# david-andrew/TerminalRayTracer

Hardware: AMD Instinct MI355X
Metric: path rays/s (primary+secondary) at 1920x1080, 64 spheres, 8 bounces (higher is better)
Workload: dtype f64

## Files before the change

include/trt_hip_diag.h:

```cpp
#ifndef TRT_HIP_DIAG_H
#define TRT_HIP_DIAG_H

#include "trt_hip.h"

#ifdef __cplusplus
extern "C" {
#endif

int trt_set_list_pool_words(trt_context *ctx, size_t words);

int trt_enable_counters(trt_context *ctx, int enable);

int trt_read_counters(trt_context *ctx, unsigned long long *path_rays, unsigned long long *shadow_rays);

int trt_read_diagnostics(trt_context *ctx, unsigned long long *wave_loop_trips, unsigned long long *phase2_rounds);

int trt_path_family_code(trt_context *ctx, int kind, int sphere, const double *parent_origin);

long trt_read_path_tables(trt_context *ctx, const Camera *camera, unsigned long long *cells, size_t capacity_cells,
                          unsigned long long *pool, size_t capacity_pool, long info[8]);

int trt_read_sweep_fallbacks(trt_context *ctx, unsigned long long *swept_traces);

int trt_read_shading_passes(trt_context *ctx, unsigned long long *passes);

int trt_read_loop_diagnostics(trt_context *ctx, unsigned long long out[8]);

long trt_read_light_grid(trt_context *ctx, int point_light, int index, unsigned long long *masks, size_t capacity_words);

long trt_read_light_lists(trt_context *ctx, int point_light, int index, unsigned long long *cells, size_t capacity_cells,
                          unsigned long long *pool, size_t capacity_pool, long info[4]);

int trt_selftest_div_sqrt(trt_context *ctx, const double *a, const double *b, size_t n, double *quot, double *root);

int trt_selftest_unit(trt_context *ctx, const double *xyzw, size_t n, double *fast, double *reference);

int trt_selftest_cube(trt_context *ctx, const float *xyz, size_t n, float *device_out, float *host_out);

int trt_selftest_sky(trt_context *ctx, const double *dirs, size_t n, int dim, long long *exact, long long *estimate, int *ambiguous);

int trt_probe_rays(trt_context *ctx, const Ray *rays, size_t n, int *obj, double *point, double *normal,
                   double *material, double *lit);

int trt_probe_rays_production(trt_context *ctx, const Camera *camera, const Ray *rays, const int *families, size_t n, int *obj,
                              double *point, double *normal, double *material, double *lit);

long trt_launch_count(trt_context *ctx);
int trt_launch_span_ms(trt_context *first, long first_launch, trt_context *last, long last_launch, float *ms);

int trt_set_scene_image(trt_context *ctx, int mode);

int trt_render_image(trt_context *ctx, int *in_device_memory, unsigned long long *image_bytes);

int trt_set_scratch_fill(trt_context *ctx, int on);

int trt_dist_allow_rccl_override(int allow);

trt_context *trt_default_context(void);

int trt_build_counts(trt_context *ctx, unsigned long long *table_builds, unsigned long long *skybox_uploads);

int trt_ansi_delta_kernel_times(trt_context *ctx, const void *d_shown_rgb8, const void *d_next_rgb8, int width, int rows, void *d_text,
                                size_t capacity_bytes, unsigned long long *d_bytes, float *ms);
int trt_ansi_delta_half_kernel_times(trt_context *ctx, const void *d_shown_rgb8, const void *d_next_rgb8, int width, int rows, void *d_text,
                                     size_t capacity_bytes, unsigned long long *d_bytes, float *ms);

#ifdef __cplusplus
}
#endif
#endif
```

terminalraytracer_amd/csrc/trt_capi.hip:

```cpp
#include "trt_context.hpp"

using namespace trt_impl;

namespace trt_impl
{

thread_local char g_error[512] = "";

int fail(int code, const char *fmt, ...)
{
    va_list ap;
    va_start(ap, fmt);
    vsnprintf(g_error, sizeof g_error, fmt, ap);
    va_end(ap);
    return code;
}

unsigned long long skybox_stamp(const Skybox *sky)
{
    unsigned long long h = 1469598103934665603ull;
    const size_t face = (size_t)sky->dim * sky->dim, step = face / 256 ? face / 256 : 1;
    for (int f = 0; f < 6; f++)
        for (size_t i = 0; i < face; i += step)
        {
            const Color c = sky->colors[f][i];
            h = (h ^ c.r) * 1099511628211ull;
            h = (h ^ c.g) * 1099511628211ull;
            h = (h ^ c.b) * 1099511628211ull;
        }
    const Color last = sky->colors[5][face - 1];
    return (h ^ ((unsigned)last.r << 16 | (unsigned)last.g << 8 | last.b)) * 1099511628211ull;
}

int upload_skybox(trt_context *ctx, const Skybox *sky)
{
    const int dim = sky->dim;
    if (dim <= 0)
        return fail(TRT_ERR_ARGUMENT, "skybox dim %d", dim);
    for (int f = 0; f < 6; f++)
        if (!sky->colors[f])
            return fail(TRT_ERR_ARGUMENT, "skybox face %d is NULL", f);
    const size_t face = (size_t)dim * dim;
    std::vector<uint32_t> packed(6 * face);
    for (int f = 0; f < 6; f++)
    {
        const Color *src = sky->colors[f];
        uint32_t *dst = packed.data() + f * face;
        for (size_t i = 0; i < face; i++)
            dst[i] = (uint32_t)src[i].r | ((uint32_t)src[i].g << 8) | ((uint32_t)src[i].b << 16);
    }
    HIP_TRY(ctx->T->d_sky.reserve(6 * face));
    HIP_TRY(hipMemcpy(ctx->T->d_sky.ptr, packed.data(), packed.size() * sizeof(uint32_t), hipMemcpyHostToDevice));
    ctx->scene.sky = ctx->T->d_sky.ptr;
    ctx->scene.sky_dim = dim;
    ctx->scene.sky_dim_f = (double)dim;
    for (int f = 0; f < 6; f++)
        ctx->sky_faces[f] = sky->colors[f];
    ctx->sky_dim = dim;
    ctx->sky_stamp = skybox_stamp(sky);
    ctx->skybox_uploads++;
    return TRT_OK;
}

int g_moving_after = 2, g_still_after = 3;

int upload_primitives(trt_context *ctx, const Scene *scene, bool per_call)
{
    const int n = scene->num_spheres, nd = scene->num_directional_lights, np = scene->num_point_lights;
    if (n < 0 || nd < 0 || np < 0)
        return fail(TRT_ERR_ARGUMENT, "negative primitive count");
    if ((n && !scene->spheres) || (nd && !scene->directional_lights) || (np && !scene->point_lights))
        return fail(TRT_ERR_ARGUMENT, "NULL primitive array with a non-zero count");
    HIP_TRY(ctx->T->d_spheres.reserve((size_t)n * 9));
    HIP_TRY(ctx->T->d_dir.reserve((size_t)nd * 6));
    HIP_TRY(ctx->T->d_point.reserve((size_t)np * 7));
    if (n)
        HIP_TRY(hipMemcpy(ctx->T->d_spheres.ptr, scene->spheres, (size_t)n * sizeof(Sphere), hipMemcpyHostToDevice));
    if (nd)
        HIP_TRY(hipMemcpy(ctx->T->d_dir.ptr, scene->directional_lights, (size_t)nd * sizeof(DirectionalLight), hipMemcpyHostToDevice));
    if (np)
        HIP_TRY(hipMemcpy(ctx->T->d_point.ptr, scene->point_lights, (size_t)np * sizeof(PointLight), hipMemcpyHostToDevice));

    const int padded = trt_cull_padded(n, trt::kCullGroup);
    std::vector<float> cull((size_t)padded * 4);
    trt_cull_scene cs;
    trt_cull_build((const double *)scene->spheres, n, trt::kCullGroup, cull.data(), &cs);
    HIP_TRY(ctx->T->d_cull.reserve(cull.size()));
    if (padded)
        HIP_TRY(hipMemcpy(ctx->T->d_cull.ptr, cull.data(), cull.size() * sizeof(float), hipMemcpyHostToDevice));
    ctx->cull.table = ctx->T->d_cull.ptr;
    ctx->cull.padded = padded;
    ctx->cull.c0x = cs.c0[0];
    ctx->cull.c0y = cs.c0[1];
    ctx->cull.c0z = cs.c0[2];
    ctx->cull.cn = cs.cn;
    ctx->cull.rm = cs.rm;

    const double *hs = (const double *)scene->spheres, *hd = (const double *)scene->directional_lights, *hp = (const double *)scene->point_lights;
    const bool same_primitives = ctx->T->h_spheres.size() == (size_t)n * 9 && ctx->T->h_dir.size() == (size_t)nd * 6 && ctx->T->h_point.size() == (size_t)np * 7 &&
                                 (!n || !memcmp(ctx->T->h_spheres.data(), hs, (size_t)n * sizeof(Sphere))) &&
                                 (!nd || !memcmp(ctx->T->h_dir.data(), hd, (size_t)nd * sizeof(DirectionalLight))) &&
                                 (!np || !memcmp(ctx->T->h_point.data(), hp, (size_t)np * sizeof(PointLight))) &&
                                 !memcmp(ctx->T->ground_built, &scene->ground, sizeof ctx->T->ground_built);
    if (!per_call)
        ctx->moving_scene = false, ctx->scene_changes_in_a_row = ctx->scene_still_calls = 0;
    else if (!same_primitives)
    {
        ctx->scene_still_calls = 0;
        if (++ctx->scene_changes_in_a_row >= g_moving_after && g_moving_after > 0)
            ctx->moving_scene = true;
    }
    else
    {
        ctx->scene_changes_in_a_row = 0;
        if (++ctx->scene_still_calls >= g_still_after)
            ctx->moving_scene = false;
    }
    const bool same = same_primitives && ctx->T->built_for_moving_scene == ctx->moving_scene &&
                      ctx->T->grids_built_for[0] == ctx->dirgrid_cells && ctx->T->grids_built_for[1] == ctx->pointgrid_cells &&
                      ctx->T->grids_built_for[2] == ctx->dirgrid_slabs && ctx->T->grids_built_for[3] == ctx->pointgrid_shells &&
                      ctx->T->path_built_for[0] == ctx->path_g_eye && ctx->T->path_built_for[1] == ctx->path_g_sph &&
                      ctx->T->path_built_for[2] == ctx->path_min_spheres && ctx->T->path_built_for[3] == ctx->path_patches &&
                      !memcmp(ctx->T->ground_built, &scene->ground, sizeof ctx->T->ground_built);
    if (!same)
    {
        ctx->T->h_spheres.assign(hs, hs + (size_t)n * 9);
        ctx->T->h_dir.assign(hd, hd + (size_t)nd * 6);
        ctx->T->h_point.assign(hp, hp + (size_t)np * 7);
        ctx->T->built_for_moving_scene = ctx->moving_scene;
        const int rc = build_tables(ctx, cs, (const double *)&scene->ground);
        if (rc)
        {
            ctx->T->grids_built_for[0] = ctx->T->grids_built_for[1] = ctx->T->grids_built_for[2] = ctx->T->grids_built_for[3] = -1;
            return rc;
        }
    }

    trt::SceneView &v = ctx->scene;
    v.spheres = ctx->T->d_spheres.ptr;
    v.dir_lights = ctx->T->d_dir.ptr;
    v.point_lights = ctx->T->d_point.ptr;
    v.num_spheres = n;
    v.num_dir = nd;
    v.num_point = np;
    memcpy(v.ground, &scene->ground, sizeof(Plane));
    return refresh_occupancy(ctx);
}

}

extern "C" int trt_rowset_rows(const trt_rowset *r)
{
    if (!rowset_valid(r))
        return 0;
    const int tiles = (r->height + r->tile_rows - 1) / r->tile_rows;
    long rows = 0;
    for (int t = r->tile_first; t < tiles; t += r->tile_step)
        rows += std::min(r->tile_rows, r->height - t * r->tile_rows);
    return (int)rows;
}

extern "C" int trt_rowset_frame_row(const trt_rowset *r, int local_row)
{
    if (!rowset_valid(r) || local_row < 0 || local_row >= trt_rowset_rows(r))
        return -1;
    const int t = local_row / r->tile_rows;
    return (r->tile_first + t * r->tile_step) * r->tile_rows + (local_row - t * r->tile_rows);
}

extern "C" const char *trt_last_error(void) { return g_error; }
extern "C" const char *trt_version(void) { return "trt-mi355x 0.1 (gfx950, fp64, contraction off)"; }

static int init_context(trt_context *ctx);

extern "C" int trt_create(int device, trt_context **out)
{
    if (!out)
        return fail(TRT_ERR_ARGUMENT, "out is NULL");
    *out = nullptr;
    int count = 0;
    HIP_TRY(hipGetDeviceCount(&count));
    if (device < 0 || device >= count)
        return fail(TRT_ERR_ARGUMENT, "device %d out of range (%d visible)", device, count);
    HIP_TRY(hipSetDevice(device));
    std::unique_ptr<trt_context> ctx(new trt_context());
    ctx->device = device;
    const int rc = init_context(ctx.get());
    if (rc)
        return rc;
    *out = ctx.release();
    return TRT_OK;
}

static int init_context(trt_context *ctx)
{
    const int device = ctx->device;
    hipDeviceProp_t prop;
    HIP_TRY(hipGetDeviceProperties(&prop, device));
    ctx->compute_units = prop.multiProcessorCount;
    ctx->lds_limit = (int)prop.sharedMemPerBlock;
    ctx->T = std::make_shared<SceneTables>();
    ctx->T->device = device;
    ctx->T->eye_slots_taken = 1u;
    if (const char *e = getenv("TRT_LIGHTGRID"))
    {
        int gd = 0, gp = 0, sd = TRT_DIRGRID_SLABS, sp = TRT_POINTGRID_SHELLS;
        if (sscanf(e, "%d,%d,%d,%d", &gd, &gp, &sd, &sp) >= 2 && gd >= 0 && gp >= 0 && gd <= 2048 && gp <= 1024 && sd >= 1 && sp >= 1 && sd <= 64 && sp <= 64)
            ctx->dirgrid_cells = gd, ctx->pointgrid_cells = gp, ctx->dirgrid_slabs = sd, ctx->pointgrid_shells = sp;
    }
    if (const char *e = getenv("TRT_PATHGRID"))
    {
        int ge = 0, gs = 0, m = TRT_PATHGRID_PATCHES;
        if (sscanf(e, "%d,%d,%d", &ge, &gs, &m) >= 2 && ge >= 0 && gs >= 0 && ge <= 1024 && gs <= 256 && m >= -1 && m <= TRT_PATCH_MAX_M)
            ctx->path_g_eye = ge, ctx->path_g_sph = gs, ctx->path_patches = m;
    }
    if (const char *e = getenv("TRT_COMPACTION"))
    {
        int mode = -1;
        if (sscanf(e, "%d", &mode) == 1 && mode >= -1 && mode <= 1)
            ctx->compaction = mode;
    }
    HIP_TRY(ctx->own_stream.create());
    ctx->stream = ctx->own_stream;
    for (int i = 0; i < kEventRing; i++)
    {
        HIP_TRY(ctx->ev_start[i].create());
        HIP_TRY(ctx->ev_mid[i].create());
        HIP_TRY(ctx->ev_stop[i].create());
    }
    for (Event &e : ctx->ev_chunk)
        HIP_TRY(e.create(hipEventDisableTiming));
    for (Event &e : ctx->ev_band)
        HIP_TRY(e.create(hipEventDisableTiming));
    HIP_TRY(ctx->ev_fork.create(hipEventDisableTiming));
    HIP_TRY(ctx->d_counters.reserve(kCounterSlots));
    HIP_TRY(ctx->d_queue.reserve(trt::kQueueWords));
    HIP_TRY(hipMemset(ctx->d_counters.ptr, 0, kCounterSlots * sizeof(unsigned long long)));
    HIP_TRY(hipMemset(ctx->d_queue.ptr, 0, trt::kQueueWords * sizeof(unsigned int)));
    allow_large_lds_tables(ctx);
    allow_large_lds_render(ctx);
    allow_large_lds_diag(ctx);
    return TRT_OK;
}

extern "C" int trt_destroy(trt_context *ctx)
{
    if (!ctx)
        return TRT_OK;
    delete ctx;
    (void)hipGetLastError();
    return TRT_OK;
}

extern "C" int trt_set_stream(trt_context *ctx, void *hip_stream)
{
    if (!ctx)
        return fail(TRT_ERR_ARGUMENT, "ctx is NULL");
    HIP_TRY(hipSetDevice(ctx->device));
    HIP_TRY(hipStreamSynchronize(ctx->stream));
    ctx->stream = hip_stream ? (hipStream_t)hip_stream : ctx->own_stream;
    return TRT_OK;
}

extern "C" int trt_reserve_cus(trt_context *ctx, int reserved)
{
    if (!ctx || reserved < 0)
        return fail(TRT_ERR_ARGUMENT, "bad argument");
    if (reserved > ctx->compute_units / 2)
        return fail(TRT_ERR_ARGUMENT, "%d of %d compute units", reserved, ctx->compute_units);
    HIP_TRY(hipSetDevice(ctx->device));
    HIP_TRY(hipStreamSynchronize(ctx->stream));
    const bool was_own = ctx->stream == ctx->own_stream;
    Stream fresh;
    if (reserved == 0)
        HIP_TRY(fresh.create());
    else
    {
        std::vector<uint32_t> mask((size_t)(ctx->compute_units + 31) / 32, 0u);
        for (int cu = 0; cu < ctx->compute_units - reserved; cu++)
            mask[(size_t)cu / 32] |= 1u << (cu % 32);
        HIP_TRY(fresh.create((uint32_t)mask.size(), mask.data()));
    }
    ctx->own_stream = std::move(fresh);
    if (was_own)
        ctx->stream = ctx->own_stream;
    ctx->reserved_cus = reserved;
    return TRT_OK;
}

extern "C" int trt_get_stream(trt_context *ctx, void **hip_stream)
{
    if (!ctx || !hip_stream)
        return fail(TRT_ERR_ARGUMENT, "NULL argument");
    *hip_stream = (void *)ctx->stream;
    return TRT_OK;
}

static void detach_tables(trt_context *ctx)
{
    if (ctx->T.use_count() <= 1)
        return;
    ctx->T->eye_slots_taken &= ~(1u << ctx->eye_slot);
    ctx->T = std::make_shared<SceneTables>();
    ctx->T->device = ctx->device;
    ctx->T->eye_slots_taken = 1u;
    ctx->eye_slot = 0;
    invalidate_eye_tables(ctx);
    ctx->grids = trt::GridView{};
    ctx->sky_dim = -1;
}

namespace trt_impl
{
int refuse_if_shared(const trt_context *ctx, const char *what)
{
    if (ctx->T.use_count() > 1)
        return fail(TRT_ERR_ARGUMENT, "%s: this context's scene tables are shared with %ld other context(s) (trt_share_scene); "
                                      "change them before sharing, or give the context a scene of its own (trt_set_scene)", what, ctx->T.use_count() - 1);
    return TRT_OK;
}
}

extern "C" int trt_share_scene(trt_context *dst, trt_context *src)
{
    if (!dst || !src || dst == src)
        return fail(TRT_ERR_ARGUMENT, "bad argument");
    if (!src->have_scene)
        return fail(TRT_ERR_NO_SCENE, "the source context has no scene");
    if (dst->device != src->device)
        return fail(TRT_ERR_ARGUMENT, "contexts of different devices (%d, %d) cannot share tables", dst->device, src->device);
    HIP_TRY(hipSetDevice(dst->device));
    HIP_TRY(hipStreamSynchronize(dst->stream));
    HIP_TRY(hipStreamSynchronize(src->stream));
    if (dst->T == src->T)
        return TRT_OK;
    int slot = -1;
    for (int k = 0; k < kEyeSlots && slot < 0; k++)
        if (!(src->T->eye_slots_taken & (1u << k)))
            slot = k;
    if (slot < 0)
        return fail(TRT_ERR_CAPACITY, "%d contexts share these tables already", kEyeSlots);
    dst->T->eye_slots_taken &= ~(1u << dst->eye_slot);
    dst->T = src->T;
    dst->T->eye_slots_taken |= 1u << slot;
    dst->eye_slot = slot;
    dst->scene = src->scene;
    dst->cull = src->cull;
    dst->grids = src->grids;
    dst->grids.eye_at = (unsigned)((size_t)slot * 2 * 6 * (size_t)src->grids.g_eye * (size_t)src->grids.g_eye);
    invalidate_eye_tables(dst);
    invalidate_eye_tables(src, src->eye_slot);
    dst->dirgrid_cells = src->dirgrid_cells, dst->pointgrid_cells = src->pointgrid_cells;
    dst->dirgrid_slabs = src->dirgrid_slabs, dst->pointgrid_shells = src->pointgrid_shells;
    dst->path_g_eye = src->path_g_eye, dst->path_g_sph = src->path_g_sph, dst->path_min_spheres = src->path_min_spheres;
    dst->path_patches = src->path_patches, dst->list_pool_cap = src->list_pool_cap;
    memcpy(dst->sky_faces, src->sky_faces, sizeof dst->sky_faces);
    dst->sky_dim = src->sky_dim;
    dst->sky_stamp = src->sky_stamp;
    dst->ior_count = 0;
    dst->have_scene = true;
    dst->occupancy_for_lds = (size_t)-1;
    return refresh_occupancy(dst);
}

extern "C" int trt_scene_info(trt_context *ctx, unsigned long long *table_bytes, int *sharers, double *build_seconds)
{
    if (!ctx)
        return fail(TRT_ERR_ARGUMENT, "ctx is NULL");
    const SceneTables &t = *ctx->T;
    if (table_bytes)
        *table_bytes = t.d_spheres.capacity * 8 + t.d_dir.capacity * 8 + t.d_point.capacity * 8 + t.d_cull.capacity * 4 + t.d_dir_masks.capacity * 8 +
                       t.d_point_masks.capacity * 8 + t.d_dirgrids.capacity * sizeof(trt_dirgrid) + t.d_pointgrids.capacity * sizeof(trt_pointgrid) +
                       t.d_discs.capacity * sizeof(trt_dirgrid_disc) + t.d_cones.capacity * sizeof(trt_pointgrid_cone) + t.d_dir_lists.capacity * 8 +
                       t.d_point_lists.capacity * 8 + t.d_path_lists.capacity * 8 + t.d_pool.capacity * 8 + t.d_pool_used.capacity * 8 +
                       t.d_families.capacity * sizeof(trt_rayfamily) + t.d_sphere_fam.capacity * 8 + t.d_patch_rec.capacity * 8 + t.d_sky.capacity * 4;
    if (sharers)
        *sharers = (int)ctx->T.use_count();
    if (build_seconds)
        *build_seconds = t.build_seconds;
    return TRT_OK;
}

extern "C" int trt_set_scene(trt_context *ctx, const Scene *scene)
{
    if (!ctx || !scene)
        return fail(TRT_ERR_ARGUMENT, "NULL argument");
    HIP_TRY(hipSetDevice(ctx->device));
    HIP_TRY(hipStreamSynchronize(ctx->stream));
    ctx->have_scene = false;
    detach_tables(ctx);
    int rc = upload_primitives(ctx, scene);
    if (rc)
        return rc;
    rc = upload_skybox(ctx, &scene->skybox);
    if (rc)
        return rc;
    ctx->have_scene = true;
    return TRT_OK;
}

extern "C" int trt_set_refraction(trt_context *ctx, const double *ior, int count)
{
    if (!ctx || count < 0 || (count > 0 && !ior))
        return fail(TRT_ERR_ARGUMENT, "bad argument");
    HIP_TRY(hipSetDevice(ctx->device));
    HIP_TRY(hipStreamSynchronize(ctx->stream));
    ctx->ior_count = 0;
    if (count == 0)
        return TRT_OK;
    for (int i = 0; i < count; i++)
        if (!(ior[i] >= 0.0) || !(ior[i] < 1e6))
            return fail(TRT_ERR_ARGUMENT, "index of refraction %g of sphere %d", ior[i], i);
    HIP_TRY(ctx->d_ior.reserve((size_t)count));
    HIP_TRY(hipMemcpy(ctx->d_ior.ptr, ior, (size_t)count * sizeof(double), hipMemcpyHostToDevice));
    ctx->ior_count = count;
    return TRT_OK;
}

extern "C" int trt_set_kernel(trt_context *ctx, int which)
{
    if (!ctx || which < 0 || which > 1)
        return fail(TRT_ERR_ARGUMENT, "kernel %d", which);
    ctx->kernel = which;
    return TRT_OK;
}

extern "C" int trt_set_compaction(trt_context *ctx, int mode)
{
    if (!ctx || mode < -1 || mode > 1)
        return fail(TRT_ERR_ARGUMENT, "compaction mode %d", mode);
    ctx->compaction = mode;
    return TRT_OK;
}

extern "C" int trt_set_light_grids(trt_context *ctx, int directional_cells, int point_cells)
{
    if (!ctx || directional_cells < 0 || point_cells < 0 || directional_cells > 2048 || point_cells > 1024)
        return fail(TRT_ERR_ARGUMENT, "light grids %d, %d", directional_cells, point_cells);
    if (const int shared = refuse_if_shared(ctx, "trt_set_light_grids"))
        return shared;
    HIP_TRY(hipSetDevice(ctx->device));
    HIP_TRY(hipStreamSynchronize(ctx->stream));
    ctx->dirgrid_cells = directional_cells;
    ctx->pointgrid_cells = point_cells;
    if (!ctx->have_scene)
        return TRT_OK;
    const int n = (int)(ctx->T->h_spheres.size() / 9);
    std::vector<float> table((size_t)trt_cull_padded(n, trt::kCullGroup) * 4 + 4);
    trt_cull_scene cs;
    trt_cull_build(ctx->T->h_spheres.data(), n, trt::kCullGroup, table.data(), &cs);
    const int rc = build_tables(ctx, cs, ctx->scene.ground);
    return rc ? rc : refresh_occupancy(ctx);
}

extern "C" int trt_set_light_slabs(trt_context *ctx, int directional_slabs, int point_shells)
{
    if (!ctx || directional_slabs < 1 || point_shells < 1 || directional_slabs > 64 || point_shells > 64)
        return fail(TRT_ERR_ARGUMENT, "light slabs %d, %d", directional_slabs, point_shells);
    if (const int shared = refuse_if_shared(ctx, "trt_set_light_slabs"))
        return shared;
    const int slabs_before = ctx->dirgrid_slabs, shells_before = ctx->pointgrid_shells;
    ctx->dirgrid_slabs = directional_slabs;
    ctx->pointgrid_shells = point_shells;
    const int rc = trt_set_light_grids(ctx, ctx->dirgrid_cells, ctx->pointgrid_cells);
    if (rc)
        ctx->dirgrid_slabs = slabs_before, ctx->pointgrid_shells = shells_before;
    return rc;
}

extern "C" int trt_set_path_grids(trt_context *ctx, int eye_cells, int sphere_cells)
{
    if (!ctx || eye_cells < 0 || sphere_cells < 0 || eye_cells > 1024 || sphere_cells > 256)
        return fail(TRT_ERR_ARGUMENT, "path grids %d, %d", eye_cells, sphere_cells);
    if (const int shared = refuse_if_shared(ctx, "trt_set_path_grids"))
        return shared;
    HIP_TRY(hipSetDevice(ctx->device));
    HIP_TRY(hipStreamSynchronize(ctx->stream));
    ctx->path_g_eye = eye_cells;
    ctx->path_g_sph = sphere_cells;
    if (!ctx->have_scene)
        return TRT_OK;
    const int n = (int)(ctx->T->h_spheres.size() / 9);
    std::vector<float> table((size_t)trt_cull_padded(n, trt::kCullGroup) * 4 + 4);
    trt_cull_scene cs;
    trt_cull_build(ctx->T->h_spheres.data(), n, trt::kCullGroup, table.data(), &cs);
    const int rc = build_tables(ctx, cs, ctx->scene.ground);
    return rc ? rc : refresh_occupancy(ctx);
}

extern "C" int trt_set_path_patches(trt_context *ctx, int m)
{
    if (!ctx || m < -1 || m > TRT_PATCH_MAX_M)
        return fail(TRT_ERR_ARGUMENT, "patches %d", m);
    if (const int shared = refuse_if_shared(ctx, "trt_set_path_patches"))
        return shared;
    HIP_TRY(hipSetDevice(ctx->device));
    HIP_TRY(hipStreamSynchronize(ctx->stream));
    ctx->path_patches = m;
    if (!ctx->have_scene)
        return TRT_OK;
    const int n = (int)(ctx->T->h_spheres.size() / 9);
    std::vector<float> table((size_t)trt_cull_padded(n, trt::kCullGroup) * 4 + 4);
    trt_cull_scene cs;
    trt_cull_build(ctx->T->h_spheres.data(), n, trt::kCullGroup, table.data(), &cs);
    const int rc = build_tables(ctx, cs, ctx->scene.ground);
    return rc ? rc : refresh_occupancy(ctx);
}

extern "C" int trt_get_path_patches(trt_context *ctx, int *m, int *patches_per_sphere)
{
    if (!ctx)
        return fail(TRT_ERR_ARGUMENT, "ctx is NULL");
    if (m)
        *m = ctx->grids.path_enabled ? ctx->grids.patch_m : 0;
    if (patches_per_sphere)
        *patches_per_sphere = ctx->grids.path_enabled ? ctx->grids.patch_count : 0;
    return TRT_OK;
}

extern "C" int trt_set_path_grids_min_spheres(trt_context *ctx, int min_spheres)
{
    if (!ctx || min_spheres < 0)
        return fail(TRT_ERR_ARGUMENT, "min_spheres %d", min_spheres);
    if (const int shared = refuse_if_shared(ctx, "trt_set_path_grids_min_spheres"))
        return shared;
    HIP_TRY(hipSetDevice(ctx->device));
    HIP_TRY(hipStreamSynchronize(ctx->stream));
    ctx->path_min_spheres = min_spheres;
    if (!ctx->have_scene)
        return TRT_OK;
    const int n = (int)(ctx->T->h_spheres.size() / 9);
    std::vector<float> table((size_t)trt_cull_padded(n, trt::kCullGroup) * 4 + 4);
    trt_cull_scene cs;
    trt_cull_build(ctx->T->h_spheres.data(), n, trt::kCullGroup, table.data(), &cs);
    const int rc = build_tables(ctx, cs, ctx->scene.ground);
    return rc ? rc : refresh_occupancy(ctx);
}
```

terminalraytracer_amd/csrc/trt_context.hpp:

```cpp
#pragma once

#include "trt_hip.h"
#include "trt_hip_diag.h"

#include <hip/hip_runtime.h>

#include <math.h>
#include <stdarg.h>
#include <stdio.h>
#include <stdlib.h>
#include <string.h>

#include <algorithm>
#include <chrono>
#include <memory>
#include <mutex>
#include <thread>
#include <vector>

#ifndef TRT_DIRGRID_CELLS
#define TRT_DIRGRID_CELLS 128
#endif
#ifndef TRT_POINTGRID_CELLS
#define TRT_POINTGRID_CELLS 64
#endif
#ifndef TRT_DIRGRID_SLABS
#define TRT_DIRGRID_SLABS 16
#endif
#ifndef TRT_POINTGRID_SHELLS
#define TRT_POINTGRID_SHELLS 16
#endif

#ifndef TRT_PATHGRID_EYE
#define TRT_PATHGRID_EYE 64
#endif
#ifndef TRT_PATHGRID_SPHERE
#define TRT_PATHGRID_SPHERE 32
#endif
#ifndef TRT_PATHGRID_MIN_SPHERES
#define TRT_PATHGRID_MIN_SPHERES 12
#endif
#ifndef TRT_PATHGRID_PATCHES
#define TRT_PATHGRID_PATCHES -1
#endif
#ifndef TRT_PATCHES_FROM_SPHERES
#define TRT_PATCHES_FROM_SPHERES 128
#endif

#include "trt_common.hpp"
#include "trt_handles.hpp"
#include "trt_rounds.hpp"

namespace trt_impl
{

int fail(int code, const char *fmt, ...);

inline double host_seconds()
{
    return std::chrono::duration<double>(std::chrono::steady_clock::now().time_since_epoch()).count();
}

#define HIP_TRY(expr)                                                                                      \
    do                                                                                                     \
    {                                                                                                      \
        hipError_t e_ = (expr);                                                                            \
        if (e_ != hipSuccess)                                                                              \
            return fail(TRT_ERR_HIP, "%s failed: %s (%s:%d)", #expr, hipGetErrorString(e_), __FILE__, __LINE__); \
    } while (0)

#if defined(TRT_MARKS) && TRT_MARKS == 2
constexpr int kCounterSlots = trt::kProfileAt + 64 * trt::kProfileKinds;
#else
constexpr int kCounterSlots = 40;
#endif
constexpr int kEventRing = 256;
constexpr double kPi = 3.14159265358979323846;


inline double triangle_wave(double t)
{
    double m = fmod(t, 2 * kPi);
    return (m < kPi) ? (m / kPi) : (2 - (m / kPi));
}

}

using trt_impl::DeviceBuffer;
using trt_impl::Event;
using trt_impl::PinnedBuffer;
using trt_impl::Stream;
using trt_impl::kEventRing;

constexpr int kEyeSlots = 8;

struct SceneTables
{
    int device = 0;
    DeviceBuffer<double> d_spheres, d_dir, d_point;
    DeviceBuffer<float> d_cull;
    DeviceBuffer<unsigned long long> d_dir_masks, d_point_masks;
    DeviceBuffer<trt_dirgrid> d_dirgrids;
    DeviceBuffer<trt_pointgrid> d_pointgrids;
    DeviceBuffer<trt_dirgrid_disc> d_discs;
    DeviceBuffer<trt_pointgrid_cone> d_cones;
    DeviceBuffer<unsigned long long> d_dir_lists, d_point_lists, d_path_lists, d_pool;
    DeviceBuffer<unsigned long long> d_pool_used;
    DeviceBuffer<trt_rayfamily> d_families;
    DeviceBuffer<double> d_sphere_fam;
    DeviceBuffer<double> d_patch_rec;
    DeviceBuffer<uint32_t> d_sky;
    int path_built_for[4] = {-1, -1, -1, -2};
    int grids_built_for[4] = {-1, -1, -1, -1};
    size_t pool_scene_words = 0, pool_eye_words = 0;
    trt_cull_scene cull_scene{};
    double ground_built[6] = {0.0, 0.0, 0.0, 0.0, 0.0, 0.0};
    std::vector<double> h_spheres, h_dir, h_point;
    unsigned eye_slots_taken = 0;
    bool built_for_moving_scene = false;
    double build_seconds = 0.0;
    ~SceneTables() { (void)hipSetDevice(device); }
};

struct trt_context
{
    int device = 0;
    Stream own_stream;
    hipStream_t stream = nullptr;
    int compute_units = 0;
    int reserved_cus = 0;
    int lds_limit = 0;

    bool have_scene = false;
    std::shared_ptr<SceneTables> T;
    int eye_slot = 0;
    trt::SceneView scene{};
    trt::CullView cull{};
    DeviceBuffer<double> d_jitter, d_fb, d_axes, d_samples, d_samples_alt;
    DeviceBuffer<double> d_image, d_image_alt;
    trt::GridView grids{};
    int dirgrid_cells = TRT_DIRGRID_CELLS, pointgrid_cells = TRT_POINTGRID_CELLS;
    int dirgrid_slabs = TRT_DIRGRID_SLABS, pointgrid_shells = TRT_POINTGRID_SHELLS;
    int path_g_eye = TRT_PATHGRID_EYE, path_g_sph = TRT_PATHGRID_SPHERE;
    int path_min_spheres = TRT_PATHGRID_MIN_SPHERES;
    int path_patches = TRT_PATHGRID_PATCHES;
    size_t list_pool_cap = 0;
    int scene_changes_in_a_row = 0, scene_still_calls = 0;
    bool moving_scene = false;
    struct EyeSlot
    {
        double eye[3];
        trt_rayfamily families[2];
        bool valid;
    };
    EyeSlot eye_slots[kEyeSlots] = {};
    int batch_frames = 0, batch_launches = 0;
    struct BatchOccupancy
    {
        const void *kernel;
        size_t lds;
        int blocks;
    };
    std::vector<BatchOccupancy> batch_occupancy;
    DeviceBuffer<double> d_ior;
    DeviceBuffer<unsigned char> d_rgb8;
    DeviceBuffer<unsigned char> d_text;
    DeviceBuffer<unsigned char> d_text_rgb8;
    DeviceBuffer<unsigned char> d_shown[2];
    int shown_at = 0;
    bool shown_valid = false;
    bool shown_half = false;
    trt_rowset shown_rows{};
    DeviceBuffer<unsigned> d_delta_tile_bytes;
    DeviceBuffer<unsigned long long> d_delta_tile_at;
    DeviceBuffer<unsigned long long> d_delta_bytes;
    int ior_count = 0;
    DeviceBuffer<unsigned long long> d_counters;
    DeviceBuffer<unsigned int> d_queue;
    PinnedBuffer h_staging;

    int jit_spp = -1;
    double jit_pw = 0.0, jit_ph = 0.0;
    int axes_w = -1, axes_h = -1;
    double axes_sw = 0.0, axes_sh = 0.0;

    int kernel = 0;
    int rounds_blocks_per_cu = 0;
    int compact_blocks_per_cu = 0;
    int big_blocks_per_cu = 0;
    int device_blocks_per_cu = 0;
    int scene_image = -1;
    int last_variant = -1;
    int last_spp = 64;
    unsigned queue_ready[2][3] = {{0, 0, 0}, {0, 0, 0}};
    int compaction = -1;
    bool scratch_fill = false;
    size_t occupancy_for_lds = (size_t)-1;
    Event ev_chunk[16];
    Event ev_band[8];
    Stream copy_stream;
    Stream alt_stream;
    Event ev_fork;
    bool counters_enabled = false;
    unsigned long long last_trips = 0, last_phase2 = 0, last_swept = 0, last_passes = 0;
    unsigned long long last_loops[8] = {0, 0, 0, 0, 0, 0, 0, 0};

    Event ev_start[kEventRing], ev_mid[kEventRing], ev_stop[kEventRing];
    long launches = 0;

    const void *sky_faces[6] = {nullptr, nullptr, nullptr, nullptr, nullptr, nullptr};
    int sky_dim = -1;
    unsigned long long sky_stamp = 0;
    unsigned long long table_builds = 0, skybox_uploads = 0;

    ~trt_context()
    {
        (void)hipSetDevice(device);
        if (stream)
            (void)hipStreamSynchronize(stream);
        if (T)
            T->eye_slots_taken &= ~(1u << eye_slot);
    }
};

namespace trt_impl
{

inline size_t image_lds_bytes(const trt_context *ctx, int spp, int frames = 1)
{
    return trt::rounds_lds_bytes(ctx->scene, spp, ctx->grids.path_enabled ? ctx->grids.patch_count : 0, frames);
}

inline size_t compact_ring_at(const trt_context *ctx, int spp, int frames = 1)
{
    return (image_lds_bytes(ctx, spp, frames) / sizeof(double) + 1) & ~(size_t)1;
}

inline size_t compact_lds_bytes(const trt_context *ctx, int spp, int frames = 1)
{
    return sizeof(double) * (compact_ring_at(ctx, spp, frames) + (size_t)(trt::kCompactBlock / 64) * trt::kRingDoubles);
}

inline size_t scene_lds_bytes(const trt::SceneView &s)
{
    return sizeof(double) * ((size_t)s.num_spheres * trt::kSphereDoubles + (size_t)s.num_dir * trt::kDirLightDoubles +
                             (size_t)s.num_point * trt::kPointLightDoubles);
}

inline double host_now_ms()
{
    return std::chrono::duration<double, std::milli>(std::chrono::steady_clock::now().time_since_epoch()).count();
}
inline bool print_host_times()
{
    static const bool on = getenv("TRT_PRINT_HOST_TIMES") != nullptr;
    return on;
}

inline bool rowset_valid(const trt_rowset *r)
{
    return r && r->width > 0 && r->height > 0 && r->tile_rows > 0 && r->tile_first >= 0 && r->tile_step > 0;
}

inline void invalidate_eye_tables(trt_context *ctx, int keep = -1)
{
    for (int s = 0; s < kEyeSlots; s++)
        if (s != keep)
            ctx->eye_slots[s] = {};
}

int upload_skybox(trt_context *ctx, const Skybox *sky);
unsigned long long skybox_stamp(const Skybox *sky);
int upload_primitives(trt_context *ctx, const Scene *scene, bool per_call = false);
int refuse_if_shared(const trt_context *ctx, const char *what);
extern int g_moving_after, g_still_after;
int patches_for(const trt_context *ctx, int n);
int build_tables(trt_context *ctx, const trt_cull_scene &cs, const double *ground);
int ensure_eye_tables(trt_context *ctx, const Camera *camera, hipStream_t stream, int slot = -1);
void allow_large_lds_tables(const trt_context *ctx);
int refresh_occupancy(trt_context *ctx);
int prepare_jitter(trt_context *ctx, const Camera *cam, int width, int height, int spp);
int prepare_axes(trt_context *ctx, const Camera *cam, int width, int height);
void allow_large_lds_render(const trt_context *ctx);
void allow_large_lds_diag(const trt_context *ctx);

}
```

terminalraytracer_amd/csrc/trt_diag.hip:

```cpp
#define TRT_UNIT_DIAG 1
#include "trt_context.hpp"
#include "trt_simple.hpp"

using namespace trt_impl;

namespace trt_impl
{
void allow_large_lds_diag(const trt_context *ctx)
{
    (void)hipFuncSetAttribute((const void *)trt::probe_rays_kernel, hipFuncAttributeMaxDynamicSharedMemorySize, ctx->lds_limit);
    (void)hipFuncSetAttribute((const void *)trt::probe_rounds_kernel<false>, hipFuncAttributeMaxDynamicSharedMemorySize, ctx->lds_limit);
    (void)hipFuncSetAttribute((const void *)trt::probe_rounds_kernel<true>, hipFuncAttributeMaxDynamicSharedMemorySize, ctx->lds_limit);
}
}

extern "C" int trt_set_list_pool_words(trt_context *ctx, size_t words)
{
    if (!ctx)
        return fail(TRT_ERR_ARGUMENT, "ctx is NULL");
    const int rc = refuse_if_shared(ctx, "trt_set_list_pool_words");
    if (rc)
        return rc;
    ctx->list_pool_cap = words;
    ctx->T->grids_built_for[0] = -1;
    return TRT_OK;
}

extern "C" int trt_read_diagnostics(trt_context *ctx, unsigned long long *wave_loop_trips, unsigned long long *phase2_rounds)
{
    if (!ctx)
        return fail(TRT_ERR_ARGUMENT, "ctx is NULL");
    if (wave_loop_trips)
        *wave_loop_trips = ctx->last_trips;
    if (phase2_rounds)
        *phase2_rounds = ctx->last_phase2;
    return TRT_OK;
}

extern "C" int trt_read_sweep_fallbacks(trt_context *ctx, unsigned long long *swept_traces)
{
    if (!ctx || !swept_traces)
        return fail(TRT_ERR_ARGUMENT, "NULL argument");
    *swept_traces = ctx->last_swept;
    return TRT_OK;
}

extern "C" int trt_read_loop_diagnostics(trt_context *ctx, unsigned long long out[8])
{
    if (!ctx || !out)
        return fail(TRT_ERR_ARGUMENT, "NULL argument");
    memcpy(out, ctx->last_loops, sizeof ctx->last_loops);
    return TRT_OK;
}

extern "C" int trt_read_shading_passes(trt_context *ctx, unsigned long long *passes)
{
    if (!ctx || !passes)
        return fail(TRT_ERR_ARGUMENT, "NULL argument");
    *passes = ctx->last_passes;
    return TRT_OK;
}

extern "C" int trt_path_family_code(trt_context *ctx, int kind, int sphere, const double *parent_origin)
{
    if (!ctx || !ctx->have_scene || !ctx->grids.path_enabled || kind < 0 || kind > 3)
        return -1;
    if (kind < 2)
        return kind;
    const int n = (int)(ctx->T->h_spheres.size() / 9);
    if (sphere < 0 || sphere >= n)
        return -1;
    if (kind == 2)
        return 2 + sphere;
    if (!parent_origin)
        return -1;
    if (!ctx->grids.patch_m)
        return 2 + n + sphere;
    const double *c = ctx->T->h_spheres.data() + 9 * (size_t)sphere;
    const int k = trt_patch_of(ctx->grids.patch_m, parent_origin[0] - c[0], parent_origin[1] - c[1], parent_origin[2] - c[2]);
    return 2 + n + ((sphere << TRT_PATCH_SHIFT) | k);
}

extern "C" long trt_read_path_tables(trt_context *ctx, const Camera *camera, unsigned long long *cells, size_t capacity_cells,
                                     unsigned long long *pool, size_t capacity_pool, long info[8])
{
    if (!ctx || !camera || !cells || !pool || !info)
        return fail(TRT_ERR_ARGUMENT, "NULL argument");
    if (!ctx->have_scene)
        return fail(TRT_ERR_NO_SCENE, "no scene");
    HIP_TRY(hipSetDevice(ctx->device));
    const int rc = ensure_eye_tables(ctx, camera, ctx->stream);
    if (rc)
        return rc;
    HIP_TRY(hipStreamSynchronize(ctx->stream));
    const trt::GridView &g = ctx->grids;
    const int n = (int)(ctx->T->h_spheres.size() / 9);
    unsigned long long used[16 * (1 + kEyeSlots)] = {0};
    HIP_TRY(hipMemcpy(used, ctx->T->d_pool_used.ptr, sizeof used, hipMemcpyDeviceToHost));
    const size_t eye_total = 2 * 6 * (size_t)g.g_eye * g.g_eye, sph_total = 2 * (size_t)n * (size_t)g.patch_count * 6 * (size_t)g.g_sph * g.g_sph;
    const size_t total = g.path_enabled ? eye_total + sph_total : 0;
    const size_t pool_words = ctx->T->pool_scene_words + kEyeSlots * ctx->T->pool_eye_words;
    const size_t eye_from = ctx->T->pool_scene_words + (size_t)ctx->eye_slot * ctx->T->pool_eye_words;
    info[0] = g.path_enabled, info[1] = g.g_eye, info[2] = g.g_sph, info[3] = n, info[4] = (long)total;
    info[5] = (long)std::min<unsigned long long>(used[0], 1ull << 62), info[6] = (long)used[16 * (1 + ctx->eye_slot)] - (long)eye_from, info[7] = (long)pool_words;
    if (!g.path_enabled)
        return 0;
    if (capacity_cells < total || capacity_pool < pool_words)
        return fail(TRT_ERR_CAPACITY, "tables have %zu cells and %zu pool words", total, pool_words);
    HIP_TRY(hipMemcpy(cells, ctx->T->d_path_lists.ptr + g.eye_at, eye_total * sizeof(unsigned long long), hipMemcpyDeviceToHost));
    if (sph_total)
        HIP_TRY(hipMemcpy(cells + eye_total, ctx->T->d_path_lists.ptr + g.sph_at, sph_total * sizeof(unsigned long long), hipMemcpyDeviceToHost));
    HIP_TRY(hipMemcpy(pool, ctx->T->d_pool.ptr, pool_words * sizeof(unsigned long long), hipMemcpyDeviceToHost));
    return (long)total;
}

extern "C" long trt_read_light_grid(trt_context *ctx, int point_light, int index, unsigned long long *masks, size_t capacity_words)
{
    if (!ctx || !masks || index < 0)
        return fail(TRT_ERR_ARGUMENT, "bad argument");
    if (!ctx->have_scene)
        return fail(TRT_ERR_NO_SCENE, "no scene");
    const trt::GridView &g = ctx->grids;
    if (!g.enabled)
        return 0;
    if (index >= (point_light ? ctx->scene.num_point : ctx->scene.num_dir))
        return fail(TRT_ERR_ARGUMENT, "light %d", index);
    const size_t words = (size_t)std::max((ctx->scene.num_spheres + 63) / 64, 1);
    const size_t stride = (point_light ? g.point_stride : g.dir_stride) * words;
    if (capacity_words < stride)
        return fail(TRT_ERR_CAPACITY, "table has %zu words, buffer %zu", stride, capacity_words);
    HIP_TRY(hipSetDevice(ctx->device));
    HIP_TRY(hipStreamSynchronize(ctx->stream));
    HIP_TRY(hipMemcpy(masks, (point_light ? ctx->T->d_point_masks.ptr : ctx->T->d_dir_masks.ptr) + stride * (size_t)index, stride * sizeof(unsigned long long),
                      hipMemcpyDeviceToHost));
    return (long)stride;
}

extern "C" long trt_read_light_lists(trt_context *ctx, int point_light, int index, unsigned long long *cells, size_t capacity_cells,
                                     unsigned long long *pool, size_t capacity_pool, long info[4])
{
    const bool query = !cells && !pool && !capacity_cells && !capacity_pool;
    if (!ctx || !info || index < 0 || (!query && (!cells || !pool)))
        return fail(TRT_ERR_ARGUMENT, "bad argument");
    if (!ctx->have_scene)
        return fail(TRT_ERR_NO_SCENE, "no scene");
    const trt::GridView &g = ctx->grids;
    const size_t stride = point_light ? g.point_stride : g.dir_stride;
    const size_t pool_words = ctx->T->pool_scene_words;
    info[0] = g.enabled ? (long)stride : 0, info[1] = g.list_bits, info[2] = g.enabled ? (long)pool_words : 0, info[3] = g.enabled;
    if (!g.enabled)
        return 0;
    if (index >= (point_light ? ctx->scene.num_point : ctx->scene.num_dir))
        return fail(TRT_ERR_ARGUMENT, "light %d", index);
    if (query)
        return (long)stride;
    if (capacity_cells < stride || capacity_pool < pool_words)
        return fail(TRT_ERR_CAPACITY, "table has %zu cells and %zu pool words", stride, pool_words);
    HIP_TRY(hipSetDevice(ctx->device));
    HIP_TRY(hipStreamSynchronize(ctx->stream));
    HIP_TRY(hipMemcpy(cells, (point_light ? ctx->T->d_point_lists.ptr : ctx->T->d_dir_lists.ptr) + stride * (size_t)index, stride * sizeof(unsigned long long),
                      hipMemcpyDeviceToHost));
    HIP_TRY(hipMemcpy(pool, ctx->T->d_pool.ptr, pool_words * sizeof(unsigned long long), hipMemcpyDeviceToHost));
    return (long)stride;
}

extern "C" int trt_selftest_div_sqrt(trt_context *ctx, const double *a, const double *b, size_t n, double *quot, double *root)
{
    if (!ctx || !a || !b || !quot || !root)
        return fail(TRT_ERR_ARGUMENT, "NULL argument");
    if (n == 0)
        return TRT_OK;
    HIP_TRY(hipSetDevice(ctx->device));
    DeviceBuffer<double> buf;
    HIP_TRY(buf.reserve(4 * n));
    double *da = buf.ptr, *db = buf.ptr + n, *dq = buf.ptr + 2 * n, *dr = buf.ptr + 3 * n;
    HIP_TRY(hipMemcpy(da, a, n * sizeof(double), hipMemcpyHostToDevice));
    HIP_TRY(hipMemcpy(db, b, n * sizeof(double), hipMemcpyHostToDevice));
    hipLaunchKernelGGL(trt::div_sqrt_kernel, dim3((unsigned)((n + 255) / 256)), dim3(256), 0, ctx->stream, da, db, (long)n, dq, dr);
    HIP_TRY(hipGetLastError());
    HIP_TRY(hipStreamSynchronize(ctx->stream));
    HIP_TRY(hipMemcpy(quot, dq, n * sizeof(double), hipMemcpyDeviceToHost));
    HIP_TRY(hipMemcpy(root, dr, n * sizeof(double), hipMemcpyDeviceToHost));
    return TRT_OK;
}

extern "C" int trt_selftest_unit(trt_context *ctx, const double *xyzw, size_t n, double *fast, double *reference)
{
    if (!ctx || !xyzw || !fast || !reference)
        return fail(TRT_ERR_ARGUMENT, "NULL argument");
    if (n == 0)
        return TRT_OK;
    HIP_TRY(hipSetDevice(ctx->device));
    DeviceBuffer<double> buf;
    HIP_TRY(buf.reserve(12 * n));
    double *dv = buf.ptr, *df = buf.ptr + 4 * n, *dr = buf.ptr + 8 * n;
    HIP_TRY(hipMemcpy(dv, xyzw, 4 * n * sizeof(double), hipMemcpyHostToDevice));
    hipLaunchKernelGGL(trt::unit_selftest_kernel, dim3((unsigned)((n + 255) / 256)), dim3(256), 0, ctx->stream, dv, (long)n, df, dr);
    HIP_TRY(hipGetLastError());
    HIP_TRY(hipStreamSynchronize(ctx->stream));
    HIP_TRY(hipMemcpy(fast, df, 4 * n * sizeof(double), hipMemcpyDeviceToHost));
    HIP_TRY(hipMemcpy(reference, dr, 4 * n * sizeof(double), hipMemcpyDeviceToHost));
    return TRT_OK;
}

namespace
{
__global__ void cube_selftest_kernel(const float *xyz, long n, float *out)
{
    const long i = (long)blockIdx.x * blockDim.x + threadIdx.x;
    if (i >= n)
        return;
    int face;
    float sc, tc, ma2;
    trt_cube_lookup(xyz[3 * i], xyz[3 * i + 1], xyz[3 * i + 2], &face, &sc, &tc, &ma2);
    out[4 * i] = (float)face, out[4 * i + 1] = sc, out[4 * i + 2] = tc, out[4 * i + 3] = ma2;
}
}

namespace
{
__global__ void sky_selftest_kernel(const double *dirs, long n, int dim, long *exact, long *estimate, int *ambiguous)
{
    const long i = (long)blockIdx.x * blockDim.x + threadIdx.x;
    if (i >= n)
        return;
    const trt::d3 d = trt::d3{dirs[3 * i], dirs[3 * i + 1], dirs[3 * i + 2]};
    bool amb;
    exact[i] = trt::sky_index_unit(dim, d, (double)dim);
    estimate[i] = trt::sky_index_estimate(dim, (float)dim, d, amb);
    ambiguous[i] = amb;
}
}

extern "C" int trt_selftest_sky(trt_context *ctx, const double *dirs, size_t n, int dim, long long *exact, long long *estimate, int *ambiguous)
{
    if (!ctx || !dirs || !exact || !estimate || !ambiguous || dim < 1)
        return fail(TRT_ERR_ARGUMENT, "bad argument");
    if (n == 0)
        return TRT_OK;
    HIP_TRY(hipSetDevice(ctx->device));
    DeviceBuffer<double> in;
    DeviceBuffer<long> out;
    DeviceBuffer<int> flags;
    HIP_TRY(in.reserve(3 * n));
    HIP_TRY(out.reserve(2 * n));
    HIP_TRY(flags.reserve(n));
    HIP_TRY(hipMemcpy(in.ptr, dirs, 3 * n * sizeof(double), hipMemcpyHostToDevice));
    hipLaunchKernelGGL(sky_selftest_kernel, dim3((unsigned)((n + 255) / 256)), dim3(256), 0, ctx->stream, (const double *)in.ptr, (long)n, dim, out.ptr, out.ptr + n, flags.ptr);
    HIP_TRY(hipGetLastError());
    HIP_TRY(hipStreamSynchronize(ctx->stream));
    HIP_TRY(hipMemcpy(exact, out.ptr, n * sizeof(long), hipMemcpyDeviceToHost));
    HIP_TRY(hipMemcpy(estimate, out.ptr + n, n * sizeof(long), hipMemcpyDeviceToHost));
    HIP_TRY(hipMemcpy(ambiguous, flags.ptr, n * sizeof(int), hipMemcpyDeviceToHost));
    return TRT_OK;
}

extern "C" int trt_selftest_cube(trt_context *ctx, const float *xyz, size_t n, float *device_out, float *host_out)
{
    if (!ctx || !xyz || !device_out || !host_out)
        return fail(TRT_ERR_ARGUMENT, "NULL argument");
    if (n == 0)
        return TRT_OK;
    HIP_TRY(hipSetDevice(ctx->device));
    DeviceBuffer<float> buf;
    HIP_TRY(buf.reserve(7 * n));
    HIP_TRY(hipMemcpy(buf.ptr, xyz, 3 * n * sizeof(float), hipMemcpyHostToDevice));
    hipLaunchKernelGGL(cube_selftest_kernel, dim3((unsigned)((n + 255) / 256)), dim3(256), 0, ctx->stream, (const float *)buf.ptr, (long)n, buf.ptr + 3 * n);
    HIP_TRY(hipGetLastError());
    HIP_TRY(hipStreamSynchronize(ctx->stream));
    HIP_TRY(hipMemcpy(device_out, buf.ptr + 3 * n, 4 * n * sizeof(float), hipMemcpyDeviceToHost));
    for (size_t i = 0; i < n; i++)
    {
        int face;
        float sc, tc, ma2;
        trt_cube_lookup(xyz[3 * i], xyz[3 * i + 1], xyz[3 * i + 2], &face, &sc, &tc, &ma2);
        host_out[4 * i] = (float)face, host_out[4 * i + 1] = sc, host_out[4 * i + 2] = tc, host_out[4 * i + 3] = ma2;
    }
    return TRT_OK;
}

extern "C" int trt_probe_rays(trt_context *ctx, const Ray *rays, size_t n, int *obj, double *point, double *normal,
                              double *material, double *lit)
{
    if (!ctx || !rays || !obj || !point || !normal || !material || !lit)
        return fail(TRT_ERR_ARGUMENT, "NULL argument");
    if (!ctx->have_scene)
        return fail(TRT_ERR_NO_SCENE, "trt_set_scene has not been called");
    if (n == 0)
        return TRT_OK;
    HIP_TRY(hipSetDevice(ctx->device));
    DeviceBuffer<double> buf;
    DeviceBuffer<int> dobj;
    HIP_TRY(buf.reserve(n * (6 + 3 + 3 + 5 + 3)));
    HIP_TRY(dobj.reserve(n));
    double *dr = buf.ptr, *dp = dr + 6 * n, *dn = dp + 3 * n, *dm = dn + 3 * n, *dl = dm + 5 * n;
    HIP_TRY(hipMemcpy(dr, rays, n * sizeof(Ray), hipMemcpyHostToDevice));
    hipLaunchKernelGGL(trt::probe_rays_kernel, dim3((unsigned)((n + 255) / 256)), dim3(256), scene_lds_bytes(ctx->scene), ctx->stream,
                       ctx->scene, dr, (long)n, dobj.ptr, dp, dn, dm, dl);
    HIP_TRY(hipGetLastError());
    HIP_TRY(hipStreamSynchronize(ctx->stream));
    HIP_TRY(hipMemcpy(obj, dobj.ptr, n * sizeof(int), hipMemcpyDeviceToHost));
    HIP_TRY(hipMemcpy(point, dp, 3 * n * sizeof(double), hipMemcpyDeviceToHost));
    HIP_TRY(hipMemcpy(normal, dn, 3 * n * sizeof(double), hipMemcpyDeviceToHost));
    HIP_TRY(hipMemcpy(material, dm, 5 * n * sizeof(double), hipMemcpyDeviceToHost));
    HIP_TRY(hipMemcpy(lit, dl, 3 * n * sizeof(double), hipMemcpyDeviceToHost));
    return TRT_OK;
}

extern "C" int trt_probe_rays_production(trt_context *ctx, const Camera *camera, const Ray *rays, const int *families, size_t n, int *obj,
                                         double *point, double *normal, double *material, double *lit)
{
    if (!ctx || !camera || !rays || !obj || !point || !normal || !material || !lit)
        return fail(TRT_ERR_ARGUMENT, "NULL argument");
    if (!ctx->have_scene)
        return fail(TRT_ERR_NO_SCENE, "trt_set_scene has not been called");
    if (n == 0)
        return TRT_OK;
    HIP_TRY(hipSetDevice(ctx->device));
    const int rc = ensure_eye_tables(ctx, camera, ctx->stream);
    if (rc)
        return rc;
    DeviceBuffer<double> buf;
    DeviceBuffer<int> dobj;
    HIP_TRY(buf.reserve(n * (6 + 3 + 3 + 5 + 3)));
    HIP_TRY(dobj.reserve(2 * n));
    double *dr = buf.ptr, *dp = dr + 6 * n, *dn = dp + 3 * n, *dm = dn + 3 * n, *dl = dm + 5 * n;
    HIP_TRY(hipMemcpy(dr, rays, n * sizeof(Ray), hipMemcpyHostToDevice));
    if (families)
    {
        const int ns = ctx->scene.num_spheres, pm = ctx->grids.path_enabled ? ctx->grids.patch_m : 0, pc = ctx->grids.path_enabled ? ctx->grids.patch_count : 0;
        std::vector<int> codes(families, families + n);
        for (int &c : codes)
        {
            bool ok = c == 0 || c == 1 || (c >= 2 && c < 2 + ns);
            if (!ok && c >= 2 + ns)
            {
                const int rest = c - 2 - ns;
                ok = pm ? ((rest >> TRT_PATCH_SHIFT) < ns && (rest & ((1 << TRT_PATCH_SHIFT) - 1)) < pc) : rest < ns;
            }
            if (!ok)
                c = -1;
        }
        HIP_TRY(hipMemcpy(dobj.ptr + n, codes.data(), n * sizeof(int), hipMemcpyHostToDevice));
    }
    trt::FrameView f{};
    memcpy(f.cam, camera, sizeof(Camera));
    f.jitter = ctx->d_jitter.ptr;
    if (ctx->grids.path_enabled && ctx->grids.patch_m > 0)
        hipLaunchKernelGGL(trt::probe_rounds_kernel<true>, dim3((unsigned)((n + trt::kPersistentBlock - 1) / trt::kPersistentBlock)), dim3(trt::kPersistentBlock),
                           image_lds_bytes(ctx, 0), ctx->stream, ctx->scene, ctx->cull, f, ctx->grids, (const double *)dr,
                           families ? (const int *)(dobj.ptr + n) : (const int *)nullptr, (long)n, dobj.ptr, dp, dn, dm, dl);
    else
        hipLaunchKernelGGL(trt::probe_rounds_kernel<false>, dim3((unsigned)((n + trt::kPersistentBlock - 1) / trt::kPersistentBlock)), dim3(trt::kPersistentBlock),
                           image_lds_bytes(ctx, 0), ctx->stream, ctx->scene, ctx->cull, f, ctx->grids, (const double *)dr,
                           families ? (const int *)(dobj.ptr + n) : (const int *)nullptr, (long)n, dobj.ptr, dp, dn, dm, dl);
    HIP_TRY(hipGetLastError());
    HIP_TRY(hipStreamSynchronize(ctx->stream));
    HIP_TRY(hipMemcpy(obj, dobj.ptr, n * sizeof(int), hipMemcpyDeviceToHost));
    HIP_TRY(hipMemcpy(point, dp, 3 * n * sizeof(double), hipMemcpyDeviceToHost));
    HIP_TRY(hipMemcpy(normal, dn, 3 * n * sizeof(double), hipMemcpyDeviceToHost));
    HIP_TRY(hipMemcpy(material, dm, 5 * n * sizeof(double), hipMemcpyDeviceToHost));
    HIP_TRY(hipMemcpy(lit, dl, 3 * n * sizeof(double), hipMemcpyDeviceToHost));
    return TRT_OK;
}
```

terminalraytracer_amd/csrc/trt_raygrid.h:

```cpp
#ifndef TRT_RAYGRID_H
#define TRT_RAYGRID_H

#include "trt_lightgrid.h"

typedef struct
{
    double a[3];
    double r_chk;
    double r_chk2;
    double rg2;
} trt_rayfamily;

#define TRT_RAYFAMILY_DOUBLES 6

#define TRT_LIST_MAX_SPHERES 256
#define TRT_PATH_MAX_SPHERES 1024
#define TRT_LIST_MAX_SPHERES_WIDE 65535
#define TRT_LIST_POOLED 0x80u
#define TRT_LIST_NONE 0xFFu

TRT_HD void trt_mirror_point(const double p[3], const double p0[3], const double nrm[3], double out[3])
{
    const double nn = nrm[0] * nrm[0] + nrm[1] * nrm[1] + nrm[2] * nrm[2];
    const double h = ((p[0] - p0[0]) * nrm[0] + (p[1] - p0[1]) * nrm[1] + (p[2] - p0[2]) * nrm[2]) / nn;
    out[0] = p[0] - 2.0 * h * nrm[0];
    out[1] = p[1] - 2.0 * h * nrm[1];
    out[2] = p[2] - 2.0 * h * nrm[2];
}

#define TRT_FAMILY_SLACK 4e-6

TRT_HD void trt_rayfamily_set(trt_rayfamily *F, const double apex[3], double r_chk, double rg)
{
    F->a[0] = apex[0], F->a[1] = apex[1], F->a[2] = apex[2];
    F->r_chk = r_chk;
    F->r_chk2 = r_chk * r_chk;
    F->rg2 = rg * rg;
}

static inline void trt_eye_families(const double eye[3], const double *ground , const trt_cull_scene *cs,
                                    trt_rayfamily fam[2])
{
    const double reach = (double)cs->cn + (double)cs->rm;
    double m[3];
    trt_mirror_point(eye, ground, ground + 3, m);
    const double *apex[2] = {eye, m};
    for (int k = 0; k < 2; k++)
    {
        const double lc[3] = {apex[k][0] - cs->c0[0], apex[k][1] - cs->c0[1], apex[k][2] - cs->c0[2]};
        const double away = __builtin_sqrt(lc[0] * lc[0] + lc[1] * lc[1] + lc[2] * lc[2]);
        const double mag = __builtin_fabs(apex[k][0]) + __builtin_fabs(apex[k][1]) + __builtin_fabs(apex[k][2]) + reach;
        trt_rayfamily_set(&fam[k], apex[k], (k ? TRT_FAMILY_SLACK : 0.0) + 1e-9 * mag, TRT_LIGHTGRID_RANGE * (reach + away) + 1.0);
    }
}

TRT_HD int trt_cubemap_cell(float x, float y, float z, float half_g, float g_max, int g)
{
    int face;
    float pu, pv, ma2;
    trt_cube_lookup(x, y, z, &face, &pu, &pv, &ma2);
#if defined(__HIP_DEVICE_COMPILE__)
    const float inv = __builtin_amdgcn_rcpf(0.5f * __builtin_fabsf(ma2));
#else
    const float inv = 1.0f / (0.5f * __builtin_fabsf(ma2));
#endif
    float cu = __builtin_fmaf(pu * inv, half_g, half_g), cv = __builtin_fmaf(pv * inv, half_g, half_g);
    cu = __builtin_fminf(__builtin_fmaxf(cu, 0.0f), g_max);
    cv = __builtin_fminf(__builtin_fmaxf(cv, 0.0f), g_max);
    return (face * g + (int)cv) * g + (int)cu;
}

#define TRT_PATCH_MAX_M 4
#define TRT_PATCH_MAX (6 * TRT_PATCH_MAX_M * TRT_PATCH_MAX_M)
#define TRT_PATCH_SHIFT 7
#define TRT_PATCH_RECORD 8

typedef struct
{
    int m;
    int count;
    double rec[TRT_PATCH_MAX][4];
} trt_patchset;

static inline void trt_patchset_init(trt_patchset *P, int m)
{
    if (m < 0)
        m = 0;
    if (m > TRT_PATCH_MAX_M)
        m = TRT_PATCH_MAX_M;
    P->m = m;
    P->count = m ? 6 * m * m : 1;
    for (int k = 0; k < TRT_PATCH_MAX; k++)
        P->rec[k][0] = P->rec[k][1] = P->rec[k][2] = 0.0, P->rec[k][3] = 1.0 + 1e-6;
    if (!m)
        return;
    const double step = 2.0 / (double)m;
    for (int face = 0; face < 6; face++)
        for (int j = 0; j < m; j++)
            for (int c = 0; c < m; c++)
            {
                const double u0 = c == 0 ? -1.001 : -1.0 + ((double)c - 0.02) * step, u1 = c == m - 1 ? 1.001 : -1.0 + ((double)c + 1.02) * step;
                const double v0 = j == 0 ? -1.001 : -1.0 + ((double)j - 0.02) * step, v1 = j == m - 1 ? 1.001 : -1.0 + ((double)j + 1.02) * step;
                const double cu[4] = {u0, u1, u1, u0}, cv[4] = {v0, v0, v1, v1};
                double corner[4][3], mid[3] = {0.0, 0.0, 0.0};
                for (int q = 0; q < 4; q++)
                {
                    trt_face_direction(face, cu[q], cv[q], corner[q]);
                    const double len = __builtin_sqrt(corner[q][0] * corner[q][0] + corner[q][1] * corner[q][1] + corner[q][2] * corner[q][2]);
                    for (int a = 0; a < 3; a++)
                        corner[q][a] /= len, mid[a] += corner[q][a];
                }
                double *rec = P->rec[(face * m + j) * m + c];
                for (int a = 0; a < 3; a++)
                    rec[a] = 0.25 * mid[a];
                for (int it = 1; it <= 4096; it++)
                {
                    int far_q = 0;
                    double far_d2 = -1.0;
                    for (int q = 0; q < 4; q++)
                    {
                        const double e[3] = {corner[q][0] - rec[0], corner[q][1] - rec[1], corner[q][2] - rec[2]};
                        const double d2 = e[0] * e[0] + e[1] * e[1] + e[2] * e[2];
                        if (d2 > far_d2)
                            far_d2 = d2, far_q = q;
                    }
                    for (int a = 0; a < 3; a++)
                        rec[a] += (corner[far_q][a] - rec[a]) / (double)(it + 1);
                }
                double far2 = 0.0;
                for (int q = 0; q < 4; q++)
                {
                    const double e[3] = {corner[q][0] - rec[0], corner[q][1] - rec[1], corner[q][2] - rec[2]};
                    const double d2 = e[0] * e[0] + e[1] * e[1] + e[2] * e[2];
                    far2 = d2 > far2 ? d2 : far2;
                }
                rec[3] = __builtin_sqrt(far2) * (1.0 + 1e-6) + 1e-9;
            }
}

TRT_HD int trt_patch_of(int m, double wx, double wy, double wz)
{
    return m ? trt_cubemap_cell((float)wx, (float)wy, (float)wz, 0.5f * (float)m, (float)(m - 1), m) : 0;
}

typedef struct
{
    double rg;
    double slack;
} trt_family_consts;

#define TRT_PATCH_APEX(c, r_abs, t) ((c) + (r_abs) * (t))
#define TRT_PATCH_RCHK(r_abs, rho, slack) ((r_abs) * (rho) + (slack))

static inline void trt_mirror_offset(const double t[3], const double nrm[3], double out[3])
{
    const double zero[3] = {0.0, 0.0, 0.0};
    trt_mirror_point(t, zero, nrm, out);
}

static inline void trt_patch_records(const trt_patchset *P, const double *ground, double *out )
{
    for (int k = 0; k < P->count; k++)
    {
        double tm[3];
        trt_mirror_offset(P->rec[k], ground + 3, tm);
        double *o = out + (size_t)k * TRT_PATCH_RECORD;
        o[0] = P->rec[k][0], o[1] = P->rec[k][1], o[2] = P->rec[k][2], o[3] = P->rec[k][3];
        o[4] = tm[0], o[5] = tm[1], o[6] = tm[2], o[7] = P->rec[k][3];
    }
}

static inline void trt_sphere_families(const double *spheres, int n, const double *ground, const trt_cull_scene *cs, const trt_patchset *P,
                                       trt_rayfamily *fam, double *centres, trt_family_consts *consts)
{
    const double reach = (double)cs->cn + (double)cs->rm;
    const double mag = __builtin_fabs(cs->c0[0]) + __builtin_fabs(cs->c0[1]) + __builtin_fabs(cs->c0[2]) + reach + 1.0;
    double away = reach;
    for (int i = 0; i < n; i++)
    {
        double m[3];
        trt_mirror_point(spheres + 9 * i, ground, ground + 3, m);
        const double lc[3] = {m[0] - cs->c0[0], m[1] - cs->c0[1], m[2] - cs->c0[2]};
        const double far = __builtin_sqrt(lc[0] * lc[0] + lc[1] * lc[1] + lc[2] * lc[2]);
        away = far > away ? far : away;
    }
    const double rg = TRT_LIGHTGRID_RANGE * (reach + away) + 1.0;
    consts->rg = rg;
    consts->slack = TRT_FAMILY_SLACK + 1e-9 * mag;
    const int count = P->count;
    for (int i = 0; i < n; i++)
    {
        const double *c = spheres + 9 * i;
        const double r_abs = __builtin_fabs(c[3]);
        double m[3];
        trt_mirror_point(c, ground, ground + 3, m);
        if (centres)
            centres[4 * i + 0] = m[0], centres[4 * i + 1] = m[1], centres[4 * i + 2] = m[2],
                            centres[4 * i + 3] = P->m ? r_abs : TRT_PATCH_RCHK(r_abs, P->rec[0][3], consts->slack);
        for (int k = 0; k < count; k++)
        {
            const double *t = P->rec[k];
            double tm[3];
            trt_mirror_offset(t, ground + 3, tm);
            const double a[3] = {TRT_PATCH_APEX(c[0], r_abs, t[0]), TRT_PATCH_APEX(c[1], r_abs, t[1]), TRT_PATCH_APEX(c[2], r_abs, t[2])};
            const double am[3] = {TRT_PATCH_APEX(m[0], r_abs, tm[0]), TRT_PATCH_APEX(m[1], r_abs, tm[1]), TRT_PATCH_APEX(m[2], r_abs, tm[2])};
            const double r_chk = TRT_PATCH_RCHK(r_abs, t[3], consts->slack);
            trt_rayfamily_set(&fam[(size_t)i * count + k], a, r_chk, rg);
            trt_rayfamily_set(&fam[((size_t)n + i) * count + k], am, r_chk + TRT_FAMILY_SLACK, rg);
        }
    }
}

TRT_HD int trt_rayfamily_member(const trt_rayfamily *F, double ox, double oy, double oz, double dx, double dy, double dz)
{
    const double wx = ox - F->a[0], wy = oy - F->a[1], wz = oz - F->a[2];
    const double cx = wy * dz - wz * dy, cy = wz * dx - wx * dz, cz = wx * dy - wy * dx;
    const double c2 = cx * cx + cy * cy + cz * cz, lam = wx * dx + wy * dy + wz * dz, w2 = wx * wx + wy * wy + wz * wz;
    return c2 <= F->r_chk2 && lam >= -F->r_chk && w2 <= F->rg2;
}

TRT_HD void trt_rayfamily_cone(const trt_rayfamily *F, const double *s, trt_pointgrid_cone *c)
{
    const double rg = __builtin_sqrt(F->rg2);
    const double a[3] = {s[0] - F->a[0], s[1] - F->a[1], s[2] - F->a[2]};
    const double D = __builtin_sqrt(a[0] * a[0] + a[1] * a[1] + a[2] * a[2]);
    const double M = rg + D + __builtin_fabs(s[3]);
    const double E = 0x1p-37 * M * M;
    const double r_build = F->r_chk * (1.0 + 1e-9) + 1e-13 * rg;
    const double rho = __builtin_sqrt(s[3] * s[3] + E) + 0x1p-45 * M + r_build;
    const double sin_grow = 1.0000000000e-5, cos_grow = 0.99999999995;
    c->everywhere = !(rho / D < 0.7) ? 1.0 : 0.0;
    if (c->everywhere != 0.0)
    {
        c->a[0] = c->a[1] = c->a[2] = 0.0;
        c->sin_a = 1.0, c->cos_a = 0.0;
        return;
    }
    for (int k = 0; k < 3; k++)
        c->a[k] = a[k] / D;
    const double sn = rho / D, cn = __builtin_sqrt(1.0 - sn * sn);
    const double sg = sn * cos_grow + cn * sin_grow + 1e-12, cg = cn * cos_grow - sn * sin_grow - 1e-12;
    c->sin_a = sg < 1.0 ? sg : 1.0;
    c->cos_a = cg > 0.0 ? cg : 0.0;
    if (!(cg > 0.0))
        c->everywhere = 1.0;
}


TRT_HD int trt_list_count(const unsigned long long *mask, int words)
{
    int count = 0;
    for (int w = 0; w < words; w++)
        count += __builtin_popcountll(mask[w]);
    return count;
}

TRT_HD unsigned long long trt_list_pack(const unsigned long long *mask, int words, int count, unsigned long long *pool, unsigned pool_offset,
                                        int bits)
{
    const int per = 64 / bits, inline_max = 56 / bits;
    if (count <= inline_max)
    {
        unsigned long long cell = (unsigned long long)count << 56;
        int k = 0;
        for (int w = 0; w < words; w++)
        {
            unsigned long long m = mask[w];
            while (m)
            {
                const int lead = __builtin_clzll(m);
                m &= ~(0x8000000000000000ull >> lead);
                cell |= (unsigned long long)(unsigned)(w * 64 + lead) << (bits * k++);
            }
        }
        return cell;
    }
    if (!pool)
        return (unsigned long long)TRT_LIST_NONE << 56;
    unsigned long long cur = 0;
    int k = 0;
    for (int w = 0; w < words; w++)
    {
        unsigned long long m = mask[w];
        while (m)
        {
            const int lead = __builtin_clzll(m);
            m &= ~(0x8000000000000000ull >> lead);
            cur |= (unsigned long long)(unsigned)(w * 64 + lead) << (bits * (k % per));
            if (++k % per == 0)
            {
                pool[pool_offset + (unsigned)(k / per) - 1u] = cur;
                cur = 0;
            }
        }
    }
    if (k % per)
        pool[pool_offset + (unsigned)(k / per)] = cur;
    return ((unsigned long long)TRT_LIST_POOLED << 56) | ((unsigned long long)(unsigned)count << 32) | pool_offset;
}

TRT_HD unsigned trt_list_pool_words(int count, int bits)
{
    const int per = 64 / bits, inline_max = 56 / bits;
    return count <= inline_max ? 0u : (unsigned)((count + per - 1) / per);
}

TRT_HD int trt_list_entries(unsigned long long cell)
{
    const unsigned ctl = (unsigned)(cell >> 56);
    if (ctl == TRT_LIST_NONE)
        return -1;
    return ctl & TRT_LIST_POOLED ? (int)((cell >> 32) & 0xffffu) : (int)ctl;
}

TRT_HD int trt_list_entry(unsigned long long cell, const unsigned long long *pool, int k, int bits)
{
    const int per = 64 / bits;
    const unsigned long long emask = (1ull << bits) - 1ull;
    if ((unsigned)(cell >> 56) & TRT_LIST_POOLED)
        return (int)((pool[(unsigned)cell + (unsigned)(k / per)] >> (bits * (k % per))) & emask);
    return (int)((cell >> (bits * k)) & emask);
}

#define TRT_FAMILY_TILE 8
#define TRT_LIST_MAX_SPHERES_HOST 256
TRT_HD int trt_family_tiled(int g) { return g >= TRT_FAMILY_TILE && g % TRT_FAMILY_TILE == 0; }

static inline long trt_rayfamily_build(const double *spheres, int n, const trt_rayfamily *F, int g, unsigned long long *masks,
                                       trt_pointgrid_cone *cones)
{
    const int words = (n + 63) / 64 > 0 ? (n + 63) / 64 : 1;
    for (int i = 0; i < n; i++)
        trt_rayfamily_cone(F, spheres + 9 * i, cones + i);
    const int tiled = trt_family_tiled(g), gt = g / TRT_FAMILY_TILE;
    long bits = 0;
    long tile_of_row = -1;
    unsigned char reach[64 * TRT_LIST_MAX_SPHERES_HOST];
    for (long cell = 0; cell < 6L * g * g; cell++)
    {
        unsigned long long *m = masks + cell * words;
        for (int w = 0; w < words; w++)
            m[w] = 0;
        const int face = (int)(cell / ((long)g * g)), j = (int)((cell / g) % g), c = (int)(cell % g);
        const int cached = tiled && gt <= 64 && n <= TRT_LIST_MAX_SPHERES_HOST;
        if (cached && tile_of_row != (long)face * gt + j / TRT_FAMILY_TILE)
        {
            tile_of_row = (long)face * gt + j / TRT_FAMILY_TILE;
            for (int tc = 0; tc < gt; tc++)
                for (int i = 0; i < n; i++)
                    reach[tc * TRT_LIST_MAX_SPHERES_HOST + i] = (unsigned char)trt_pointgrid_reaches(cones + i, face, tc, j / TRT_FAMILY_TILE, gt);
        }
        for (int i = 0; i < n; i++)
        {
            const int in_tile = !tiled ? 1 : (cached ? reach[(c / TRT_FAMILY_TILE) * TRT_LIST_MAX_SPHERES_HOST + i]
                                                    : trt_pointgrid_reaches(cones + i, face, c / TRT_FAMILY_TILE, j / TRT_FAMILY_TILE, gt));
            if (in_tile && trt_pointgrid_reaches(cones + i, face, c, j, g))
            {
                trt_lightgrid_set(m, i);
                bits++;
            }
        }
    }
    return bits;
}

#endif
```

terminalraytracer_amd/csrc/trt_rounds.hpp:

```cpp
#pragma once

#include "trt_device.hpp"
#include "trt_filter.h"
#include "trt_lightgrid.h"
#include "trt_raygrid.h"
#include "trt_common.hpp"

#define TRT_EXPECT_LIST(c) __builtin_expect(!!(c), 1)
#define TRT_EXPECT_RARE(c) __builtin_expect(!!(c), 0)

namespace trt
{


#define CONSTANT_AS __attribute__((address_space(4)))
template <class T>
TRT_DEV T load_kernel_argument(const char CONSTANT_AS *at)
{
    static_assert(sizeof(T) % 8 == 0 && alignof(T) == 8, "argument structs are whole 64-bit words");
    T out;
    const unsigned long long CONSTANT_AS *src = (const unsigned long long CONSTANT_AS *)at;
    unsigned long long *dst = (unsigned long long *)&out;
#pragma unroll
    for (size_t i = 0; i < sizeof(T) / 8; i++)
        dst[i] = src[i];
    return out;
}

struct GridView
{
    const trt_dirgrid *dir;
    const trt_pointgrid *point;
    const unsigned long long *dir_lists, *point_lists;
    unsigned dir_stride, point_stride;
    int enabled;
    int list_bits;
    int path_enabled;
    int g_eye, g_sph;
    int patch_m, patch_count;
    unsigned eye_at, sph_at;
    const unsigned long long *path_lists;
    const unsigned long long *pool;
    const double *sphere_fam;
    const double *patch_rec;
    double rg2_sph;
    double slack0;
    trt_rayfamily eye[2];
};

static_assert(sizeof(trt_rayfamily) == 8 * TRT_RAYFAMILY_DOUBLES, "families of the eye in the LDS image");
static_assert(sizeof(trt_dirgrid) == 8 * kDirGridDoubles && sizeof(trt_pointgrid) == 8 * kPointGridDoubles, "light-table headers in the LDS image");

constexpr int kDirRecord = 8;

struct LdsImage
{
    const float4 *cull;
    const float4 *cull_dir;
    const double *sph;
    const double *mat;
    const double *dir;
    const double *pt;
    const double *b255;
    const double *cam;
    const double *jit;
    const trt_dirgrid *dirgrid;
    const trt_pointgrid *pointgrid;
    const double *fam;
    const double *eye;
    const double *patch;
};

inline size_t rounds_lds_bytes(const SceneView &s, int spp, int patches, int frames = 1)
{
    const size_t padded = ((size_t)s.num_spheres + kCullGroup - 1) / kCullGroup * kCullGroup;
    return sizeof(double) * (padded * 2 + (size_t)s.num_spheres * 4 + ((size_t)s.num_spheres + 2) * 5 + (size_t)s.num_dir * kDirRecord +
                             (size_t)s.num_point * 7 + 256 + kLdsCameraDoubles + 2 * (size_t)spp + 1  +
                             (size_t)s.num_dir * padded * 2 + (size_t)s.num_dir * kDirGridDoubles + (size_t)s.num_point * kPointGridDoubles +
                             (size_t)s.num_spheres * 4 + 2 * TRT_RAYFAMILY_DOUBLES + (size_t)patches * TRT_PATCH_RECORD +
                             (size_t)(frames - 1) * (kLdsCameraDoubles + 2 * TRT_RAYFAMILY_DOUBLES));
}

struct ImageParts
{
    float4 *cull, *cull_dir;
    double *sph, *mat, *dir, *pt, *b255, *cam, *jit, *dirgrid, *pointgrid, *fam, *eye, *patch;
};

TRT_DEV ImageParts image_layout(double *base, int n, int nd, int np, int padded, int spp, int frames = 1)
{
    ImageParts p;
    p.cull = (float4 *)base;
    p.sph = base + padded * 2;
    p.mat = p.sph + 4 * n;
    p.dir = p.mat + (n + 2) * 5;
    p.pt = p.dir + nd * kDirRecord;
    p.b255 = p.pt + np * 7;
    p.cam = p.b255 + 256;
    p.jit = p.cam + frames * kLdsCameraDoubles;
    p.cull_dir = (float4 *)(base + (((p.jit + 2 * spp) - base + 1) & ~1L));
    p.dirgrid = (double *)(p.cull_dir + nd * padded);
    p.pointgrid = p.dirgrid + nd * kDirGridDoubles;
    p.fam = p.pointgrid + np * kPointGridDoubles;
    p.eye = p.fam + 4 * n;
    p.patch = p.eye + frames * 2 * TRT_RAYFAMILY_DOUBLES;
    return p;
}

TRT_DEV LdsImage image_view(const ImageParts &p)
{
    return LdsImage{p.cull, p.cull_dir, p.sph, p.mat, p.dir, p.pt, p.b255, p.cam, p.jit,
                    (const trt_dirgrid *)p.dirgrid, (const trt_pointgrid *)p.pointgrid, p.fam, p.eye, p.patch};
}

TRT_DEV void fill_image(const ImageParts &p, const SceneView &s, const CullView &cull, const FrameView &f, const GridView &grids)
{
    const int n = s.num_spheres, nd = s.num_dir, np = s.num_point;
    for (int i = threadIdx.x; i < cull.padded; i += blockDim.x)
        p.cull[i] = ((const float4 *)cull.table)[i];
    for (int i = threadIdx.x; i < n; i += blockDim.x)
    {
        const double *sp = s.spheres + (long)i * kSphereDoubles;
        p.sph[4 * i + 0] = sp[0];
        p.sph[4 * i + 1] = sp[1];
        p.sph[4 * i + 2] = sp[2];
        p.sph[4 * i + 3] = sp[3] * sp[3];
        for (int j = 0; j < 5; j++)
            p.mat[i * 5 + j] = sp[4 + j];
    }
    for (int i = threadIdx.x; i < 10; i += blockDim.x)
        p.mat[n * 5 + i] = s.ground[6 + i];
    for (int i = threadIdx.x; i < nd; i += blockDim.x)
    {
        const double *li = s.dir_lights + i * kDirLightDoubles;
        const d3 tl = unit(scale(load3(li), -1.0));
        p.dir[i * kDirRecord + 0] = tl.x, p.dir[i * kDirRecord + 1] = tl.y, p.dir[i * kDirRecord + 2] = tl.z;
        p.dir[i * kDirRecord + 3] = li[3], p.dir[i * kDirRecord + 4] = li[4], p.dir[i * kDirRecord + 5] = li[5];
        p.dir[i * kDirRecord + 6] = dot(tl, tl);
        p.dir[i * kDirRecord + 7] = dot(tl, load3(s.ground + 3));
    }
    for (int i = threadIdx.x; i < np * 7; i += blockDim.x)
        p.pt[i] = s.point_lights[i];
    for (int i = threadIdx.x; i < 256; i += blockDim.x)
        p.b255[i] = (double)i / 255.0;
    for (int i = threadIdx.x; i < 12; i += blockDim.x)
        p.cam[i] = f.cam[i];
    if (threadIdx.x < 3)
        p.cam[13 + threadIdx.x] = f.cam[6 + threadIdx.x] * -f.cam[12];
    if (threadIdx.x == 0)
        p.cam[12] = -f.cam[12];
    for (int i = threadIdx.x; i < 2 * f.spp; i += blockDim.x)
        p.jit[i] = f.jitter[i];
    __syncthreads();
    for (int i = threadIdx.x; i < nd * cull.padded; i += blockDim.x)
    {
        const int li = i / cull.padded, j = i - li * cull.padded;
        const float4 e = p.cull[j];
        const float dx = (float)p.dir[li * kDirRecord + 0], dy = (float)p.dir[li * kDirRecord + 1], dz = (float)p.dir[li * kDirRecord + 2];
        p.cull_dir[i] = float4{e.x, e.y, e.z, trt_filter_fixed_dir_kk(e.x, e.y, e.z, e.w, dx, dy, dz)};
    }
    if (grids.enabled)
    {
        for (int i = threadIdx.x; i < nd * kDirGridDoubles; i += blockDim.x)
            p.dirgrid[i] = ((const double *)grids.dir)[i];
        for (int i = threadIdx.x; i < np * kPointGridDoubles; i += blockDim.x)
            p.pointgrid[i] = ((const double *)grids.point)[i];
    }
    if (grids.path_enabled)
    {
        for (int i = threadIdx.x; i < n * 4; i += blockDim.x)
            p.fam[i] = grids.sphere_fam[i];
        for (int i = threadIdx.x; i < 2 * TRT_RAYFAMILY_DOUBLES; i += blockDim.x)
            p.eye[i] = ((const double *)grids.eye)[i];
        for (int i = threadIdx.x; i < grids.patch_count * TRT_PATCH_RECORD; i += blockDim.x)
            p.patch[i] = grids.patch_rec[i];
    }
    __syncthreads();
    if (grids.enabled)
    {
        for (int i = threadIdx.x; i < nd; i += blockDim.x)
        {
            const d3 sd = load3(p.dir + i * kDirRecord);
            if (!(__builtin_fabs(dot(sd, sd) - 1.0) <= 9.094947017729282e-13))
                ((trt_dirgrid *)p.dirgrid)[i].rg2 = -1.0f;
        }
        __syncthreads();
    }
}

TRT_DEV LdsImage stage_lds_image(double *lds, const SceneView &s, const CullView &cull, const FrameView &f, const GridView &grids)
{
    const ImageParts p = image_layout(lds, s.num_spheres, s.num_dir, s.num_point, cull.padded, f.spp);
    fill_image(p, s, cull, f, grids);
    return image_view(p);
}

struct Hit
{
    double d2;
    d3 p;
    int i;
    double t;
};


template <bool ANY_HIT, bool REFRACT = false, bool UNIT_A = false>
TRT_DEV bool exact_step(const LdsImage &L, d3 o, d3 d, double a, int i, bool valid, Hit &best, int inside = -1)
{
    static_assert(!(ANY_HIT && REFRACT), "shadow rays are the reference's");
    const double2 c01 = ((const double2 *)L.sph)[2 * i], c23 = ((const double2 *)L.sph)[2 * i + 1];
    const d3 c = d3{c01.x, c01.y, c23.x};
    const d3 oc = sub(o, c);
    const double b = 2.0 * dot(oc, d);
    const double cc = dot(oc, oc) - c23.y;
    const double disc = b * b - 4.0 * a * cc;
    const bool far_root = REFRACT && i == inside;
    bool done = false;
    if (valid && !(disc < 0.0) && (b < 0.0 || far_root))
    {
        const double root = sqrt_exact(disc);
        if (ANY_HIT)
        {
            const double q = -b - root;
            bool hit = UNIT_A ? q > TRT_SHADOW_QMIN : q / (2.0 * a) > 0.0;
            if (UNIT_A && q > 0.0 && !hit)
                hit = q / (2.0 * a) > 0.0;
            best.i = hit ? i : best.i;
            done = hit;
        }
        else
        {
            const double t0 = (far_root ? -b + root : -b - root) / (2.0 * a);
            const bool hit = t0 > 0.0;
            const d3 p = d3{o.x + t0 * d.x, o.y + t0 * d.y, o.z + t0 * d.z};
            const double d2 = dist2(o, p);
            const bool closer = hit && d2 < best.d2;
            best.d2 = closer ? d2 : best.d2;
            best.t = closer ? t0 : best.t;
            best.i = closer ? i : best.i;
        }
    }
    return done;
}

constexpr int kListPrefilter = 12;


template <bool ANY_HIT, bool REFRACT = false, int MARK_BASE = 0>
TRT_DEV Hit trace(const LdsImage &L, const CullView &cull, int n, d3 o, d3 d, bool active, unsigned long long active_lanes, d3 gp, d3 gn, unsigned &phase2_rounds, unsigned &lane_tests,
                  const float4 *fixed, bool use_list, unsigned long long cell, const unsigned long long *pool, int list_bits, int inside = -1,
                  const double *shared_ad = nullptr)
{
#define TRT_TRACE_MARK(k) TRT_MARK_AT(MARK_BASE + (k))
    (void)fixed;
    Hit best;
    best.d2 = __builtin_inf();
    best.p = o;
    best.i = -1;
    best.t = 0.0;
    const double a = shared_ad ? shared_ad[0] : dot(d, d);
    if (TRT_EXPECT_LIST(use_list))
    {
        const unsigned ctl = (unsigned)(cell >> 56);
        bool pooled = (ctl & TRT_LIST_POOLED) != 0;
        int count = active ? (pooled ? (int)((cell >> 32) & 0xffffu) : (int)ctl) : 0;
        const unsigned at = (unsigned)cell;
        const unsigned entry_mask = (1u << list_bits) - 1u;
        const int per_shift = list_bits == 8 ? 3 : 2, per_mask = (1 << per_shift) - 1;
        int fetch_at = lanes_with(pooled) != 0 ? 0 : per_mask + 1;
        asm("" : "+s"(fetch_at));
        unsigned long long cur = cell;
        int k = 0;
        TRT_TRACE_MARK(0);
        if (__any(count > kListPrefilter))
        {
            trt_ray_filter flt;
            trt_filter_setup(&flt, o.x, o.y, o.z, d.x, d.y, d.z, a, cull.c0x, cull.c0y, cull.c0z, cull.cn, cull.rm);
            unsigned long long kept = 0, word = cell;
            int nk = 0;
            bool over = false;
            for (int j = 0; __any(j < count); j++)
            {
                const bool valid = j < count;
                if ((j & per_mask) == fetch_at)
                    if (__any(valid && pooled))
                        if (valid && pooled)
                            word = pool[at + ((unsigned)j >> per_shift)];
                const unsigned i = valid ? (unsigned)word & entry_mask : 0u;
                word >>= list_bits;
                unsigned sign;
                if (ANY_HIT && fixed)
                {
                    const float4 e = fixed[i];
                    sign = trt_filter_sign_fixed_dir(&flt, e.x, e.y, e.z, e.w);
                }
                else
                {
                    const float4 e = L.cull[i];
                    sign = trt_filter_sign(&flt, e.x, e.y, e.z, e.w);
                }
                if (valid && (!flt.ok || !(sign >> 31)))
                {
                    over = over || nk > per_mask;
                    kept |= nk <= per_mask ? (unsigned long long)i << (list_bits * nk) : 0ull;
                    nk++;
                }
            }
            if (!__any(over))
            {
                cur = kept;
                count = nk;
                pooled = false;
                fetch_at = per_mask + 1;
            }
        }
        TRT_TRACE_MARK(1);
        while (__any(k < count))
        {
            phase2_rounds++;
            const bool valid = k < count;
            lane_tests += valid;
            if ((k & per_mask) == fetch_at)
                if (__any(valid && pooled))
                    if (valid && pooled)
                        cur = pool[at + ((unsigned)k >> per_shift)];
            const int i = valid ? (int)((unsigned)cur & entry_mask) : 0;
            cur >>= list_bits;
            k++;
            if (exact_step<ANY_HIT, REFRACT, ANY_HIT>(L, o, d, a, i, valid, best, inside))
                count = 0;
        }
    }
    else
    {
        trt_ray_filter flt;
        trt_filter_setup(&flt, o.x, o.y, o.z, d.x, d.y, d.z, a, cull.c0x, cull.c0y, cull.c0z, cull.cn, cull.rm);
        TRT_TRACE_MARK(0);
        for (int base = 0; base < cull.padded; base += 64)
        {
            const int chunk = (cull.padded - base) < 64 ? (cull.padded - base) : 64;
            unsigned word[2];
#pragma unroll
            for (int h = 0; h < 2; h++)
            {
                const int first = base + 32 * h, count = (chunk - 32 * h) < 32 ? (chunk - 32 * h) : 32;
                unsigned bits = ~0u;
                for (int g = 0; g < count; g += kCullGroup)
                {
#pragma unroll
                    for (int j = 0; j < kCullGroup; j++)
                    {
                        if (ANY_HIT && fixed)
                        {
                            const float4 e = fixed[first + g + j];
                            bits = __builtin_amdgcn_alignbit(bits, trt_filter_sign_fixed_dir(&flt, e.x, e.y, e.z, e.w), 31);
                        }
                        else
                        {
                            const float4 e = L.cull[first + g + j];
                            bits = __builtin_amdgcn_alignbit(bits, trt_filter_sign(&flt, e.x, e.y, e.z, e.w), 31);
                        }
                    }
                }
                word[h] = count > 0 ? ~(bits << (32 - count)) & (count == 32 ? ~0u : ~((1u << (32 - count)) - 1u)) : 0u;
            }
            unsigned long long cand = ((unsigned long long)word[0] << 32) | word[1];
            if (!flt.ok)
                cand = chunk == 64 ? ~0ull : ~((1ull << (64 - chunk)) - 1ull);
            if (!active)
                cand = 0;
            TRT_TRACE_MARK(1);
            while (__any(cand != 0))
            {
                phase2_rounds++;
                const int lead = __builtin_clzll(cand | 1ull);
                const bool valid = cand != 0 && base + lead < n;
                lane_tests += valid;
                const int i = valid ? base + lead : 0;
                cand &= ~(0x8000000000000000ull >> lead);
                if (exact_step<ANY_HIT, REFRACT>(L, o, d, a, i, valid, best, inside))
                    cand = 0ull;
            }
        }
    }
    if (!ANY_HIT && best.i >= 0)
        best.p = d3{o.x + best.t * d.x, o.y + best.t * d.y, o.z + best.t * d.z};
    TRT_TRACE_MARK(2);
    {
        const double denom = shared_ad ? shared_ad[1] : dot(d, gn), num = dot(sub(gp, o), gn);
        const bool steep = __builtin_fabs(denom) > 0.00001;
        const bool same_sign = (long long)(__builtin_bit_cast(unsigned long long, num) ^ __builtin_bit_cast(unsigned long long, denom)) >= 0;
        const bool maybe = active && !(ANY_HIT && best.i >= 0) && steep && same_sign;
        unsigned long long maybe_lanes = active_lanes & lanes_with(steep) & lanes_with(same_sign);
        if (ANY_HIT)
            maybe_lanes &= ~lanes_with(best.i >= 0);
        if (maybe_lanes != 0)
        {
            const double t = num / denom;
            const bool hit = maybe && t > 0.00001;
            if (ANY_HIT)
                best.i = hit ? n : best.i;
            else
            {
                const d3 p = d3{o.x + t * d.x, o.y + t * d.y, o.z + t * d.z};
                const double d2 = dist2(o, p);
                const bool closer = hit && d2 < best.d2;
                best.d2 = closer ? d2 : best.d2;
                best.p.x = closer ? p.x : best.p.x;
                best.p.y = closer ? p.y : best.p.y;
                best.p.z = closer ? p.z : best.p.z;
                best.i = closer ? n : best.i;
            }
        }
    }
    TRT_TRACE_MARK(3);
#undef TRT_TRACE_MARK
    return best;
}

TRT_DEV void point_light_search(const LdsImage &L, int n, d3 o, d3 d, bool active, unsigned long long active_lanes, d3 gp, d3 gn, unsigned &rounds, unsigned &lane_tests,
                                unsigned long long cell, const unsigned long long *pool, int list_bits, double lo, double hi, bool &dark, bool &unsure)
{
    (void)n;
    const double a = dot(d, d);
    const unsigned ctl = (unsigned)(cell >> 56);
    const bool pooled = (ctl & TRT_LIST_POOLED) != 0;
    int count = active ? (pooled ? (int)((cell >> 32) & 0xffffu) : (int)ctl) : 0;
    const unsigned at = (unsigned)cell;
    const unsigned entry_mask = (1u << list_bits) - 1u;
    const int per_shift = list_bits == 8 ? 3 : 2, per_mask = (1 << per_shift) - 1;
    int fetch_at = lanes_with(pooled) != 0 ? 0 : per_mask + 1;
    asm("" : "+s"(fetch_at));
    unsigned long long cur = cell;
    int k = 0;
    dark = false, unsure = false;
    while (__any(k < count))
    {
        rounds++;
        const bool valid = k < count;
        lane_tests += valid;
        if ((k & per_mask) == fetch_at)
            if (__any(valid && pooled))
                if (valid && pooled)
                    cur = pool[at + ((unsigned)k >> per_shift)];
        const int i = valid ? (int)((unsigned)cur & entry_mask) : 0;
        cur >>= list_bits;
        k++;
        const double2 c01 = ((const double2 *)L.sph)[2 * i], c23 = ((const double2 *)L.sph)[2 * i + 1];
        const d3 oc = sub(o, d3{c01.x, c01.y, c23.x});
        const double b = 2.0 * dot(oc, d);
        const double cc = dot(oc, oc) - c23.y;
        const double disc = b * b - 4.0 * a * cc;
        if (valid && !(disc < 0.0) && b < 0.0)
        {
            const double q = -b - sqrt_exact(disc), qq = q * q;
            const bool blocks = q > TRT_SHADOW_QMIN && qq * TRT_SHADOW_K1 <= lo;
            unsure = unsure || (q > 0.0 && !blocks && !(qq >= hi));
            dark = dark || blocks;
            count = blocks ? 0 : count;
        }
    }
    {
        const double denom = dot(d, gn), num = dot(sub(gp, o), gn);
        const bool steep = __builtin_fabs(denom) > 0.00001;
        const bool same_sign = (long long)(__builtin_bit_cast(unsigned long long, num) ^ __builtin_bit_cast(unsigned long long, denom)) >= 0;
        const bool maybe = active && !dark && steep && same_sign;
        if (__any(maybe))
        {
            const double t = num / denom;
            const bool hit = maybe && t > 0.00001;
            const double qq = (t * t) * (4.0 * a) * a;
            const bool blocks = hit && qq * TRT_SHADOW_K1 <= lo;
            dark = dark || blocks;
            unsure = unsure || (hit && !blocks && !(qq >= hi));
        }
    }
    unsure = unsure && !dark;
}

template <bool BATCH = false>
TRT_DEV unsigned long long path_cell(const LdsImage &L, const GridView &G, int n, int fam, d3 o, d3 d, bool active, unsigned long long active_lanes,
                                     unsigned long long &fallback_lanes, int frame = 0)
{
    const bool in_family = fam >= 0;
    const unsigned long long family_lanes = lanes_with(in_family);
    const bool has = active && in_family;
    const int f = has ? fam : 0;
    const int s = f >= 2 ? f - 2 : 0, i = s >= n ? s - n : s;
    const bool of_eye = f < 2, mirrored = s >= n;
    const double *rec = L.fam + 4 * i;
    d3 apex = mirrored ? load3(rec) : load3(L.sph + 4 * i);
    double r_chk = mirrored ? rec[3] + TRT_FAMILY_SLACK : rec[3];
    const double *E = BATCH ? L.eye + frame * (2 * TRT_RAYFAMILY_DOUBLES) + TRT_RAYFAMILY_DOUBLES * (f & 1) : L.eye + TRT_RAYFAMILY_DOUBLES * (f & 1);
    const double rg2_eye = E[5];
    if (of_eye)
    {
        apex = load3(E);
        r_chk = E[3];
    }
    const double rg2 = of_eye ? rg2_eye : G.rg2_sph;
    const d3 w = sub(o, apex);
    const d3 c = d3{w.y * d.z - w.z * d.y, w.z * d.x - w.x * d.z, w.x * d.y - w.y * d.x};
    const bool near_line = dot(c, c) <= r_chk * r_chk, ahead = dot(w, d) >= -r_chk, in_range = dot(w, w) <= rg2;
    const bool unit_dir = __builtin_fabs(dot(d, d) - 1.0) <= 9.094947017729282e-13;
    const bool member = near_line & ahead & in_range & unit_dir;
    const unsigned long long member_lanes = family_lanes & lanes_with(near_line) & lanes_with(ahead) & lanes_with(in_range) & lanes_with(unit_dir);
    const int g = of_eye ? G.g_eye : G.g_sph;
    const int at = trt_cubemap_cell((float)d.x, (float)d.y, (float)d.z, 0.5f * (float)g, (float)(g - 1), g);
    const unsigned eye_cells = 6u * (unsigned)G.g_eye * (unsigned)G.g_eye, sph_cells = 6u * (unsigned)G.g_sph * (unsigned)G.g_sph;
    const unsigned base = of_eye ? G.eye_at + (BATCH ? 2u * (unsigned)frame + (unsigned)f : (unsigned)f) * eye_cells : G.sph_at + (unsigned)s * sph_cells;
    unsigned long long cell = 0;
    if (has && member)
        cell = G.path_lists[base + (unsigned)at];
    fallback_lanes = active_lanes & (~member_lanes | lanes_with((unsigned)(cell >> 56) == TRT_LIST_NONE));
    return cell;
}

template <bool BATCH = false>
TRT_DEV unsigned long long path_cell_patches(const LdsImage &L, const GridView &G, int n, int &fam, d3 o, d3 d, bool active, unsigned long long active_lanes,
                                             unsigned long long &fallback_lanes, int frame = 0)
{
    const bool in_family = fam >= 0;
    const unsigned long long family_lanes = lanes_with(in_family);
    const bool has = active && in_family;
    const int f = has ? fam : 0;
    const bool of_eye = f < 2, mirrored = f >= 2 + n;
    const int code = f - 2 - n;
    const int i = mirrored ? code >> TRT_PATCH_SHIFT : (of_eye ? 0 : f - 2);
    const double *at_sphere = L.sph + 4 * i, *at_mirror = L.fam + 4 * i;
    const double *src = of_eye ? L.eye + (BATCH ? frame * (2 * TRT_RAYFAMILY_DOUBLES) : 0) + TRT_RAYFAMILY_DOUBLES * (f & 1) : (mirrored ? at_mirror : at_sphere);
    const d3 base_at = load3(src);
    const int here = trt_cubemap_cell((float)(o.x - base_at.x), (float)(o.y - base_at.y), (float)(o.z - base_at.z), 0.5f * (float)G.patch_m,
                                      (float)(G.patch_m - 1), G.patch_m);
    const int k = mirrored ? code & ((1 << TRT_PATCH_SHIFT) - 1) : (of_eye ? 0 : here);
    fam = !has ? -1 : (f == 0 ? 1 : (!of_eye && !mirrored ? 2 + n + (((f - 2) << TRT_PATCH_SHIFT) | k) : -1));
    const double r_abs = of_eye ? 0.0 : at_mirror[3];
    const double *pr = L.patch + TRT_PATCH_RECORD * k + (mirrored ? 4 : 0);
    const d3 apex = d3{TRT_PATCH_APEX(base_at.x, r_abs, pr[0]), TRT_PATCH_APEX(base_at.y, r_abs, pr[1]), TRT_PATCH_APEX(base_at.z, r_abs, pr[2])};
    const double rho = pr[3];
    double rchk_eye = src[3], rg2_eye = src[5];
    asm("" : "+v"(rchk_eye), "+v"(rg2_eye));
    double r_chk = TRT_PATCH_RCHK(r_abs, rho, G.slack0), rg2 = G.rg2_sph;
    r_chk = mirrored ? r_chk + TRT_FAMILY_SLACK : r_chk;
    r_chk = of_eye ? rchk_eye : r_chk;
    rg2 = of_eye ? rg2_eye : rg2;
    const d3 w = sub(o, apex);
    const d3 c = d3{w.y * d.z - w.z * d.y, w.z * d.x - w.x * d.z, w.x * d.y - w.y * d.x};
    const bool near_line = dot(c, c) <= r_chk * r_chk, ahead = dot(w, d) >= -r_chk, in_range = dot(w, w) <= rg2;
    const bool unit_dir = __builtin_fabs(dot(d, d) - 1.0) <= 9.094947017729282e-13;
    const bool member = near_line & ahead & in_range & unit_dir;
    const unsigned long long member_lanes = family_lanes & lanes_with(near_line) & lanes_with(ahead) & lanes_with(in_range) & lanes_with(unit_dir);
    const int g = of_eye ? G.g_eye : G.g_sph;
    const int at = trt_cubemap_cell((float)d.x, (float)d.y, (float)d.z, 0.5f * (float)g, (float)(g - 1), g);
    const unsigned eye_cells = 6u * (unsigned)G.g_eye * (unsigned)G.g_eye, sph_cells = 6u * (unsigned)G.g_sph * (unsigned)G.g_sph;
    const unsigned table = ((mirrored ? (unsigned)n : 0u) + (unsigned)i) * (unsigned)G.patch_count + (unsigned)k;
    const unsigned base = of_eye ? G.eye_at + (BATCH ? 2u * (unsigned)frame + (unsigned)f : (unsigned)f) * eye_cells : G.sph_at + table * sph_cells;
    unsigned long long cell = 0;
    if (has && member)
        cell = G.path_lists[base + (unsigned)at];
    fallback_lanes = active_lanes & (~member_lanes | lanes_with((unsigned)(cell >> 56) == TRT_LIST_NONE));
    return cell;
}

TRT_DEV unsigned lanes_below(unsigned long long mask)
{
    return __builtin_amdgcn_mbcnt_hi((unsigned)(mask >> 32), __builtin_amdgcn_mbcnt_lo((unsigned)mask, 0u));
}

struct Tally
{
    unsigned path = 0, shadow = 0, rounds = 0, swept = 0, passes = 0;
    unsigned iters[3] = {0, 0, 0};
    unsigned tests[3] = {0, 0, 0};
    unsigned full = 0;
};

struct PathHit
{
    Hit ph;
    bool hit;
    bool sky;
    unsigned long long hit_lanes, sky_lanes;
    d3 back;
    d3 normal;
    int mat;
};

template <bool COUNT, bool REFRACT = false, bool PATCHES = false, bool BATCH = false>
TRT_DEV PathHit path_stage(const LdsImage &L, const CullView &cull, const GridView &grids, int n, d3 o, d3 d, int &fam, bool alive, unsigned long long alive_lanes,
                           d3 gp, d3 gn, Tally &tally, int inside = -1, int frame = 0)
{
    bool p_list = false;
    unsigned long long p_cell = 0;
    if (grids.path_enabled)
    {
        unsigned long long fallback_lanes;
        if constexpr (PATCHES)
            p_cell = path_cell_patches<BATCH>(L, grids, n, fam, o, d, alive, alive_lanes, fallback_lanes, frame);
        else
            p_cell = path_cell<BATCH>(L, grids, n, fam, o, d, alive, alive_lanes, fallback_lanes, frame);
        p_list = fallback_lanes == 0;
    }
    if (COUNT && !p_list)
        tally.swept++;
    PathHit r;
    r.ph = trace<false, REFRACT, 2>(L, cull, n, o, d, alive, alive_lanes, gp, gn, tally.iters[0], tally.tests[0], nullptr, p_list, p_cell, grids.pool, grids.list_bits, inside);
    r.hit = alive && r.ph.i >= 0;
    r.sky = alive && r.ph.i < 0;
    r.hit_lanes = alive_lanes & lanes_with(r.ph.i >= 0);
    r.sky_lanes = alive_lanes & ~r.hit_lanes;
    if (r.hit)
        fam = r.ph.i < n ? 2 + r.ph.i : (PATCHES ? fam : (fam == 0 ? 1 : (fam >= 2 && fam < 2 + n ? fam + n : -1)));
    r.back = unit(r.hit ? sub(o, r.ph.p) : d);
    r.normal = d;
    r.mat = 0;
    if (r.hit_lanes != 0)
    {
        d3 raw = gn;
        r.mat = n + checker_odd(r.ph.p);
        if (r.ph.i >= 0 && r.ph.i < n)
        {
            raw = sub(r.ph.p, load3(L.sph + 4 * r.ph.i));
            r.mat = r.ph.i;
        }
        r.normal = unit(raw);
    }
    TRT_MARK_AT(6);
    return r;
}

template <bool COUNT>
TRT_DEV d3 shadow_stage(const LdsImage &L, const CullView &cull, const GridView &grids, int n, int nd, int nl, d3 o, d3 normal, int mat,
                        bool lit_lanes, unsigned long long lit_word, d3 gp, d3 gn, Tally &tally)
{
    d3 lit = d3{0.0, 0.0, 0.0};
    if (lit_word == 0)
        return lit;
    for (int li = 0; li < nl; li++)
    {
        if (COUNT && lit_lanes)
            tally.shadow++;
        d3 sd, lcolor;
        bool is_lit;
        double factor;
        if (li < nd)
        {
            TRT_MARK_AT(24);
            sd = load3(L.dir + li * kDirRecord);
            lcolor = load3(L.dir + li * kDirRecord + 3);
            bool use_list = false;
            unsigned long long cell = 0;
            if (grids.enabled)
            {
                const trt_dirgrid *G = L.dirgrid + li;
                int far;
                const int c = trt_dirgrid_cell(G, o.x, o.y, o.z, &far);
                if (lit_lanes && !far)
                    cell = grids.dir_lists[(size_t)li * grids.dir_stride + (unsigned)c];
                use_list = (lit_word & (lanes_with(far != 0) | lanes_with((unsigned)(cell >> 56) == TRT_LIST_NONE))) == 0;
            }
            if (COUNT && !use_list)
                tally.swept++;
            TRT_MARK_AT(8);
            const Hit sh = trace<true, false, 9>(L, cull, n, o, sd, lit_lanes, lit_word, gp, gn, tally.iters[1], tally.tests[1], L.cull_dir + li * cull.padded, use_list, cell, grids.pool, grids.list_bits,
                                                 -1, L.dir + li * kDirRecord + 6);
            is_lit = sh.i < 0;
            factor = min1(dot(normal, sd));
            TRT_MARK_AT(13);
        }
        else
        {
            TRT_MARK_AT(25);
            const double *pl = L.pt + (li - nd) * 7;
            const d3 to_light = sub(load3(pl), o);
            const double light_d2 = dot(to_light, to_light);
            const double strength = clampd(pl[6] / light_d2, 0.0, 1.0);
            sd = unit(to_light);
            lcolor = load3(pl + 3);
            bool use_list = false;
            unsigned long long cell = 0;
            if (grids.enabled)
            {
                const trt_pointgrid *G = L.pointgrid + (li - nd);
                int far;
                const int c = trt_pointgrid_cell(G, o.x, o.y, o.z, &far);
                far |= !(__builtin_fabs(dot(sd, sd) - 1.0) <= 9.094947017729282e-13);
                if (lit_lanes && !far)
                    cell = grids.point_lists[(size_t)(li - nd) * grids.point_stride + (unsigned)c];
                use_list = (lit_word & (lanes_with(far != 0) | lanes_with((unsigned)(cell >> 56) == TRT_LIST_NONE))) == 0;
            }
            if (COUNT && !use_list)
                tally.swept++;
            TRT_MARK_AT(14);
            bool full = !use_list;
            is_lit = true;
            if (use_list)
            {
                const trt_pointgrid *G = L.pointgrid + (li - nd);
                double lo, hi;
                trt_point_shadow_bounds(G, light_d2, dot(sd, sd), &lo, &hi);
                bool dark, unsure;
                point_light_search(L, n, o, sd, lit_lanes, lit_word, gp, gn, tally.iters[2], tally.tests[2], cell, grids.pool, grids.list_bits, lo, hi, dark, unsure);
                is_lit = !dark;
                full = __any(lit_lanes && unsure);
                TRT_MARK_AT(17);
            }
            if (TRT_EXPECT_RARE(full))
            {
                if (COUNT)
                    tally.full++;
                const Hit sh = trace<false, false, 26>(L, cull, n, o, sd, lit_lanes, lit_word, gp, gn, tally.iters[2], tally.tests[2], nullptr, use_list, cell, grids.pool, grids.list_bits);
                is_lit = sh.i < 0;
                const bool surely_lit = light_d2 < sh.d2 * (1.0 - 1.01e-6) - 1.01e-6;
                const bool surely_dark = sh.d2 > 1e-10 && light_d2 >= sh.d2;
                if (sh.i >= 0)
                    is_lit = surely_lit;
                if (__any(lit_lanes && sh.i >= 0 && !surely_lit && !surely_dark))
                {
                    const d3 to_blocker = sub(add(sh.p, scale(unit(sub(o, sh.p)), 0.000001)), o);
                    if (sh.i >= 0 && !surely_lit && !surely_dark)
                        is_lit = light_d2 < dot(to_blocker, to_blocker);
                }
            }
            factor = strength * min1(dot(normal, sd));
            TRT_MARK_AT(19);
        }
        if (lit_lanes && is_lit)
            lit = add(lit, mulc(scale(lcolor, factor), load3(L.mat + mat * 5)));
    }
    return lit;
}

#ifndef TRT_ROUNDS_WAVES
#if TRT_BLOCK > 768
#define TRT_ROUNDS_WAVES 4
#else
#define TRT_ROUNDS_WAVES 3
#endif
#endif

constexpr int kRingTasks = 128;
constexpr int kRingDoubles = 7 * kRingTasks + kRingTasks / 4 + 3 * 64;

constexpr size_t kArgScene = 0;
constexpr size_t kArgCull = (kArgScene + sizeof(SceneView) + alignof(CullView) - 1) / alignof(CullView) * alignof(CullView);
constexpr size_t kArgFrame = (kArgCull + sizeof(CullView) + alignof(FrameView) - 1) / alignof(FrameView) * alignof(FrameView);
constexpr size_t kArgGrids = (kArgFrame + sizeof(FrameView) + alignof(GridView) - 1) / alignof(GridView) * alignof(GridView);
struct RenderKernelArguments
{
    SceneView s;
    CullView cull;
    FrameView f;
    GridView grids;
};
static_assert(offsetof(RenderKernelArguments, cull) == kArgCull && offsetof(RenderKernelArguments, f) == kArgFrame &&
                  offsetof(RenderKernelArguments, grids) == kArgGrids,
              "TRT_FRESH_ARGS reads the kernel's arguments at these offsets");

constexpr int kBatchMax = 8;
struct BatchView
{
    double cam[kBatchMax][15];
    trt_rayfamily eye[kBatchMax][2];
    unsigned frames, units_per_frame;
    unsigned frame_magic, reserved;
};
constexpr size_t kArgBatch = (kArgGrids + sizeof(GridView) + alignof(BatchView) - 1) / alignof(BatchView) * alignof(BatchView);
static_assert(kArgBatch + sizeof(BatchView) <= 4096, "the arguments of a BATCH launch fit the 4 KB kernarg segment");
static_assert(sizeof(BatchView::cam) % 8 == 0 && offsetof(BatchView, eye) == sizeof(BatchView::cam) && offsetof(BatchView, frames) % 8 == 0,
              "BatchView is read as whole 64-bit words");
constexpr int kBatchFrameShift = 28;
constexpr int kBatchBounceMask = (1 << kBatchFrameShift) - 1;
static_assert(kBatchMax <= 8, "three bits of `bounces` hold the frame");
template <class T>
TRT_DEV T *in_device_memory(T *p)
{
    T __attribute__((address_space(1))) *g = (T __attribute__((address_space(1))) *)p;
    asm("" : "+s"(g));
    return (T *)g;
}
TRT_DEV SceneView in_device_memory(SceneView v)
{
    v.spheres = in_device_memory(v.spheres), v.dir_lights = in_device_memory(v.dir_lights), v.point_lights = in_device_memory(v.point_lights);
    v.sky = in_device_memory(v.sky);
    return v;
}
TRT_DEV CullView in_device_memory(CullView v)
{
    v.table = in_device_memory(v.table);
    return v;
}
TRT_DEV FrameView in_device_memory(FrameView v)
{
    v.jitter = in_device_memory(v.jitter), v.col_x = in_device_memory(v.col_x), v.row_y = in_device_memory(v.row_y);
    v.samples = in_device_memory(v.samples), v.out = in_device_memory(v.out), v.ior = in_device_memory(v.ior);
    v.counters = in_device_memory(v.counters), v.queue = in_device_memory(v.queue);
    return v;
}
TRT_DEV GridView in_device_memory(GridView v)
{
    v.dir = in_device_memory(v.dir), v.point = in_device_memory(v.point);
    v.dir_lists = in_device_memory(v.dir_lists), v.point_lists = in_device_memory(v.point_lists);
    v.path_lists = in_device_memory(v.path_lists), v.pool = in_device_memory(v.pool), v.sphere_fam = in_device_memory(v.sphere_fam);
    v.patch_rec = in_device_memory(v.patch_rec);
    return v;
}
#define TRT_FRESH_ARGS                                                                             \
    const char CONSTANT_AS *fresh_ = (const char CONSTANT_AS *)__builtin_amdgcn_kernarg_segment_ptr(); \
    asm volatile("" : "+s"(fresh_));                                                               \
    const SceneView s = in_device_memory(load_kernel_argument<SceneView>(fresh_ + kArgScene));     \
    const CullView cull = in_device_memory(load_kernel_argument<CullView>(fresh_ + kArgCull));     \
    const FrameView f = in_device_memory(load_kernel_argument<FrameView>(fresh_ + kArgFrame));     \
    const GridView grids = in_device_memory(load_kernel_argument<GridView>(fresh_ + kArgGrids));   \
    const int n = s.num_spheres, nd = s.num_dir, nl = s.num_dir + s.num_point;                     \
    const unsigned pixels_here = (unsigned)f.local_rows * (unsigned)f.width;                       \
    const unsigned total = pixels_here * (unsigned)f.spp;                                          \
    const d3 gp = load3(s.ground), gn = load3(s.ground + 3);                                       \
    (void)n, (void)nd, (void)nl, (void)total, (void)pixels_here, (void)gp, (void)gn, (void)cull, (void)grids

struct alignas(8) BatchShape
{
    unsigned frames, units_per_frame, frame_magic, reserved;
};
TRT_DEV BatchShape load_batch_shape()
{
    const char CONSTANT_AS *args = (const char CONSTANT_AS *)__builtin_amdgcn_kernarg_segment_ptr();
    asm volatile("" : "+s"(args));
    return load_kernel_argument<BatchShape>(args + kArgBatch + offsetof(BatchView, frames));
}

TRT_DEV LdsImage stage_lds_image_batch(double *lds, const SceneView &s, const CullView &cull, const FrameView &f, const GridView &grids)
{
    const int frames = (int)load_batch_shape().frames;
    const ImageParts p = image_layout(lds, s.num_spheres, s.num_dir, s.num_point, cull.padded, f.spp, frames);
    fill_image(p, s, cull, f, grids);
    const double CONSTANT_AS *cams = (const double CONSTANT_AS *)((const char CONSTANT_AS *)__builtin_amdgcn_kernarg_segment_ptr() + kArgBatch);
    const double CONSTANT_AS *eyes = cams + sizeof(BatchView::cam) / sizeof(double);
    for (int i = threadIdx.x; i < frames * kLdsCameraDoubles; i += blockDim.x)
    {
        const int b = i / kLdsCameraDoubles, j = i - b * kLdsCameraDoubles;
        const double CONSTANT_AS *c = cams + b * 15;
        p.cam[i] = j < 12 ? c[j] : (j == 12 ? -c[12] : c[6 + (j - 13)] * -c[12]);
    }
    if (grids.path_enabled)
        for (int i = threadIdx.x; i < frames * 2 * TRT_RAYFAMILY_DOUBLES; i += blockDim.x)
            p.eye[i] = eyes[i];
    __syncthreads();
    return image_view(p);
}

#ifndef TRT_COMPACT_BLOCK
#define TRT_COMPACT_BLOCK 1024
#endif
constexpr int kCompactBlock = TRT_COMPACT_BLOCK;
constexpr int kBigBlock = 1024;

template <bool COUNT, bool REFRACT = false, bool COMPACT = false, bool PATCHES = false, bool BIG = false, bool DEVICE_IMAGE = false, bool BATCH = false,
          class... BatchArgument>
__global__ __launch_bounds__(BIG ? kBigBlock : COMPACT ? kCompactBlock : kPersistentBlock, ((COMPACT && !COUNT) || BIG) ? 4 : TRT_ROUNDS_WAVES) void render_rounds_kernel(SceneView s, CullView cull, FrameView f, GridView grids, BatchArgument... batch)
{
    static_assert(sizeof...(BatchArgument) == (BATCH ? 1 : 0), "a BATCH launch has one more argument, a BatchView; the others none");
    static_assert(!BATCH || (!COUNT && !REFRACT && !BIG && !DEVICE_IMAGE), "several frames per launch: the plain, patch and decoupled rounds");
    static_assert(!(REFRACT && COMPACT), "the refraction extension runs on the plain rounds");
    static_assert(!(PATCHES && COMPACT), "scenes with patches run the plain rounds");
    static_assert(!BIG || (PATCHES && !COUNT && !REFRACT && !COMPACT), "1024-thread workgroups: the shipping patch instantiation only");
    static_assert(!DEVICE_IMAGE || (!REFRACT && !COMPACT && !BIG), "the device-memory image: the plain rounds only");
    extern __shared__ __attribute__((aligned(16))) double lds[];
    const LdsImage L = BATCH ? stage_lds_image_batch(lds, s, cull, f, grids)
                       : DEVICE_IMAGE ? image_view(image_layout(const_cast<double *>(f.image), s.num_spheres, s.num_dir, s.num_point, cull.padded, f.spp))
                                      : stage_lds_image(lds, s, cull, f, grids);
    const int n = s.num_spheres, nd = s.num_dir, nl = s.num_dir + s.num_point;
    const int lane = threadIdx.x & 63;
    const unsigned pixels_here = (unsigned)f.local_rows * (unsigned)f.width;
    const unsigned total = pixels_here * (unsigned)f.spp;
    (void)total;
    const d3 gp = load3(s.ground), gn = load3(s.ground + 3);

    bool alive = true;
    bool want_unit = true;
    unsigned slot_id = 0;
    d3 sample = d3{0.0, 0.0, 0.0};
    double weight = 1.0, weight_sum = 0.0;
    int bounces = 0;
    d3 o = d3{0.0, 0.0, 0.0}, d = d3{0.0, 0.0, -1.0};
    d3 next_dir = d;
    int fam = 0;
    int inside = -1;
    Tally tally;
    unsigned pool_next = 0, pool_end = 0;
    {
        const unsigned group = blockIdx.x, waves = blockDim.x >> 6, wave = (unsigned)__builtin_amdgcn_readfirstlane((int)(threadIdx.x >> 6));
        const unsigned j = (group >> f.queue_shift) * waves + wave;
        pool_next = ((j << f.queue_shift) + (group & ((1u << f.queue_shift) - 1u))) * f.chunk;
        pool_end = pool_next + f.chunk;
    }
    double *const ring = lds + f.ring_at + (unsigned)__builtin_amdgcn_readfirstlane((int)(threadIdx.x >> 6)) * kRingDoubles;
    unsigned short *const ring_mat = (unsigned short *)(ring + 7 * kRingTasks);
    double *const parked = ring + 7 * kRingTasks + kRingTasks / 4;
    if (COMPACT)
    {
        for (int i = lane; i < kRingDoubles; i += 64)
            ring[i] = 0.0;
        __builtin_amdgcn_fence(__ATOMIC_SEQ_CST, "wavefront");
// ... 399 lines not shown
```

terminalraytracer_amd/csrc/trt_tables.hip:

```cpp
#include "trt_context.hpp"

using namespace trt_impl;

namespace
{

__global__ void build_dirgrid_kernel(const trt_dirgrid_disc *discs, int n, int g, int slabs, int words, unsigned long long *masks)
{
    const long cell = (long)blockIdx.x * blockDim.x + threadIdx.x;
    if (cell >= (long)slabs * g * g)
        return;
    const int c = (int)(cell % g), j = (int)((cell / g) % g), slab = (int)(cell / ((long)g * g));
    for (int w = 0; w < words; w++)
    {
        unsigned long long m = 0;
        for (int b = 0; b < 64 && w * 64 + b < n; b++)
            if (trt_dirgrid_in_slab(discs + w * 64 + b, slab) && trt_dirgrid_reaches(discs + w * 64 + b, c, j))
                m |= 0x8000000000000000ull >> b;
        masks[cell * words + w] = m;
    }
}

__global__ void build_pointgrid_kernel(const trt_pointgrid_cone *cones, int n, int g, int shells, int words, unsigned long long *masks)
{
    const long cell = (long)blockIdx.x * blockDim.x + threadIdx.x;
    if (cell >= 6L * shells * g * g)
        return;
    const int shell = (int)(cell / (6L * g * g)), face = (int)((cell / ((long)g * g)) % 6), j = (int)((cell / g) % g), c = (int)(cell % g);
    for (int w = 0; w < words; w++)
    {
        unsigned long long m = 0;
        for (int b = 0; b < 64 && w * 64 + b < n; b++)
            if (trt_pointgrid_in_shell(cones + w * 64 + b, shell, shells) && trt_pointgrid_reaches(cones + w * 64 + b, face, c, j, g))
                m |= 0x8000000000000000ull >> b;
        masks[cell * words + w] = m;
    }
}

__device__ unsigned long long pack_cell(const unsigned long long *mask, int words, unsigned long long *pool, unsigned long long *pool_used,
                                        unsigned pool_limit, int bits, bool valid = true)
{
    const int count = valid ? trt_list_count(mask, words) : 0;
    const unsigned need = valid ? trt_list_pool_words(count, bits) : 0u;
    const int lane = (int)(threadIdx.x & 63);
    unsigned upto = need;
#pragma unroll
    for (int d = 1; d < 64; d <<= 1)
    {
        const unsigned below = __shfl_up(upto, d);
        upto += lane >= d ? below : 0u;
    }
    const unsigned total = __shfl(upto, 63);
    unsigned long long base = 0;
    if (total)
    {
        if (lane == 63)
            base = atomicAdd(pool_used, (unsigned long long)total);
        base = __shfl(base, 63);
    }
    if (!valid)
        return 0ull;
    if (need == 0)
        return trt_list_pack(mask, words, count, nullptr, 0u, bits);
    const unsigned long long at = base + (upto - need);
    if (count > 0xffff || at + need > (unsigned long long)pool_limit)
        return (unsigned long long)TRT_LIST_NONE << 56;
    return trt_list_pack(mask, words, count, pool, (unsigned)at, bits);
}

__global__ void set_pool_counter_kernel(unsigned long long *counter, unsigned long long value) { *counter = value; }

__global__ void pack_lists_kernel(const unsigned long long *masks, long cells, int words, unsigned long long *lists, unsigned long long *pool,
                                  unsigned long long *pool_used, unsigned pool_limit, int bits)
{
    const long cell = (long)blockIdx.x * blockDim.x + threadIdx.x;
    const bool valid = cell < cells;
    const unsigned long long packed = pack_cell(masks + (valid ? cell : 0) * words, words, pool, pool_used, pool_limit, bits, valid);
    if (valid)
        lists[cell] = packed;
}

static_assert(TRT_FAMILY_TILE * TRT_FAMILY_TILE == 64, "a tile per wave");
constexpr int kSceneTilesPerBlock = 16;
unsigned family_grid_blocks(int g, int tiles_per_block)
{
    const unsigned cells = 6u * (unsigned)g * (unsigned)g;
    return trt_family_tiled(g) ? (cells / 64u + (unsigned)tiles_per_block - 1u) / (unsigned)tiles_per_block : (cells + 255u) / 256u;
}

template <int kWords>
constexpr size_t family_lds_bytes()
{
    return sizeof(trt_pointgrid_cone) * 64 * kWords + sizeof(unsigned long long) * kWords + sizeof(unsigned long long) * 4 * 64 * kWords;
}

template <int kWords>
__global__ __launch_bounds__(256) void build_family_lists_kernel(const double *spheres, int n, const trt_rayfamily *families, trt_rayfamily f0,
                                                                 trt_rayfamily f1, int by_value, int g, unsigned long long *lists,
                                                                 unsigned long long *pool, unsigned long long *pool_used, unsigned pool_limit,
                                                                 int tiles_per_block)
{
    extern __shared__ __attribute__((aligned(16))) unsigned char family_lds[];
    trt_pointgrid_cone *const cones = (trt_pointgrid_cone *)family_lds;
    unsigned long long *const reach = (unsigned long long *)(cones + 64 * kWords);
    unsigned long long(*const part)[64][kWords] = (unsigned long long(*)[64][kWords])(reach + kWords);
    const int bits = kWords > 4 ? 16 : 8;
    const trt_rayfamily F = by_value ? (blockIdx.y == 0 ? f0 : f1) : families[blockIdx.y];
    for (int i = threadIdx.x; i < n; i += blockDim.x)
        trt_rayfamily_cone(&F, spheres + 9 * i, &cones[i]);
    __syncthreads();
    const unsigned cells = 6u * (unsigned)g * (unsigned)g;
    const int words = (n + 63) / 64 > 0 ? (n + 63) / 64 : 1;
    if (!trt_family_tiled(g))
    {
        const unsigned cell = blockIdx.x * blockDim.x + threadIdx.x;
        const bool valid = cell < cells;
        const int face = (int)(cell / ((unsigned)g * (unsigned)g)), j = (int)((cell / (unsigned)g) % (unsigned)g), c = (int)(cell % (unsigned)g);
        unsigned long long m[kWords];
#pragma unroll
        for (int w = 0; w < kWords; w++)
            m[w] = 0;
        for (int i = 0; valid && i < n; i++)
            if (trt_pointgrid_reaches(&cones[i], face, c, j, g))
                m[i >> 6] |= 0x8000000000000000ull >> (i & 63);
        const unsigned long long packed = pack_cell(m, words, pool, pool_used, pool_limit, bits, valid);
        if (valid)
            lists[(size_t)blockIdx.y * cells + cell] = packed;
        return;
    }
    const unsigned gt = (unsigned)g / TRT_FAMILY_TILE, tiles = 6u * gt * gt;
    const int lane = (int)(threadIdx.x & 63), q = (int)(threadIdx.x >> 6);
    for (unsigned tile = blockIdx.x * (unsigned)tiles_per_block; tile < tiles && tile < (blockIdx.x + 1u) * (unsigned)tiles_per_block; tile++)
    {
        const int face = (int)(tile / (gt * gt)), tj = (int)((tile / gt) % gt), tc = (int)(tile % gt);
        __syncthreads();
#pragma unroll
        for (int chunk = 0; chunk < kWords / 4; chunk++)
        {
            const int i = 256 * chunk + (int)threadIdx.x;
            const bool reaches = i < n && trt_pointgrid_reaches(&cones[i], face, tc, tj, (int)gt);
            const unsigned long long word = __ballot(reaches);
            if (lane == 0)
                reach[4 * chunk + q] = word;
        }
        __syncthreads();
        const int j = tj * TRT_FAMILY_TILE + lane / TRT_FAMILY_TILE, c = tc * TRT_FAMILY_TILE + lane % TRT_FAMILY_TILE;
#pragma unroll
        for (int w = 0; w < kWords; w++)
        {
            unsigned long long m = 0;
            unsigned long long todo = 64 * w < n ? reach[w] & (0x1111111111111111ull << q) : 0ull;
            while (todo)
            {
                const int k = __builtin_ctzll(todo);
                todo &= todo - 1;
                if (trt_pointgrid_reaches(&cones[64 * w + k], face, c, j, g))
                    m |= 0x8000000000000000ull >> k;
            }
            part[q][lane][w] = m;
        }
        __syncthreads();
        if (q == 0)
        {
            unsigned long long m[kWords];
#pragma unroll
            for (int w = 0; w < kWords; w++)
                m[w] = part[0][lane][w] | part[1][lane][w] | part[2][lane][w] | part[3][lane][w];
            const unsigned cell = ((unsigned)face * (unsigned)g + (unsigned)j) * (unsigned)g + (unsigned)c;
            lists[(size_t)blockIdx.y * cells + cell] = pack_cell(m, words, pool, pool_used, pool_limit, bits);
        }
    }
}

void launch_family_builder(int n, dim3 grid, hipStream_t stream, const double *spheres, const trt_rayfamily *families, trt_rayfamily f0, trt_rayfamily f1,
                           int by_value, int g, unsigned long long *lists, unsigned long long *pool, unsigned long long *pool_used, unsigned pool_limit,
                           int tiles_per_block)
{
    if (n <= TRT_LIST_MAX_SPHERES)
        hipLaunchKernelGGL(build_family_lists_kernel<4>, grid, dim3(256), family_lds_bytes<4>(), stream, spheres, n, families, f0, f1, by_value, g, lists, pool,
                           pool_used, pool_limit, tiles_per_block);
    else
        hipLaunchKernelGGL(build_family_lists_kernel<TRT_PATH_MAX_SPHERES / 64>, grid, dim3(256), family_lds_bytes<TRT_PATH_MAX_SPHERES / 64>(), stream, spheres, n,
                           families, f0, f1, by_value, g, lists, pool, pool_used, pool_limit, tiles_per_block);
}

}

namespace trt_impl
{

void allow_large_lds_tables(const trt_context *ctx)
{
    (void)hipFuncSetAttribute((const void *)build_family_lists_kernel<TRT_PATH_MAX_SPHERES / 64>, hipFuncAttributeMaxDynamicSharedMemorySize, ctx->lds_limit);
}

static int build_light_grids(trt_context *ctx, const trt_cull_scene &cs)
{
    const int n = (int)(ctx->T->h_spheres.size() / 9), nd = (int)(ctx->T->h_dir.size() / 6), np = (int)(ctx->T->h_point.size() / 7);
    const int gd = ctx->dirgrid_cells, gp = ctx->pointgrid_cells, sd = std::max(ctx->dirgrid_slabs, 1), sp = std::max(ctx->pointgrid_shells, 1);
    trt::GridView &g = ctx->grids;
    g.enabled = 0;
    ctx->T->grids_built_for[0] = gd;
    ctx->T->grids_built_for[1] = gp;
    ctx->T->grids_built_for[2] = ctx->dirgrid_slabs;
    ctx->T->grids_built_for[3] = ctx->pointgrid_shells;
    if (gd < 8 || gp < 2 || nd + np == 0 || n > TRT_LIST_MAX_SPHERES_WIDE)
        return TRT_OK;
    const int bits = n > TRT_LIST_MAX_SPHERES ? 16 : 8;
    g.list_bits = bits;
    const size_t words = (size_t)std::max((n + 63) / 64, 1), slots = (size_t)std::max(n, 1);
    const size_t dir_stride = (size_t)sd * gd * gd * words, point_stride = 6 * (size_t)sp * gp * gp * words;
    std::vector<trt_dirgrid> dg(nd);
    std::vector<trt_pointgrid> pg(np);
    std::vector<trt_dirgrid_disc> discs(slots * nd);
    std::vector<trt_pointgrid_cone> cones(slots * np);
    for (int i = 0; i < nd; i++)
    {
        const double *li = ctx->T->h_dir.data() + 6 * i;
        const double to_light[3] = {-li[0], -li[1], -li[2]};
        const double len2 = to_light[0] * to_light[0] + to_light[1] * to_light[1] + to_light[2] * to_light[2];
        if (!(len2 > 0.0) || !(len2 < 1e300))
            return TRT_OK;
        trt_dirgrid_prepare(ctx->T->h_spheres.data(), n, &cs, to_light, gd, sd, &dg[i], discs.data() + slots * i);
    }
    for (int i = 0; i < np; i++)
        trt_pointgrid_prepare(ctx->T->h_spheres.data(), n, &cs, ctx->T->h_point.data() + 7 * i, gp, sp, &pg[i], cones.data() + slots * i);
    HIP_TRY(ctx->T->d_dir_masks.reserve(dir_stride * nd));
    HIP_TRY(ctx->T->d_point_masks.reserve(point_stride * np));
    HIP_TRY(ctx->T->d_dirgrids.reserve(nd));
    HIP_TRY(ctx->T->d_pointgrids.reserve(np));
    HIP_TRY(ctx->T->d_discs.reserve(discs.size()));
    HIP_TRY(ctx->T->d_cones.reserve(cones.size()));
    if (nd)
    {
        HIP_TRY(hipMemcpy(ctx->T->d_dirgrids.ptr, dg.data(), dg.size() * sizeof(trt_dirgrid), hipMemcpyHostToDevice));
        HIP_TRY(hipMemcpy(ctx->T->d_discs.ptr, discs.data(), discs.size() * sizeof(trt_dirgrid_disc), hipMemcpyHostToDevice));
    }
    if (np)
    {
        HIP_TRY(hipMemcpy(ctx->T->d_pointgrids.ptr, pg.data(), pg.size() * sizeof(trt_pointgrid), hipMemcpyHostToDevice));
        HIP_TRY(hipMemcpy(ctx->T->d_cones.ptr, cones.data(), cones.size() * sizeof(trt_pointgrid_cone), hipMemcpyHostToDevice));
    }
    const int block = 256;
    for (int i = 0; i < nd; i++)
        hipLaunchKernelGGL(build_dirgrid_kernel, dim3((unsigned)(((size_t)sd * gd * gd + block - 1) / block)), dim3(block), 0, ctx->stream,
                           ctx->T->d_discs.ptr + slots * i, n, gd, sd, (int)words, ctx->T->d_dir_masks.ptr + dir_stride * i);
    for (int i = 0; i < np; i++)
        hipLaunchKernelGGL(build_pointgrid_kernel, dim3((unsigned)((6 * (size_t)sp * gp * gp + block - 1) / block)), dim3(block), 0, ctx->stream,
                           ctx->T->d_cones.ptr + slots * i, n, gp, sp, (int)words, ctx->T->d_point_masks.ptr + point_stride * i);
    const size_t dir_cells = (size_t)sd * gd * gd, point_cells = 6 * (size_t)sp * gp * gp;
    HIP_TRY(ctx->T->d_dir_lists.reserve(dir_cells * nd));
    HIP_TRY(ctx->T->d_point_lists.reserve(point_cells * np));
    HIP_TRY(hipMemsetAsync(ctx->T->d_dir_lists.ptr, 0xFF, std::max<size_t>(dir_cells * nd, 1) * sizeof(unsigned long long), ctx->stream));
    HIP_TRY(hipMemsetAsync(ctx->T->d_point_lists.ptr, 0xFF, std::max<size_t>(point_cells * np, 1) * sizeof(unsigned long long), ctx->stream));
    if (nd)
        hipLaunchKernelGGL(pack_lists_kernel, dim3((unsigned)((dir_cells * nd + block - 1) / block)), dim3(block), 0, ctx->stream, ctx->T->d_dir_masks.ptr,
                           (long)(dir_cells * nd), (int)words, ctx->T->d_dir_lists.ptr, ctx->T->d_pool.ptr, ctx->T->d_pool_used.ptr, (unsigned)ctx->T->pool_scene_words, bits);
    if (np)
        hipLaunchKernelGGL(pack_lists_kernel, dim3((unsigned)((point_cells * np + block - 1) / block)), dim3(block), 0, ctx->stream, ctx->T->d_point_masks.ptr,
                           (long)(point_cells * np), (int)words, ctx->T->d_point_lists.ptr, ctx->T->d_pool.ptr, ctx->T->d_pool_used.ptr, (unsigned)ctx->T->pool_scene_words, bits);
    HIP_TRY(hipGetLastError());
    HIP_TRY(hipStreamSynchronize(ctx->stream));
    g.dir = ctx->T->d_dirgrids.ptr;
    g.point = ctx->T->d_pointgrids.ptr;
    g.dir_lists = ctx->T->d_dir_lists.ptr;
    g.point_lists = ctx->T->d_point_lists.ptr;
    g.dir_stride = (unsigned)dir_cells;
    g.point_stride = (unsigned)point_cells;
    g.pool = ctx->T->d_pool.ptr;
    g.enabled = 1;
    return TRT_OK;
}

constexpr unsigned long long kAutoPatchBudgetBytes = 4ull << 30;
int patches_for(const trt_context *ctx, int n)
{
    if (ctx->path_patches >= 0)
        return std::min(ctx->path_patches, TRT_PATCH_MAX_M);
    if (ctx->moving_scene)
        return 0;
    int m = n >= TRT_PATCHES_FROM_SPHERES ? 2 : 0;
    const unsigned long long per_table = 6ull * (unsigned long long)ctx->path_g_sph * (unsigned long long)ctx->path_g_sph;
    while (m > 0 && 2ull * (unsigned long long)n * (6ull * m * m) * per_table * 12ull > kAutoPatchBudgetBytes)
        m--;
    return m;
}

static int build_path_tables(trt_context *ctx, const trt_cull_scene &cs, const double *ground)
{
    const int n = (int)(ctx->T->h_spheres.size() / 9);
    trt::GridView &g = ctx->grids;
    g.path_enabled = 0;
    g.patch_m = g.patch_count = 0;
    invalidate_eye_tables(ctx);
    ctx->T->path_built_for[0] = ctx->path_g_eye;
    ctx->T->path_built_for[1] = ctx->path_g_sph;
    ctx->T->path_built_for[2] = ctx->path_min_spheres;
    ctx->T->path_built_for[3] = ctx->path_patches;
    ctx->T->cull_scene = cs;
    memcpy(ctx->T->ground_built, ground, sizeof ctx->T->ground_built);
    const int ge = ctx->path_g_eye, gs = ctx->path_g_sph;
    if (ge < 2 || gs < 2 || n > TRT_PATH_MAX_SPHERES || n < ctx->path_min_spheres)
        return TRT_OK;
    trt_patchset patches;
    trt_patchset_init(&patches, patches_for(ctx, n));
    const size_t P = (size_t)patches.count, families = 2 * (size_t)n * P;
    const size_t eye_cells = 6 * (size_t)ge * ge, sph_cells = 6 * (size_t)gs * gs;
    const size_t eye_part = (size_t)kEyeSlots * 2 * eye_cells;
    if (eye_part + families * sph_cells >= 0xffffffffull)
        return fail(TRT_ERR_CAPACITY, "path tables of %zu families x %zu cells", families, sph_cells);
    HIP_TRY(ctx->T->d_path_lists.reserve(eye_part + families * sph_cells));
    HIP_TRY(hipMemsetAsync(ctx->T->d_path_lists.ptr, 0xFF, (eye_part + families * sph_cells) * sizeof(unsigned long long), ctx->stream));
    HIP_TRY(ctx->T->d_families.reserve(std::max<size_t>(families, 1)));
    HIP_TRY(ctx->T->d_sphere_fam.reserve(4 * (size_t)std::max(n, 1)));
    HIP_TRY(ctx->T->d_patch_rec.reserve(P * TRT_PATCH_RECORD));
    std::vector<trt_rayfamily> fam(std::max<size_t>(families, 1));
    std::vector<double> rec(4 * (size_t)std::max(n, 1)), prec(P * TRT_PATCH_RECORD);
    trt_family_consts consts;
    trt_sphere_families(ctx->T->h_spheres.data(), n, ground, &cs, &patches, fam.data(), rec.data(), &consts);
    trt_patch_records(&patches, ground, prec.data());
    HIP_TRY(hipMemcpy(ctx->T->d_patch_rec.ptr, prec.data(), prec.size() * sizeof(double), hipMemcpyHostToDevice));
    if (n)
    {
        HIP_TRY(hipMemcpy(ctx->T->d_families.ptr, fam.data(), families * sizeof(trt_rayfamily), hipMemcpyHostToDevice));
        HIP_TRY(hipMemcpy(ctx->T->d_sphere_fam.ptr, rec.data(), 4 * (size_t)n * sizeof(double), hipMemcpyHostToDevice));
        for (size_t first = 0; first < families; first += 32768)
        {
            const unsigned batch = (unsigned)std::min<size_t>(32768, families - first);
            launch_family_builder(n, dim3(family_grid_blocks(gs, kSceneTilesPerBlock), batch), ctx->stream, (const double *)ctx->T->d_spheres.ptr,
                                  (const trt_rayfamily *)ctx->T->d_families.ptr + first, trt_rayfamily{}, trt_rayfamily{}, 0, gs,
                                  ctx->T->d_path_lists.ptr + eye_part + first * sph_cells, ctx->T->d_pool.ptr, ctx->T->d_pool_used.ptr, (unsigned)ctx->T->pool_scene_words,
                                  kSceneTilesPerBlock);
        }
        HIP_TRY(hipGetLastError());
        HIP_TRY(hipStreamSynchronize(ctx->stream));
    }
    g.path_lists = ctx->T->d_path_lists.ptr;
    g.eye_at = (unsigned)((size_t)ctx->eye_slot * 2 * eye_cells);
    g.sph_at = (unsigned)eye_part;
    g.pool = ctx->T->d_pool.ptr;
    g.sphere_fam = ctx->T->d_sphere_fam.ptr;
    g.patch_rec = ctx->T->d_patch_rec.ptr;
    g.patch_m = patches.m;
    g.patch_count = patches.count;
    g.rg2_sph = consts.rg * consts.rg;
    g.slack0 = consts.slack;
    g.g_eye = ge;
    g.g_sph = gs;
    g.path_enabled = 1;
    return TRT_OK;
}

int build_tables(trt_context *ctx, const trt_cull_scene &cs, const double *ground)
{
    ctx->table_builds++;
    const size_t n = ctx->T->h_spheres.size() / 9, nd = ctx->T->h_dir.size() / 6, np = ctx->T->h_point.size() / 7;
    const size_t gd = (size_t)ctx->dirgrid_cells, gp = (size_t)ctx->pointgrid_cells, ge = (size_t)ctx->path_g_eye, gs = (size_t)ctx->path_g_sph;
    const size_t sd = (size_t)std::max(ctx->dirgrid_slabs, 1), sp = (size_t)std::max(ctx->pointgrid_shells, 1);
    const int m = patches_for(ctx, (int)n);
    const size_t sphere_cells = 2 * n * (m ? 6 * (size_t)m * m : 1) * 6 * gs * gs;
    const size_t wide = n > TRT_LIST_MAX_SPHERES ? 2 : 1, sphere_part = n > TRT_PATH_MAX_SPHERES ? 0 : (m ? sphere_cells / 2 : sphere_cells);
    ctx->T->pool_scene_words = std::max<size_t>(1024, wide * (nd * sd * gd * gd + np * 6 * sp * gp * gp + sphere_part));
    const size_t per_word = wide == 2 ? 4 : 8;
    ctx->T->pool_eye_words = std::max<size_t>(1024, 2 * 6 * ge * ge * std::min<size_t>((n + per_word - 1) / per_word, 64));
    if (ctx->list_pool_cap)
    {
        ctx->T->pool_scene_words = std::min(ctx->T->pool_scene_words, std::max<size_t>(ctx->list_pool_cap, 1));
        ctx->T->pool_eye_words = std::min(ctx->T->pool_eye_words, std::max<size_t>(ctx->list_pool_cap, 1));
    }
    const double t0 = host_seconds();
    int rc = TRT_OK;
    for (int pass = 0; pass < 2 && !rc; pass++)
    {
        if (ctx->T->pool_scene_words + kEyeSlots * ctx->T->pool_eye_words >= 0xffffffffull)
            return fail(TRT_ERR_CAPACITY, "candidate tables too large");
        ctx->grids = trt::GridView{};
        ctx->grids.list_bits = n > TRT_LIST_MAX_SPHERES ? 16 : 8;
        HIP_TRY(ctx->T->d_pool.reserve(ctx->T->pool_scene_words + kEyeSlots * ctx->T->pool_eye_words));
        HIP_TRY(ctx->T->d_pool_used.reserve(16 * (1 + kEyeSlots)));
        HIP_TRY(hipMemsetAsync(ctx->T->d_pool_used.ptr, 0, 16 * (1 + kEyeSlots) * sizeof(unsigned long long), ctx->stream));
        rc = build_light_grids(ctx, cs);
        if (!rc)
            rc = build_path_tables(ctx, cs, ground);
        if (rc || ctx->list_pool_cap)
            break;
        unsigned long long asked = 0;
        HIP_TRY(hipMemcpyAsync(&asked, ctx->T->d_pool_used.ptr, sizeof asked, hipMemcpyDeviceToHost, ctx->stream));
        HIP_TRY(hipStreamSynchronize(ctx->stream));
        if (asked <= ctx->T->pool_scene_words)
            break;
        ctx->T->pool_scene_words = (size_t)asked + 1024;
    }
    ctx->T->build_seconds = host_seconds() - t0;
    return rc;
}

static int build_eye_slot(trt_context *ctx, const trt_rayfamily *families, int slot, hipStream_t stream)
{
    const trt::GridView &g = ctx->grids;
    const int n = (int)(ctx->T->h_spheres.size() / 9), ge = g.g_eye;
    const size_t eye_cells = 6 * (size_t)ge * ge;
    const size_t pool_from = ctx->T->pool_scene_words + (size_t)slot * ctx->T->pool_eye_words;
    unsigned long long *const counter = ctx->T->d_pool_used.ptr + 16 * (1 + slot);
    hipLaunchKernelGGL(set_pool_counter_kernel, dim3(1), dim3(1), 0, stream, counter, (unsigned long long)pool_from);
    launch_family_builder(n, dim3(family_grid_blocks(ge, 1), 2u), stream, (const double *)ctx->T->d_spheres.ptr, (const trt_rayfamily *)nullptr, families[0], families[1], 1,
                          ge, ctx->T->d_path_lists.ptr + (size_t)slot * 2 * eye_cells, ctx->T->d_pool.ptr, counter, (unsigned)(pool_from + ctx->T->pool_eye_words), 1);
    HIP_TRY(hipGetLastError());
    return TRT_OK;
}

int ensure_eye_tables(trt_context *ctx, const Camera *camera, hipStream_t stream, int slot)
{
    trt::GridView &g = ctx->grids;
    if (!g.path_enabled)
        return TRT_OK;
    if (slot < 0)
        slot = ctx->eye_slot;
    trt_context::EyeSlot &built = ctx->eye_slots[slot];
    const double eye[3] = {camera->frame.origin.x, camera->frame.origin.y, camera->frame.origin.z};
    if (built.valid && !memcmp(eye, built.eye, sizeof eye))
        return TRT_OK;
    built.valid = false;
    trt_eye_families(eye, ctx->T->ground_built, &ctx->T->cull_scene, built.families);
    if (slot == ctx->eye_slot)
        g.eye[0] = built.families[0], g.eye[1] = built.families[1];
    const int rc = build_eye_slot(ctx, built.families, slot, stream);
    if (rc)
        return rc;
    memcpy(built.eye, eye, sizeof eye);
    built.valid = true;
    return TRT_OK;
}

}
```

terminalraytracer_amd/hip.py:

```python
import ctypes as C
import functools
import os

import numpy as np

from . import layout as L

_HERE = os.path.dirname(os.path.abspath(__file__))
LIB_PATH = os.environ.get("TRT_HIP_LIB") or os.path.join(_HERE, "libtrt_hip.so")

TRT_OK = 0
ERRORS = {-1: "TRT_ERR_HIP", -2: "TRT_ERR_ARGUMENT", -3: "TRT_ERR_NO_SCENE", -4: "TRT_ERR_CAPACITY",
          -5: "TRT_ERR_NOT_INITIALISED"}


class TrtError(RuntimeError):
    def __init__(self, code, message):
        super().__init__(f"{ERRORS.get(code, code)}: {message}")
        self.code = code


class RowSet(C.Structure):
    _fields_ = [("width", C.c_int), ("height", C.c_int), ("tile_rows", C.c_int), ("tile_first", C.c_int),
                ("tile_step", C.c_int)]

    @staticmethod
    def whole(width, height):
        return RowSet(width, height, height, 0, 1)

    @staticmethod
    def shard(width, height, rank, world, tile_rows=8):
        return RowSet(width, height, tile_rows, rank, world)


_VP, _I, _SZ = C.c_void_p, C.c_int, C.c_size_t
SYMBOLS = {
    "project_scene": (None, [C.POINTER(L.Scene), C.POINTER(L.Screen)]),
    "trt_render_frame": (_I, [C.POINTER(L.Scene), C.POINTER(L.Screen), _I, _I]),
    "render_frame": (_I, [C.POINTER(L.Scene), C.POINTER(L.Screen), _I, _I]),
    "trt_render_frame_rgb8": (_I, [C.POINTER(L.Scene), _I, _I, _I, _I, _VP]),
    "trt_render_frame_ansi": (_I, [C.POINTER(L.Scene), _I, _I, _I, _I, _VP]),
    "trt_render_frame_ansi_half": (_I, [C.POINTER(L.Scene), _I, _I, _I, _I, _VP]),
    "trt_render_frame_ansi_delta": (_I, [C.POINTER(L.Scene), _I, _I, _I, _I, _VP, _SZ, C.POINTER(_SZ)]),
    "trt_init": (_I, [_I]),
    "trt_shutdown": (_I, []),
    "trt_upload_skybox": (_I, [C.POINTER(L.Skybox)]),
    "trt_invalidate_skybox": (_I, []),
    "trt_rowset_rows": (_I, [C.POINTER(RowSet)]),
    "trt_rowset_frame_row": (_I, [C.POINTER(RowSet), _I]),
    "trt_create": (_I, [_I, C.POINTER(_VP)]),
    "trt_destroy": (_I, [_VP]),
    "trt_set_stream": (_I, [_VP, _VP]),
    "trt_set_scene": (_I, [_VP, C.POINTER(L.Scene)]),
    "trt_render_device": (_I, [_VP, C.POINTER(L.Camera), C.POINTER(RowSet), _I, _I, _VP, _SZ]),
    "trt_render_device_rgb8": (_I, [_VP, C.POINTER(L.Camera), C.POINTER(RowSet), _I, _I, _VP, _SZ]),
    "trt_quantize_device": (_I, [_VP, _VP, _SZ, _VP]),
    "trt_ansi_bytes": (_SZ, [_I, _I]),
    "trt_render_device_ansi": (_I, [_VP, C.POINTER(L.Camera), C.POINTER(RowSet), _I, _I, _VP, _SZ]),
    "trt_ansi_from_rgb8_device": (_I, [_VP, _VP, _I, _I, _VP]),
    "trt_ansi_half_bytes": (_SZ, [_I, _I]),
    "trt_render_device_ansi_half": (_I, [_VP, C.POINTER(L.Camera), C.POINTER(RowSet), _I, _I, _VP, _SZ]),
    "trt_ansi_half_from_rgb8_device": (_I, [_VP, _VP, _I, _I, _VP]),
    "trt_render_host_ansi_half": (_I, [_VP, C.POINTER(L.Camera), C.POINTER(RowSet), _I, _I, _VP]),
    "trt_render_device_batch_ansi_half": (_I, [_VP, _VP, _I, C.POINTER(RowSet), _I, _I, _VP, _SZ]),
    "trt_render_host_batch_ansi_half": (_I, [_VP, _VP, _I, C.POINTER(RowSet), _I, _I, _VP]),
    "trt_render_frame_ansi_delta_half": (_I, [C.POINTER(L.Scene), _I, _I, _I, _I, _VP, _SZ, C.POINTER(_SZ)]),
    "trt_ansi_delta_half_capacity": (_SZ, [_I, _I]),
    "trt_ansi_delta_half_from_rgb8_device": (_I, [_VP, _VP, _VP, _I, _I, _VP, _SZ, _VP]),
    "trt_ansi_delta_half_kernel_times": (_I, [_VP, _VP, _VP, _I, _I, _VP, _SZ, _VP, C.POINTER(C.c_float)]),
    "trt_render_device_ansi_delta_half": (_I, [_VP, C.POINTER(L.Camera), C.POINTER(RowSet), _I, _I, _VP, _SZ, _VP]),
    "trt_render_host_ansi_delta_half": (_I, [_VP, C.POINTER(L.Camera), C.POINTER(RowSet), _I, _I, _VP, _SZ, C.POINTER(_SZ)]),
    "trt_ansi_delta_capacity": (_SZ, [_I, _I]),
    "trt_ansi_delta_from_rgb8_device": (_I, [_VP, _VP, _VP, _I, _I, _VP, _SZ, _VP]),
    "trt_ansi_delta_kernel_times": (_I, [_VP, _VP, _VP, _I, _I, _VP, _SZ, _VP, C.POINTER(C.c_float)]),
    "trt_render_device_ansi_delta": (_I, [_VP, C.POINTER(L.Camera), C.POINTER(RowSet), _I, _I, _VP, _SZ, _VP]),
    "trt_render_host_ansi_delta": (_I, [_VP, C.POINTER(L.Camera), C.POINTER(RowSet), _I, _I, _VP, _SZ, C.POINTER(_SZ)]),
    "trt_ansi_delta_reset": (_I, [_VP]),
    "trt_render_host": (_I, [_VP, C.POINTER(L.Camera), C.POINTER(RowSet), _I, _I, _VP]),
    "trt_render_host_rgb8": (_I, [_VP, C.POINTER(L.Camera), C.POINTER(RowSet), _I, _I, _VP]),
    "trt_render_host_ansi": (_I, [_VP, C.POINTER(L.Camera), C.POINTER(RowSet), _I, _I, _VP]),
    "trt_render_device_batch": (_I, [_VP, _VP, _I, C.POINTER(RowSet), _I, _I, _VP, _SZ]),
    "trt_render_host_batch": (_I, [_VP, _VP, _I, C.POINTER(RowSet), _I, _I, _VP]),
    "trt_render_device_batch_rgb8": (_I, [_VP, _VP, _I, C.POINTER(RowSet), _I, _I, _VP, _SZ]),
    "trt_render_host_batch_rgb8": (_I, [_VP, _VP, _I, C.POINTER(RowSet), _I, _I, _VP]),
    "trt_render_device_batch_ansi": (_I, [_VP, _VP, _I, C.POINTER(RowSet), _I, _I, _VP, _SZ]),
    "trt_render_host_batch_ansi": (_I, [_VP, _VP, _I, C.POINTER(RowSet), _I, _I, _VP]),
    "trt_batch_info": (_I, [_VP, C.POINTER(_I), C.POINTER(_I)]),
    "trt_synchronize": (_I, [_VP]),
    "trt_kernel_times": (_I, [_VP, C.POINTER(C.c_float), _I]),
    "trt_render_kernel_times": (_I, [_VP, C.POINTER(C.c_float), C.POINTER(C.c_float), _I]),
    "trt_enable_counters": (_I, [_VP, _I]),
    "trt_read_counters": (_I, [_VP, C.POINTER(C.c_ulonglong), C.POINTER(C.c_ulonglong)]),
    "trt_read_diagnostics": (_I, [_VP, C.POINTER(C.c_ulonglong), C.POINTER(C.c_ulonglong)]),
    "trt_set_kernel": (_I, [_VP, _I]),
    "trt_set_light_grids": (_I, [_VP, _I, _I]),
    "trt_set_light_slabs": (_I, [_VP, _I, _I]),
    "trt_share_scene": (_I, [_VP, _VP]),
    "trt_set_scene_policy": (_I, [_I, _I]),
    "trt_scene_is_moving": (_I, []),
    "trt_scene_info": (_I, [_VP, C.POINTER(C.c_ulonglong), C.POINTER(_I), C.POINTER(C.c_double)]),
    "trt_set_list_pool_words": (_I, [_VP, C.c_size_t]),
    "trt_set_path_grids": (_I, [_VP, _I, _I]),
    "trt_set_path_grids_min_spheres": (_I, [_VP, _I]),
    "trt_set_path_patches": (_I, [_VP, _I]),
    "trt_get_path_patches": (_I, [_VP, C.POINTER(_I), C.POINTER(_I)]),
    "trt_path_family_code": (_I, [_VP, _I, _I, _VP]),
    "trt_set_compaction": (_I, [_VP, _I]),
    "trt_render_variant": (_I, [_VP, C.POINTER(_I), C.POINTER(_I)]),
    "trt_set_scene_image": (_I, [_VP, _I]),
    "trt_render_image": (_I, [_VP, C.POINTER(_I), C.POINTER(C.c_ulonglong)]),
    "trt_set_scratch_fill": (_I, [_VP, _I]),
    "trt_default_context": (_VP, []),
    "trt_build_counts": (_I, [_VP, C.POINTER(C.c_ulonglong), C.POINTER(C.c_ulonglong)]),
    "trt_read_path_tables": (C.c_long, [_VP, C.POINTER(L.Camera), _VP, C.c_size_t, _VP, C.c_size_t, C.POINTER(C.c_long)]),
    "trt_read_sweep_fallbacks": (_I, [_VP, C.POINTER(C.c_ulonglong)]),
    "trt_read_shading_passes": (_I, [_VP, C.POINTER(C.c_ulonglong)]),
    "trt_read_loop_diagnostics": (_I, [_VP, C.POINTER(C.c_ulonglong)]),
    "trt_set_refraction": (_I, [_VP, _VP, _I]),
    "trt_reserve_cus": (_I, [_VP, _I]),
    "trt_get_stream": (_I, [_VP, C.POINTER(C.c_void_p)]),
    "trt_selftest_cube": (_I, [_VP, _VP, C.c_size_t, _VP, _VP]),
    "trt_selftest_unit": (_I, [_VP, _VP, C.c_size_t, _VP, _VP]),
    "trt_selftest_sky": (_I, [_VP, _VP, C.c_size_t, _I, _VP, _VP, _VP]),
    "trt_read_light_grid": (C.c_long, [_VP, _I, _I, _VP, C.c_size_t]),
    "trt_read_light_lists": (C.c_long, [_VP, _I, _I, _VP, C.c_size_t, _VP, C.c_size_t, C.POINTER(C.c_long)]),
    "trt_kernel_info": (_I, [_VP] + [C.POINTER(_I)] * 5),
    "trt_selftest_div_sqrt": (_I, [_VP, _VP, _VP, _SZ, _VP, _VP]),
    "trt_probe_rays": (_I, [_VP, _VP, _SZ, _VP, _VP, _VP, _VP, _VP]),
    "trt_probe_rays_production": (_I, [_VP, C.POINTER(L.Camera), _VP, _VP, _SZ, _VP, _VP, _VP, _VP, _VP]),
    "trt_launch_count": (C.c_long, [_VP]),
    "trt_launch_span_ms": (_I, [_VP, C.c_long, _VP, C.c_long, C.POINTER(C.c_float)]),
    "trt_dist_unique_id": (_I, [_VP]),
    "trt_dist_frame_times": (_I, [_VP, C.POINTER(C.c_float), C.POINTER(C.c_float)]),
    "trt_dist_allow_rccl_override": (_I, [_I]),
    "trt_dist_rccl_library": (C.c_char_p, []),
    "trt_dist_comm_ranks": (_I, [_VP]),
    "trt_dist_create": (_I, [_I, C.POINTER(L.Scene), _VP, _I, _I, _I, _I, _I, _I, _I, C.POINTER(_VP)]),
    "trt_dist_set_scene": (_I, [_VP, C.POINTER(L.Scene)]),
    "trt_dist_render": (_I, [_VP, C.POINTER(L.Camera), _I, _I, C.POINTER(_VP)]),
    "trt_dist_synchronize": (_I, [_VP]),
    "trt_dist_enable_rgb8": (_I, [_VP]),
    "trt_dist_render_rgb8": (_I, [_VP, C.POINTER(L.Camera), _I, _I, C.POINTER(_VP)]),
    "trt_dist_fetch_rgb8": (_I, [_VP, _VP, _VP]),
    "trt_dist_fetch": (_I, [_VP, _VP, _VP]),
    "trt_dist_source_rows": (_I, [_I, _I, _I, _I, C.POINTER(_I)]),
    "trt_dist_info": (_I, [_VP] + [C.POINTER(_I)] * 5),
    "trt_dist_context": (_VP, [_VP, _I]),
    "trt_dist_destroy": (_I, [_VP]),
    "trt_dist_last_error": (C.c_char_p, []),
    "trt_last_error": (C.c_char_p, []),
    "trt_version": (C.c_char_p, []),
}


@functools.lru_cache(maxsize=None)
def lib():
    if not os.path.exists(LIB_PATH):
        raise ImportError(f"{LIB_PATH} is missing: build it with `make lib` (hipcc --offload-arch=gfx950). "
                          "There is no fallback path.")
    try:
        import torch
    except ImportError:
        pass
    dll = C.CDLL(LIB_PATH)
    for name, (res, args) in SYMBOLS.items():
        fn = getattr(dll, name)
        fn.restype = res
        fn.argtypes = args
    return dll


def _check(code):
    if code != TRT_OK:
        raise TrtError(code, lib().trt_last_error().decode())


def camera_struct(camera_array):
    cam = L.Camera()
    a = np.ascontiguousarray(camera_array, dtype=np.float64).reshape(15)
    C.memmove(C.byref(cam), a.ctypes.data, 120)
    return cam


class Context:

    PRODUCTION, REFERENCE_ORDER = 0, 1

    def __init__(self, device=0, _borrowed=None):
        self._owned = _borrowed is None
        if self._owned:
            self._h = _VP()
            _check(lib().trt_create(device, C.byref(self._h)))
        else:
            self._h = _VP(_borrowed)
        self.device = device

    def close(self):
        if self._h and self._owned:
            lib().trt_destroy(self._h)
        self._h = _VP()

    def __enter__(self):
        return self

    def __exit__(self, *exc):
        self.close()

    def __del__(self):
        try:
            self.close()
        except Exception:
            pass

    def set_stream(self, stream_handle):
        _check(lib().trt_set_stream(self._h, _VP(stream_handle or 0)))

    def set_scene(self, scene_data):
        scene = scene_data.as_scene()
        _check(lib().trt_set_scene(self._h, C.byref(scene)))

    def set_kernel(self, which):
        _check(lib().trt_set_kernel(self._h, which))

    def reserve_cus(self, reserved):
        _check(lib().trt_reserve_cus(self._h, reserved))

    def stream_ptr(self):
        p = C.c_void_p()
        _check(lib().trt_get_stream(self._h, C.byref(p)))
        return p.value or 0

    def set_light_grids(self, directional_cells, point_cells):
        _check(lib().trt_set_light_grids(self._h, directional_cells, point_cells))

    def share_scene(self, source):
        _check(lib().trt_share_scene(self._h, source._h))

    def scene_info(self):
        b, n, t = C.c_ulonglong(), _I(), C.c_double()
        _check(lib().trt_scene_info(self._h, C.byref(b), C.byref(n), C.byref(t)))
        return {"table_bytes": b.value, "sharers": n.value, "build_seconds": t.value}

    def set_list_pool_words(self, words):
        _check(lib().trt_set_list_pool_words(self._h, words))

    def set_light_slabs(self, directional_slabs, point_shells):
        _check(lib().trt_set_light_slabs(self._h, directional_slabs, point_shells))

    def set_path_grids(self, eye_cells, sphere_cells):
        _check(lib().trt_set_path_grids(self._h, eye_cells, sphere_cells))

    def set_path_patches(self, m):
        _check(lib().trt_set_path_patches(self._h, m))

    def path_patches(self):
        m, p = _I(), _I()
        _check(lib().trt_get_path_patches(self._h, C.byref(m), C.byref(p)))
        return m.value, p.value

    def family_codes(self, families, rays, num_spheres):
        families = np.asarray(families, dtype=np.int32)
        rays = np.ascontiguousarray(rays, dtype=np.float64).reshape(-1, 6)
        out = families.copy()
        n = num_spheres
        for j in np.nonzero(families >= 2 + n)[0]:
            s = int(families[j]) - 2 - n
            assert j > 0 and families[j - 1] == 2 + s, "a mirror ray's parent must precede it"
            parent = np.ascontiguousarray(rays[j - 1, :3])
            out[j] = lib().trt_path_family_code(self._h, 3, s, parent.ctypes.data)
        return out

    def set_path_grids_min_spheres(self, min_spheres):
        _check(lib().trt_set_path_grids_min_spheres(self._h, min_spheres))

    def set_compaction(self, mode):
        _check(lib().trt_set_compaction(self._h, mode))

    def render_variant(self):
        d, t = _I(), _I()
        _check(lib().trt_render_variant(self._h, C.byref(d), C.byref(t)))
        return {"decoupled": bool(d.value), "workgroup_threads": t.value}

    def set_scene_image(self, mode):
        _check(lib().trt_set_scene_image(self._h, mode))

    def render_image(self):
        d, b = _I(), C.c_ulonglong()
        _check(lib().trt_render_image(self._h, C.byref(d), C.byref(b)))
        return {"in_device_memory": bool(d.value), "image_bytes": b.value}

    def build_counts(self):
        b, u = C.c_ulonglong(), C.c_ulonglong()
        _check(lib().trt_build_counts(self._h, C.byref(b), C.byref(u)))
        return b.value, u.value

    def set_scratch_fill(self, on=True):
        _check(lib().trt_set_scratch_fill(self._h, 1 if on else 0))

    def read_path_tables(self, camera_array):
        cam = camera_struct(camera_array)
        info = (C.c_long * 8)()
        probe = np.zeros(1, dtype=np.uint64)
        lib().trt_read_path_tables(self._h, C.byref(cam), probe.ctypes.data, 0, probe.ctypes.data, 0, info)
        cells = np.zeros(max(1, info[4]), dtype=np.uint64)
        pool = np.zeros(max(1, info[7]), dtype=np.uint64)
        got = lib().trt_read_path_tables(self._h, C.byref(cam), cells.ctypes.data, cells.size, pool.ctypes.data, pool.size, info)
        if got < 0:
            _check(int(got))
        keys = ("enabled", "eye_cells", "sphere_cells", "spheres", "cells", "pool_used_scene", "pool_used_eye", "pool_capacity")
        return dict(zip(keys, [int(x) for x in info])), cells[:got], pool

    def set_refraction(self, ior=None):
        if ior is None:
            _check(lib().trt_set_refraction(self._h, None, 0))
        else:
            a = np.ascontiguousarray(ior, dtype=np.float64)
            _check(lib().trt_set_refraction(self._h, a.ctypes.data, a.size))

    def read_sweep_fallbacks(self):
        v = C.c_ulonglong()
        _check(lib().trt_read_sweep_fallbacks(self._h, C.byref(v)))
        return v.value

    def selftest_unit(self, xyzw):
        v = np.ascontiguousarray(xyzw, dtype=np.float64).reshape(-1, 4)
        fast, ref = np.zeros_like(v), np.zeros_like(v)
        _check(lib().trt_selftest_unit(self._h, v.ctypes.data, v.shape[0], fast.ctypes.data, ref.ctypes.data))
        return fast, ref

    def selftest_cube(self, xyz):
        v = np.ascontiguousarray(xyz, dtype=np.float32).reshape(-1, 3)
        dev, host = np.zeros((v.shape[0], 4), dtype=np.float32), np.zeros((v.shape[0], 4), dtype=np.float32)
        _check(lib().trt_selftest_cube(self._h, v.ctypes.data, v.shape[0], dev.ctypes.data, host.ctypes.data))
        return dev, host

    def selftest_sky(self, dirs, dim):
        v = np.ascontiguousarray(dirs, dtype=np.float64).reshape(-1, 3)
        exact, est = np.zeros(v.shape[0], dtype=np.int64), np.zeros(v.shape[0], dtype=np.int64)
        amb = np.zeros(v.shape[0], dtype=np.int32)
        _check(lib().trt_selftest_sky(self._h, v.ctypes.data, v.shape[0], int(dim), exact.ctypes.data, est.ctypes.data, amb.ctypes.data))
        return exact, est, amb

    def read_light_grid(self, point_light, index, words):
        out = np.zeros(words, dtype=np.uint64)
        got = lib().trt_read_light_grid(self._h, int(point_light), index, out.ctypes.data, words)
        if got < 0:
            _check(int(got))
        return out[:got]

    def read_light_lists(self, point_light, index):
        info = (C.c_long * 4)()
        got = lib().trt_read_light_lists(self._h, int(point_light), index, None, 0, None, 0, info)
        if got < 0:
            _check(int(got))
        cells = np.zeros(max(1, info[0]), dtype=np.uint64)
        pool = np.zeros(max(1, info[2]), dtype=np.uint64)
        got = lib().trt_read_light_lists(self._h, int(point_light), index, cells.ctypes.data, cells.size, pool.ctypes.data, pool.size, info)
        if got < 0:
            _check(int(got))
        return dict(zip(("cells", "list_bits", "pool_words", "enabled"), [int(x) for x in info])), cells[:got], pool

    def render_device(self, camera_array, rows, bounce_limit, rays_per_pixel, device_ptr, capacity_bytes):
        cam = camera_struct(camera_array)
        _check(lib().trt_render_device(self._h, C.byref(cam), C.byref(rows), bounce_limit, rays_per_pixel,
                                       _VP(device_ptr), capacity_bytes))

    def render_device_rgb8(self, camera_array, rows, bounce_limit, rays_per_pixel, device_ptr, capacity_bytes):
        cam = camera_struct(camera_array)
        _check(lib().trt_render_device_rgb8(self._h, C.byref(cam), C.byref(rows), bounce_limit, rays_per_pixel,
                                            _VP(device_ptr), capacity_bytes))

    def quantize_device(self, device_ptr, num_pixels, rgb_ptr):
        _check(lib().trt_quantize_device(self._h, _VP(device_ptr), num_pixels, _VP(rgb_ptr)))

    def render_host(self, camera_array, rows, bounce_limit, rays_per_pixel):
        n = lib().trt_rowset_rows(C.byref(rows))
        out = np.zeros((n, rows.width, 3), dtype=np.float64)
        cam = camera_struct(camera_array)
        _check(lib().trt_render_host(self._h, C.byref(cam), C.byref(rows), bounce_limit, rays_per_pixel,
                                     out.ctypes.data))
        return out

    def render_host_rgb8(self, camera_array, rows, bounce_limit, rays_per_pixel):
        n = lib().trt_rowset_rows(C.byref(rows))
        out = np.zeros((n, rows.width, 3), dtype=np.uint8)
        cam = camera_struct(camera_array)
        _check(lib().trt_render_host_rgb8(self._h, C.byref(cam), C.byref(rows), bounce_limit, rays_per_pixel, out.ctypes.data))
        return out

    def render_device_ansi(self, camera_array, rows, bounce_limit, rays_per_pixel, device_ptr, capacity_bytes):
        cam = camera_struct(camera_array)
        _check(lib().trt_render_device_ansi(self._h, C.byref(cam), C.byref(rows), bounce_limit, rays_per_pixel,
                                            _VP(device_ptr), capacity_bytes))

    def render_host_ansi(self, camera_array, rows, bounce_limit, rays_per_pixel):
        out = np.zeros(ansi_bytes(rows.width, lib().trt_rowset_rows(C.byref(rows))), dtype=np.uint8)
        cam = camera_struct(camera_array)
        _check(lib().trt_render_host_ansi(self._h, C.byref(cam), C.byref(rows), bounce_limit, rays_per_pixel, out.ctypes.data))
        return out

    def ansi_from_rgb8(self, rgb_ptr, width, rows, text_ptr):
        _check(lib().trt_ansi_from_rgb8_device(self._h, _VP(rgb_ptr), width, rows, _VP(text_ptr)))

    def render_device_ansi_half(self, camera_array, rows, bounce_limit, rays_per_pixel, device_ptr, capacity_bytes):
        cam = camera_struct(camera_array)
        _check(lib().trt_render_device_ansi_half(self._h, C.byref(cam), C.byref(rows), bounce_limit, rays_per_pixel,
                                                 _VP(device_ptr), capacity_bytes))

    def render_host_ansi_half(self, camera_array, rows, bounce_limit, rays_per_pixel):
        out = np.zeros(ansi_half_bytes(rows.width, lib().trt_rowset_rows(C.byref(rows))), dtype=np.uint8)
        cam = camera_struct(camera_array)
        _check(lib().trt_render_host_ansi_half(self._h, C.byref(cam), C.byref(rows), bounce_limit, rays_per_pixel, out.ctypes.data))
        return out

    def ansi_half_from_rgb8(self, rgb_ptr, width, rows, text_ptr):
        _check(lib().trt_ansi_half_from_rgb8_device(self._h, _VP(rgb_ptr), width, rows, _VP(text_ptr)))


    def _delta_from_rgb8(self, entry, shown_ptr, next_ptr, width, rows, text_ptr, capacity_bytes, bytes_ptr):
        _check(getattr(lib(), entry)(self._h, _VP(shown_ptr), _VP(next_ptr), width, rows, _VP(text_ptr), capacity_bytes, _VP(bytes_ptr)))

    def _delta_kernel_times(self, entry, shown_ptr, next_ptr, width, rows, text_ptr, capacity_bytes, bytes_ptr):
        ms = (C.c_float * 3)()
        _check(getattr(lib(), entry)(self._h, _VP(shown_ptr), _VP(next_ptr), width, rows, _VP(text_ptr), capacity_bytes, _VP(bytes_ptr), ms))
        return tuple(ms)

    def _render_device_delta(self, entry, camera_array, rows, bounce_limit, rays_per_pixel, device_ptr, capacity_bytes, bytes_ptr):
        cam = camera_struct(camera_array)
        _check(getattr(lib(), entry)(self._h, C.byref(cam), C.byref(rows), bounce_limit, rays_per_pixel, _VP(device_ptr), capacity_bytes, _VP(bytes_ptr)))

    def _render_host_delta(self, entry, capacity, camera_array, rows, bounce_limit, rays_per_pixel, out):
        if out is None:
            out = np.empty(capacity(rows.width, lib().trt_rowset_rows(C.byref(rows))), dtype=np.uint8)
        n = _SZ(0)
        cam = camera_struct(camera_array)
        _check(getattr(lib(), entry)(self._h, C.byref(cam), C.byref(rows), bounce_limit, rays_per_pixel, out.ctypes.data, out.size, C.byref(n)))
        return out[:n.value]

    def ansi_delta_from_rgb8(self, shown_ptr, next_ptr, width, rows, text_ptr, capacity_bytes, bytes_ptr):
        self._delta_from_rgb8("trt_ansi_delta_from_rgb8_device", shown_ptr, next_ptr, width, rows, text_ptr, capacity_bytes, bytes_ptr)

    def ansi_delta_kernel_times(self, shown_ptr, next_ptr, width, rows, text_ptr, capacity_bytes, bytes_ptr):
        return self._delta_kernel_times("trt_ansi_delta_kernel_times", shown_ptr, next_ptr, width, rows, text_ptr, capacity_bytes, bytes_ptr)

    def render_device_ansi_delta(self, camera_array, rows, bounce_limit, rays_per_pixel, device_ptr, capacity_bytes, bytes_ptr):
        self._render_device_delta("trt_render_device_ansi_delta", camera_array, rows, bounce_limit, rays_per_pixel, device_ptr, capacity_bytes, bytes_ptr)

    def render_host_ansi_delta(self, camera_array, rows, bounce_limit, rays_per_pixel, out=None):
        return self._render_host_delta("trt_render_host_ansi_delta", ansi_delta_capacity, camera_array, rows, bounce_limit, rays_per_pixel, out)

    def ansi_delta_reset(self):
        _check(lib().trt_ansi_delta_reset(self._h))

    def ansi_delta_half_from_rgb8(self, shown_ptr, next_ptr, width, rows, text_ptr, capacity_bytes, bytes_ptr):
        self._delta_from_rgb8("trt_ansi_delta_half_from_rgb8_device", shown_ptr, next_ptr, width, rows, text_ptr, capacity_bytes, bytes_ptr)

    def ansi_delta_half_kernel_times(self, shown_ptr, next_ptr, width, rows, text_ptr, capacity_bytes, bytes_ptr):
        return self._delta_kernel_times("trt_ansi_delta_half_kernel_times", shown_ptr, next_ptr, width, rows, text_ptr, capacity_bytes, bytes_ptr)

    def render_device_ansi_delta_half(self, camera_array, rows, bounce_limit, rays_per_pixel, device_ptr, capacity_bytes, bytes_ptr):
        self._render_device_delta("trt_render_device_ansi_delta_half", camera_array, rows, bounce_limit, rays_per_pixel, device_ptr, capacity_bytes, bytes_ptr)

    def render_host_ansi_delta_half(self, camera_array, rows, bounce_limit, rays_per_pixel, out=None):
        return self._render_host_delta("trt_render_host_ansi_delta_half", ansi_delta_half_capacity, camera_array, rows, bounce_limit, rays_per_pixel, out)

    @staticmethod
    def _camera_batch(cameras):
        cams = np.ascontiguousarray(cameras, dtype=np.float64)
        if cams.ndim != 2 or cams.shape[1] != 15:
            raise ValueError("cameras: float64 [n, 15] (Camera, TRT.c:178-184)")
        return cams

    def render_device_batch(self, cameras, rows, bounce_limit, rays_per_pixel, device_ptr, capacity_bytes):
        cams = self._camera_batch(cameras)
        _check(lib().trt_render_device_batch(self._h, cams.ctypes.data, cams.shape[0], C.byref(rows), bounce_limit, rays_per_pixel,
                                             _VP(device_ptr), capacity_bytes))

    def render_host_batch(self, cameras, rows, bounce_limit, rays_per_pixel):
        cams = self._camera_batch(cameras)
        out = np.zeros((cams.shape[0], lib().trt_rowset_rows(C.byref(rows)), rows.width, 3), dtype=np.float64)
        _check(lib().trt_render_host_batch(self._h, cams.ctypes.data, cams.shape[0], C.byref(rows), bounce_limit, rays_per_pixel,
                                           out.ctypes.data))
        return out

    def render_batch_rgb8(self, cameras, rows, bounce_limit, rays_per_pixel, device_ptr, capacity_bytes):
        cams = self._camera_batch(cameras)
        _check(lib().trt_render_device_batch_rgb8(self._h, cams.ctypes.data, cams.shape[0], C.byref(rows), bounce_limit, rays_per_pixel,
                                                  _VP(device_ptr), capacity_bytes))

    def render_host_batch_rgb8(self, cameras, rows, bounce_limit, rays_per_pixel):
        cams = self._camera_batch(cameras)
        out = np.zeros((cams.shape[0], lib().trt_rowset_rows(C.byref(rows)), rows.width, 3), dtype=np.uint8)
        _check(lib().trt_render_host_batch_rgb8(self._h, cams.ctypes.data, cams.shape[0], C.byref(rows), bounce_limit, rays_per_pixel,
                                                out.ctypes.data))
        return out

    def render_batch_ansi(self, cameras, rows, bounce_limit, rays_per_pixel, device_ptr, capacity_bytes):
        cams = self._camera_batch(cameras)
        _check(lib().trt_render_device_batch_ansi(self._h, cams.ctypes.data, cams.shape[0], C.byref(rows), bounce_limit, rays_per_pixel,
                                                  _VP(device_ptr), capacity_bytes))

    def render_host_batch_ansi(self, cameras, rows, bounce_limit, rays_per_pixel):
        cams = self._camera_batch(cameras)
        out = np.zeros((cams.shape[0], ansi_bytes(rows.width, lib().trt_rowset_rows(C.byref(rows)))), dtype=np.uint8)
        _check(lib().trt_render_host_batch_ansi(self._h, cams.ctypes.data, cams.shape[0], C.byref(rows), bounce_limit, rays_per_pixel,
                                                out.ctypes.data))
        return out

    def render_batch_ansi_half(self, cameras, rows, bounce_limit, rays_per_pixel, device_ptr, capacity_bytes):
        cams = self._camera_batch(cameras)
        _check(lib().trt_render_device_batch_ansi_half(self._h, cams.ctypes.data, cams.shape[0], C.byref(rows), bounce_limit, rays_per_pixel,
                                                       _VP(device_ptr), capacity_bytes))

    def render_host_batch_ansi_half(self, cameras, rows, bounce_limit, rays_per_pixel):
        cams = self._camera_batch(cameras)
        out = np.zeros((cams.shape[0], ansi_half_bytes(rows.width, lib().trt_rowset_rows(C.byref(rows)))), dtype=np.uint8)
        _check(lib().trt_render_host_batch_ansi_half(self._h, cams.ctypes.data, cams.shape[0], C.byref(rows), bounce_limit, rays_per_pixel,
                                                     out.ctypes.data))
        return out

    def batch_info(self):
        n, k = _I(), _I()
        _check(lib().trt_batch_info(self._h, C.byref(n), C.byref(k)))
        return n.value, k.value

    def synchronize(self):
        _check(lib().trt_synchronize(self._h))

    def kernel_times(self, max_count=256):
        buf = (C.c_float * max_count)()
        n = lib().trt_kernel_times(self._h, buf, max_count)
        if n < 0:
            _check(n)
        return [buf[i] for i in range(n)]

    def render_kernel_times(self, max_count=256):
        a, b = (C.c_float * max_count)(), (C.c_float * max_count)()
        n = lib().trt_render_kernel_times(self._h, a, b, max_count)
        if n < 0:
            _check(n)
        return [a[i] for i in range(n)], [b[i] for i in range(n)]

    def launch_count(self):
        return int(lib().trt_launch_count(self._h))

    def launch_span_ms(self, first_launch, last, last_launch):
        ms = C.c_float()
        _check(lib().trt_launch_span_ms(self._h, first_launch, last._h, last_launch, C.byref(ms)))
        return float(ms.value)

    def enable_counters(self, on=True):
        _check(lib().trt_enable_counters(self._h, 1 if on else 0))

    def read_counters(self):
        p, s = C.c_ulonglong(), C.c_ulonglong()
        _check(lib().trt_read_counters(self._h, C.byref(p), C.byref(s)))
        return p.value, s.value

    def read_diagnostics(self):
        t, p = C.c_ulonglong(), C.c_ulonglong()
        _check(lib().trt_read_diagnostics(self._h, C.byref(t), C.byref(p)))
        v = C.c_ulonglong()
        _check(lib().trt_read_shading_passes(self._h, C.byref(v)))
        loops = (C.c_ulonglong * 8)()
        _check(lib().trt_read_loop_diagnostics(self._h, loops))
        kinds = ("path", "directional", "point")
        return {"wave_loop_trips": t.value, "phase2_rounds": p.value, "swept_traces": self.read_sweep_fallbacks(), "shading_passes": v.value,
                "exact_loop_iterations": {k: int(loops[i]) for i, k in enumerate(kinds)},
                "exact_loop_lane_activity": {k: round(loops[3 + i] / max(1, 64 * loops[i]), 4) for i, k in enumerate(kinds)},
                "point_light_closest_hit_fallbacks": int(loops[6])}

    def kernel_info(self):
        v = [_I() for _ in range(5)]
        _check(lib().trt_kernel_info(self._h, *[C.byref(x) for x in v]))
        return dict(zip(("vgprs", "sgprs", "static_lds_bytes", "max_blocks_per_cu", "compute_units"),
                        [x.value for x in v]))

    def selftest_div_sqrt(self, a, b):
        a = np.ascontiguousarray(a, dtype=np.float64)
        b = np.ascontiguousarray(b, dtype=np.float64)
        q, r = np.empty_like(a), np.empty_like(a)
        _check(lib().trt_selftest_div_sqrt(self._h, a.ctypes.data, b.ctypes.data, a.size, q.ctypes.data, r.ctypes.data))
        return q, r

    def probe_rays(self, rays):
        rays = np.ascontiguousarray(rays, dtype=np.float64).reshape(-1, 6)
        n = rays.shape[0]
        obj = np.zeros(n, dtype=np.int32)
        point, normal, material, lit = np.zeros((n, 3)), np.zeros((n, 3)), np.zeros((n, 5)), np.zeros((n, 3))
        _check(lib().trt_probe_rays(self._h, rays.ctypes.data, n, obj.ctypes.data, point.ctypes.data,
                                    normal.ctypes.data, material.ctypes.data, lit.ctypes.data))
        return obj, point, normal, material, lit


    def probe_rays_production(self, camera_array, rays, families=None):
        rays = np.ascontiguousarray(rays, dtype=np.float64).reshape(-1, 6)
        n = rays.shape[0]
        fam = None if families is None else np.ascontiguousarray(families, dtype=np.int32)
        obj = np.zeros(n, dtype=np.int32)
        point, normal, material, lit = np.zeros((n, 3)), np.zeros((n, 3)), np.zeros((n, 5)), np.zeros((n, 3))
        cam = camera_struct(camera_array)
        _check(lib().trt_probe_rays_production(self._h, C.byref(cam), rays.ctypes.data, None if fam is None else fam.ctypes.data, n,
                                               obj.ctypes.data, point.ctypes.data, normal.ctypes.data, material.ctypes.data, lit.ctypes.data))
        return obj, point, normal, material, lit


def default_context():
    h = lib().trt_default_context()
    return Context(0, _borrowed=h) if h else None


def render_frame(scene_data, width, height, bounce_limit=10, rays_per_pixel=10, symbol="trt_render_frame"):
    from .scenes import new_screen
    scene = scene_data.as_scene()
# ... 178 lines not shown
```

Baseline: 37.34 billion.

## Add lean sphere path lists that drop the emitting sphere for outward rays

Builds a second copy of the per-sphere path-grid candidate lists with the owning sphere removed, using a new device kernel that repacks each cell into the shared pool. When a secondary ray leaves a sphere outward and is not inside it, path_cell looks up the lean twin, so the traversal skips a pointless self-intersection test. The twins are on by default for static scenes within a memory budget, and the pool is enlarged to hold them. This costs extra table memory, build time and one more dot product per lookup.

```diff
diff --git a/include/trt_hip_diag.h b/include/trt_hip_diag.h
--- a/include/trt_hip_diag.h
+++ b/include/trt_hip_diag.h
@@ -19,6 +19,10 @@
 
 long trt_read_path_tables(trt_context *ctx, const Camera *camera, unsigned long long *cells, size_t capacity_cells,
                           unsigned long long *pool, size_t capacity_pool, long info[8]);
+
+int trt_set_path_lean_lists(trt_context *ctx, int mode);
+int trt_get_path_lean_lists(trt_context *ctx, int *in_use, unsigned long long *twin_bytes);
+long trt_read_path_lean_tables(trt_context *ctx, unsigned long long *cells, size_t capacity_cells);
 
 int trt_read_sweep_fallbacks(trt_context *ctx, unsigned long long *swept_traces);
 
diff --git a/terminalraytracer_amd/csrc/trt_capi.hip b/terminalraytracer_amd/csrc/trt_capi.hip
--- a/terminalraytracer_amd/csrc/trt_capi.hip
+++ b/terminalraytracer_amd/csrc/trt_capi.hip
@@ -121,6 +121,7 @@
                       ctx->T->grids_built_for[2] == ctx->dirgrid_slabs && ctx->T->grids_built_for[3] == ctx->pointgrid_shells &&
                       ctx->T->path_built_for[0] == ctx->path_g_eye && ctx->T->path_built_for[1] == ctx->path_g_sph &&
                       ctx->T->path_built_for[2] == ctx->path_min_spheres && ctx->T->path_built_for[3] == ctx->path_patches &&
+                      ctx->T->path_built_for[4] == lean_lists_wanted(ctx) &&
                       !memcmp(ctx->T->ground_built, &scene->ground, sizeof ctx->T->ground_built);
     if (!same)
     {
@@ -219,6 +220,12 @@
         int mode = -1;
         if (sscanf(e, "%d", &mode) == 1 && mode >= -1 && mode <= 1)
             ctx->compaction = mode;
+    }
+    if (const char *e = getenv("TRT_PATH_LEAN"))
+    {
+        int mode = -1;
+        if (sscanf(e, "%d", &mode) == 1 && mode >= -1 && mode <= 1)
+            ctx->path_lean = mode;
     }
     HIP_TRY(ctx->own_stream.create());
     ctx->stream = ctx->own_stream;
@@ -353,7 +360,7 @@
     dst->dirgrid_cells = src->dirgrid_cells, dst->pointgrid_cells = src->pointgrid_cells;
     dst->dirgrid_slabs = src->dirgrid_slabs, dst->pointgrid_shells = src->pointgrid_shells;
     dst->path_g_eye = src->path_g_eye, dst->path_g_sph = src->path_g_sph, dst->path_min_spheres = src->path_min_spheres;
-    dst->path_patches = src->path_patches, dst->list_pool_cap = src->list_pool_cap;
+    dst->path_patches = src->path_patches, dst->list_pool_cap = src->list_pool_cap, dst->path_lean = src->path_lean;
     memcpy(dst->sky_faces, src->sky_faces, sizeof dst->sky_faces);
     dst->sky_dim = src->sky_dim;
     dst->sky_stamp = src->sky_stamp;
@@ -507,6 +514,51 @@
     return rc ? rc : refresh_occupancy(ctx);
 }
 
+extern "C" int trt_set_path_lean_lists(trt_context *ctx, int mode)
+{
+    if (!ctx || mode < -1 || mode > 1)
+        return fail(TRT_ERR_ARGUMENT, "lean lists %d", mode);
+    HIP_TRY(hipSetDevice(ctx->device));
+    HIP_TRY(hipStreamSynchronize(ctx->stream));
+    const int before = ctx->path_lean;
+    ctx->path_lean = mode;
+    if (!ctx->have_scene)
+        return TRT_OK;
+    const int level = lean_lists_wanted(ctx);
+    if (level > ctx->T->path_built_for[4] && !ctx->T->lean_at)
+    {
+        if (const int shared = refuse_if_shared(ctx, "trt_set_path_lean_lists"))
+        {
+            ctx->path_lean = before;
+            return shared;
+        }
+        const int n = (int)(ctx->T->h_spheres.size() / 9);
+        std::vector<float> table((size_t)trt_cull_padded(n, trt::kCullGroup) * 4 + 4);
+        trt_cull_scene cs;
+        trt_cull_build(ctx->T->h_spheres.data(), n, trt::kCullGroup, table.data(), &cs);
+        const int rc = build_tables(ctx, cs, ctx->scene.ground);
+        return rc ? rc : refresh_occupancy(ctx);
+    }
+    if (level > ctx->T->path_built_for[4])
+        ctx->T->path_built_for[4] = level;
+    apply_lean_lists(ctx);
+    return TRT_OK;
+}
+
+extern "C" int trt_get_path_lean_lists(trt_context *ctx, int *in_use, unsigned long long *twin_bytes)
+{
+    if (!ctx)
+        return fail(TRT_ERR_ARGUMENT, "ctx is NULL");
+    const trt::GridView &g = ctx->grids;
+    if (in_use)
+        *in_use = g.path_enabled && g.lean_off != 0;
+    if (twin_bytes)
+        *twin_bytes = g.path_enabled && ctx->T->lean_at ? 8ull * (unsigned long long)ctx->T->h_spheres.size() / 9 * (unsigned long long)g.patch_count * 6ull *
+                                                              (unsigned long long)g.g_sph * (unsigned long long)g.g_sph
+                                                        : 0ull;
+    return TRT_OK;
+}
+
 extern "C" int trt_get_path_patches(trt_context *ctx, int *m, int *patches_per_sphere)
 {
     if (!ctx)
diff --git a/terminalraytracer_amd/csrc/trt_context.hpp b/terminalraytracer_amd/csrc/trt_context.hpp
--- a/terminalraytracer_amd/csrc/trt_context.hpp
+++ b/terminalraytracer_amd/csrc/trt_context.hpp
@@ -110,7 +110,8 @@
     DeviceBuffer<double> d_sphere_fam;
     DeviceBuffer<double> d_patch_rec;
     DeviceBuffer<uint32_t> d_sky;
-    int path_built_for[4] = {-1, -1, -1, -2};
+    int path_built_for[5] = {-1, -1, -1, -2, -1};
+    size_t lean_at = 0;
     int grids_built_for[4] = {-1, -1, -1, -1};
     size_t pool_scene_words = 0, pool_eye_words = 0;
     trt_cull_scene cull_scene{};
@@ -144,6 +145,7 @@
     int path_g_eye = TRT_PATHGRID_EYE, path_g_sph = TRT_PATHGRID_SPHERE;
     int path_min_spheres = TRT_PATHGRID_MIN_SPHERES;
     int path_patches = TRT_PATHGRID_PATCHES;
+    int path_lean = -1;
     size_t list_pool_cap = 0;
     int scene_changes_in_a_row = 0, scene_still_calls = 0;
     bool moving_scene = false;
@@ -275,6 +277,8 @@
 int refuse_if_shared(const trt_context *ctx, const char *what);
 extern int g_moving_after, g_still_after;
 int patches_for(const trt_context *ctx, int n);
+int lean_lists_wanted(const trt_context *ctx);
+void apply_lean_lists(trt_context *ctx);
 int build_tables(trt_context *ctx, const trt_cull_scene &cs, const double *ground);
 int ensure_eye_tables(trt_context *ctx, const Camera *camera, hipStream_t stream, int slot = -1);
 void allow_large_lds_tables(const trt_context *ctx);
diff --git a/terminalraytracer_amd/csrc/trt_diag.hip b/terminalraytracer_amd/csrc/trt_diag.hip
--- a/terminalraytracer_amd/csrc/trt_diag.hip
+++ b/terminalraytracer_amd/csrc/trt_diag.hip
@@ -111,6 +111,25 @@
     if (sph_total)
         HIP_TRY(hipMemcpy(cells + eye_total, ctx->T->d_path_lists.ptr + g.sph_at, sph_total * sizeof(unsigned long long), hipMemcpyDeviceToHost));
     HIP_TRY(hipMemcpy(pool, ctx->T->d_pool.ptr, pool_words * sizeof(unsigned long long), hipMemcpyDeviceToHost));
+    return (long)total;
+}
+
+extern "C" long trt_read_path_lean_tables(trt_context *ctx, unsigned long long *cells, size_t capacity_cells)
+{
+    if (!ctx || !cells)
+        return fail(TRT_ERR_ARGUMENT, "NULL argument");
+    if (!ctx->have_scene)
+        return fail(TRT_ERR_NO_SCENE, "no scene");
+    const trt::GridView &g = ctx->grids;
+    if (!g.path_enabled || !ctx->T->lean_at)
+        return 0;
+    const size_t total = ctx->T->h_spheres.size() / 9 * (size_t)g.patch_count * 6 * (size_t)g.g_sph * g.g_sph;
+    if (capacity_cells < total)
+        return fail(TRT_ERR_CAPACITY, "the twins have %zu cells", total);
+    HIP_TRY(hipSetDevice(ctx->device));
+    HIP_TRY(hipStreamSynchronize(ctx->stream));
+    if (total)
+        HIP_TRY(hipMemcpy(cells, ctx->T->d_path_lists.ptr + ctx->T->lean_at, total * sizeof(unsigned long long), hipMemcpyDeviceToHost));
     return (long)total;
 }
 
diff --git a/terminalraytracer_amd/csrc/trt_raygrid.h b/terminalraytracer_amd/csrc/trt_raygrid.h
--- a/terminalraytracer_amd/csrc/trt_raygrid.h
+++ b/terminalraytracer_amd/csrc/trt_raygrid.h
@@ -322,6 +322,48 @@
     return (int)((cell >> (bits * k)) & emask);
 }
 
+TRT_HD unsigned trt_list_lean_words(unsigned long long cell, const unsigned long long *pool, int own, int bits)
+{
+    const int count = trt_list_entries(cell);
+    for (int k = 0; k < count; k++)
+        if (trt_list_entry(cell, pool, k, bits) == own)
+            return trt_list_pool_words(count - 1, bits);
+    return 0u;
+}
+
+TRT_HD unsigned long long trt_list_lean(unsigned long long cell, unsigned long long *pool, int own, int bits, int has_room, unsigned pool_offset)
+{
+    const int per = 64 / bits, inline_max = 56 / bits;
+    const int count = trt_list_entries(cell);
+    int at = -1;
+    for (int k = 0; k < count && at < 0; k++)
+        if (trt_list_entry(cell, pool, k, bits) == own)
+            at = k;
+    if (at < 0)
+        return cell;
+    const int left = count - 1;
+    if (left > inline_max && !has_room)
+        return cell;
+    unsigned long long cur = left <= inline_max ? (unsigned long long)left << 56 : 0ull;
+    int k = 0;
+    for (int j = 0; j < count; j++)
+    {
+        if (j == at)
+            continue;
+        cur |= (unsigned long long)(unsigned)trt_list_entry(cell, pool, j, bits) << (bits * (k % per));
+        if (++k % per == 0 && left > inline_max)
+        {
+            pool[pool_offset + (unsigned)(k / per) - 1u] = cur;
+            cur = 0;
+        }
+    }
+    if (left <= inline_max)
+        return cur;
+    if (k % per)
+        pool[pool_offset + (unsigned)(k / per)] = cur;
+    return ((unsigned long long)TRT_LIST_POOLED << 56) | ((unsigned long long)(unsigned)left << 32) | pool_offset;
+}
+
 #define TRT_FAMILY_TILE 8
 #define TRT_LIST_MAX_SPHERES_HOST 256
 TRT_HD int trt_family_tiled(int g) { return g >= TRT_FAMILY_TILE && g % TRT_FAMILY_TILE == 0; }
diff --git a/terminalraytracer_amd/csrc/trt_rounds.hpp b/terminalraytracer_amd/csrc/trt_rounds.hpp
--- a/terminalraytracer_amd/csrc/trt_rounds.hpp
+++ b/terminalraytracer_amd/csrc/trt_rounds.hpp
@@ -39,6 +39,7 @@
     int g_eye, g_sph;
     int patch_m, patch_count;
     unsigned eye_at, sph_at;
+    unsigned lean_off;
     const unsigned long long *path_lists;
     const unsigned long long *pool;
     const double *sphere_fam;
@@ -480,7 +481,7 @@
 
 template <bool BATCH = false>
 TRT_DEV unsigned long long path_cell(const LdsImage &L, const GridView &G, int n, int fam, d3 o, d3 d, bool active, unsigned long long active_lanes,
-                                     unsigned long long &fallback_lanes, int frame = 0)
+                                     unsigned long long &fallback_lanes, int frame = 0, int inside = -1)
 {
     const bool in_family = fam >= 0;
     const unsigned long long family_lanes = lanes_with(in_family);
@@ -501,14 +502,17 @@
     const double rg2 = of_eye ? rg2_eye : G.rg2_sph;
     const d3 w = sub(o, apex);
     const d3 c = d3{w.y * d.z - w.z * d.y, w.z * d.x - w.x * d.z, w.x * d.y - w.y * d.x};
-    const bool near_line = dot(c, c) <= r_chk * r_chk, ahead = dot(w, d) >= -r_chk, in_range = dot(w, w) <= rg2;
+    const double along = dot(w, d);
+    const bool near_line = dot(c, c) <= r_chk * r_chk, ahead = along >= -r_chk, in_range = dot(w, w) <= rg2;
     const bool unit_dir = __builtin_fabs(dot(d, d) - 1.0) <= 9.094947017729282e-13;
     const bool member = near_line & ahead & in_range & unit_dir;
     const unsigned long long member_lanes = family_lanes & lanes_with(near_line) & lanes_with(ahead) & lanes_with(in_range) & lanes_with(unit_dir);
     const int g = of_eye ? G.g_eye : G.g_sph;
     const int at = trt_cubemap_cell((float)d.x, (float)d.y, (float)d.z, 0.5f * (float)g, (float)(g - 1), g);
     const unsigned eye_cells = 6u * (unsigned)G.g_eye * (unsigned)G.g_eye, sph_cells = 6u * (unsigned)G.g_sph * (unsigned)G.g_sph;
-    const unsigned base = of_eye ? G.eye_at + (BATCH ? 2u * (unsigned)frame + (unsigned)f : (unsigned)f) * eye_cells : G.sph_at + (unsigned)s * sph_cells;
+    const bool outwards = f >= 2 && !mirrored && along >= 0.0 && i != inside;
+    const unsigned base = of_eye ? G.eye_at + (BATCH ? 2u * (unsigned)frame + (unsigned)f : (unsigned)f) * eye_cells
+                                 : G.sph_at + (outwards ? G.lean_off : 0u) + (unsigned)s * sph_cells;
     unsigned long long cell = 0;
     if (has && member)
         cell = G.path_lists[base + (unsigned)at];
@@ -518,7 +522,7 @@
 
 template <bool BATCH = false>
 TRT_DEV unsigned long long path_cell_patches(const LdsImage &L, const GridView &G, int n, int &fam, d3 o, d3 d, bool active, unsigned long long active_lanes,
-                                             unsigned long long &fallback_lanes, int frame = 0)
+                                             unsigned long long &fallback_lanes, int frame = 0, int inside = -1)
 {
     const bool in_family = fam >= 0;
     const unsigned long long family_lanes = lanes_with(in_family);
@@ -530,8 +534,8 @@
     const double *at_sphere = L.sph + 4 * i, *at_mirror = L.fam + 4 * i;
     const double *src = of_eye ? L.eye + (BATCH ? frame * (2 * TRT_RAYFAMILY_DOUBLES) : 0) + TRT_RAYFAMILY_DOUBLES * (f & 1) : (mirrored ? at_mirror : at_sphere);
     const d3 base_at = load3(src);
-    const int here = trt_cubemap_cell((float)(o.x - base_at.x), (float)(o.y - base_at.y), (float)(o.z - base_at.z), 0.5f * (float)G.patch_m,
-                                      (float)(G.patch_m - 1), G.patch_m);
+    const d3 from_base = sub(o, base_at);
+    const int here = trt_cubemap_cell((float)from_base.x, (float)from_base.y, (float)from_base.z, 0.5f * (float)G.patch_m, (float)(G.patch_m - 1), G.patch_m);
     const int k = mirrored ? code & ((1 << TRT_PATCH_SHIFT) - 1) : (of_eye ? 0 : here);
     fam = !has ? -1 : (f == 0 ? 1 : (!of_eye && !mirrored ? 2 + n + (((f - 2) << TRT_PATCH_SHIFT) | k) : -1));
     const double r_abs = of_eye ? 0.0 : at_mirror[3];
@@ -554,7 +558,9 @@
     const int at = trt_cubemap_cell((float)d.x, (float)d.y, (float)d.z, 0.5f * (float)g, (float)(g - 1), g);
     const unsigned eye_cells = 6u * (unsigned)G.g_eye * (unsigned)G.g_eye, sph_cells = 6u * (unsigned)G.g_sph * (unsigned)G.g_sph;
     const unsigned table = ((mirrored ? (unsigned)n : 0u) + (unsigned)i) * (unsigned)G.patch_count + (unsigned)k;
-    const unsigned base = of_eye ? G.eye_at + (BATCH ? 2u * (unsigned)frame + (unsigned)f : (unsigned)f) * eye_cells : G.sph_at + table * sph_cells;
+    const bool outwards = !of_eye && !mirrored && dot(from_base, d) >= 0.0 && i != inside;
+    const unsigned base = of_eye ? G.eye_at + (BATCH ? 2u * (unsigned)frame + (unsigned)f : (unsigned)f) * eye_cells
+                                 : G.sph_at + (outwards ? G.lean_off : 0u) + table * sph_cells;
     unsigned long long cell = 0;
     if (has && member)
         cell = G.path_lists[base + (unsigned)at];
@@ -596,9 +602,9 @@
     {
         unsigned long long fallback_lanes;
         if constexpr (PATCHES)
-            p_cell = path_cell_patches<BATCH>(L, grids, n, fam, o, d, alive, alive_lanes, fallback_lanes, frame);
+            p_cell = path_cell_patches<BATCH>(L, grids, n, fam, o, d, alive, alive_lanes, fallback_lanes, frame, REFRACT ? inside : -1);
         else
-            p_cell = path_cell<BATCH>(L, grids, n, fam, o, d, alive, alive_lanes, fallback_lanes, frame);
+            p_cell = path_cell<BATCH>(L, grids, n, fam, o, d, alive, alive_lanes, fallback_lanes, frame, REFRACT ? inside : -1);
         p_list = fallback_lanes == 0;
     }
     if (COUNT && !p_list)
diff --git a/terminalraytracer_amd/csrc/trt_tables.hip b/terminalraytracer_amd/csrc/trt_tables.hip
--- a/terminalraytracer_amd/csrc/trt_tables.hip
+++ b/terminalraytracer_amd/csrc/trt_tables.hip
@@ -37,11 +37,8 @@
     }
 }
 
-__device__ unsigned long long pack_cell(const unsigned long long *mask, int words, unsigned long long *pool, unsigned long long *pool_used,
-                                        unsigned pool_limit, int bits, bool valid = true)
-{
-    const int count = valid ? trt_list_count(mask, words) : 0;
-    const unsigned need = valid ? trt_list_pool_words(count, bits) : 0u;
+__device__ unsigned long long take_pool_words(unsigned need, unsigned long long *pool_used)
+{
     const int lane = (int)(threadIdx.x & 63);
     unsigned upto = need;
 #pragma unroll
@@ -58,14 +55,36 @@
             base = atomicAdd(pool_used, (unsigned long long)total);
         base = __shfl(base, 63);
     }
+    return base + (upto - need);
+}
+
+__device__ unsigned long long pack_cell(const unsigned long long *mask, int words, unsigned long long *pool, unsigned long long *pool_used,
+                                        unsigned pool_limit, int bits, bool valid = true)
+{
+    const int count = valid ? trt_list_count(mask, words) : 0;
+    const unsigned need = valid ? trt_list_pool_words(count, bits) : 0u;
+    const unsigned long long at = take_pool_words(need, pool_used);
     if (!valid)
         return 0ull;
     if (need == 0)
         return trt_list_pack(mask, words, count, nullptr, 0u, bits);
-    const unsigned long long at = base + (upto - need);
     if (count > 0xffff || at + need > (unsigned long long)pool_limit)
         return (unsigned long long)TRT_LIST_NONE << 56;
     return trt_list_pack(mask, words, count, pool, (unsigned)at, bits);
+}
+
+__global__ __launch_bounds__(256) void build_lean_lists_kernel(const unsigned long long *full, unsigned long long *lean, unsigned long long cells,
+                                                               unsigned table_cells, unsigned tables_per_sphere, unsigned long long *pool,
+                                                               unsigned long long *pool_used, unsigned pool_limit, int bits)
+{
+    const unsigned long long at_cell = (unsigned long long)blockIdx.x * blockDim.x + threadIdx.x;
+    const bool valid = at_cell < cells;
+    const unsigned long long cell = valid ? full[at_cell] : 0ull;
+    const int own = (int)(at_cell / table_cells / tables_per_sphere);
+    const unsigned need = valid ? trt_list_lean_words(cell, pool, own, bits) : 0u;
+    const unsigned long long at = take_pool_words(need, pool_used);
+    if (valid)
+        lean[at_cell] = trt_list_lean(cell, pool, own, bits, at + need <= (unsigned long long)pool_limit, (unsigned)at);
 }
 
 __global__ void set_pool_counter_kernel(unsigned long long *counter, unsigned long long value) { *counter = value; }
@@ -286,6 +305,22 @@
     return m;
 }
 
+int lean_lists_wanted(const trt_context *ctx) { return ctx->path_lean > 0 ? 2 : (ctx->path_lean < 0 && !ctx->moving_scene ? 1 : 0); }
+
+static bool builds_lean_lists(const trt_context *ctx, size_t families, size_t sph_cells, size_t eye_part)
+{
+    const size_t with_twins = (families + families / 2) * sph_cells;
+    return lean_lists_wanted(ctx) && eye_part + with_twins < 0xffffffffull &&
+           (lean_lists_wanted(ctx) > 1 || (unsigned long long)with_twins * 12ull <= kAutoPatchBudgetBytes);
+}
+
+void apply_lean_lists(trt_context *ctx)
+{
+    trt::GridView &g = ctx->grids;
+    const bool on = ctx->T->lean_at != 0 && ctx->path_lean != 0;
+    g.lean_off = on ? (unsigned)ctx->T->lean_at - g.sph_at : 0u;
+}
+
 static int build_path_tables(trt_context *ctx, const trt_cull_scene &cs, const double *ground)
 {
     const int n = (int)(ctx->T->h_spheres.size() / 9);
@@ -297,6 +332,9 @@
     ctx->T->path_built_for[1] = ctx->path_g_sph;
     ctx->T->path_built_for[2] = ctx->path_min_spheres;
     ctx->T->path_built_for[3] = ctx->path_patches;
+    ctx->T->path_built_for[4] = lean_lists_wanted(ctx);
+    ctx->T->lean_at = 0;
+    g.lean_off = 0;
     ctx->T->cull_scene = cs;
     memcpy(ctx->T->ground_built, ground, sizeof ctx->T->ground_built);
     const int ge = ctx->path_g_eye, gs = ctx->path_g_sph;
@@ -307,10 +345,12 @@
     const size_t P = (size_t)patches.count, families = 2 * (size_t)n * P;
     const size_t eye_cells = 6 * (size_t)ge * ge, sph_cells = 6 * (size_t)gs * gs;
     const size_t eye_part = (size_t)kEyeSlots * 2 * eye_cells;
+    const bool lean = builds_lean_lists(ctx, families, sph_cells, eye_part);
+    const size_t lean_cells = lean ? families / 2 * sph_cells : 0;
     if (eye_part + families * sph_cells >= 0xffffffffull)
         return fail(TRT_ERR_CAPACITY, "path tables of %zu families x %zu cells", families, sph_cells);
-    HIP_TRY(ctx->T->d_path_lists.reserve(eye_part + families * sph_cells));
-    HIP_TRY(hipMemsetAsync(ctx->T->d_path_lists.ptr, 0xFF, (eye_part + families * sph_cells) * sizeof(unsigned long long), ctx->stream));
+    HIP_TRY(ctx->T->d_path_lists.reserve(eye_part + families * sph_cells + lean_cells));
+    HIP_TRY(hipMemsetAsync(ctx->T->d_path_lists.ptr, 0xFF, (eye_part + families * sph_cells + lean_cells) * sizeof(unsigned long long), ctx->stream));
     HIP_TRY(ctx->T->d_families.reserve(std::max<size_t>(families, 1)));
     HIP_TRY(ctx->T->d_sphere_fam.reserve(4 * (size_t)std::max(n, 1)));
     HIP_TRY(ctx->T->d_patch_rec.reserve(P * TRT_PATCH_RECORD));
@@ -331,6 +371,14 @@
                                   (const trt_rayfamily *)ctx->T->d_families.ptr + first, trt_rayfamily{}, trt_rayfamily{}, 0, gs,
                                   ctx->T->d_path_lists.ptr + eye_part + first * sph_cells, ctx->T->d_pool.ptr, ctx->T->d_pool_used.ptr, (unsigned)ctx->T->pool_scene_words,
                                   kSceneTilesPerBlock);
+        }
+        if (lean_cells)
+        {
+            unsigned long long *const full = ctx->T->d_path_lists.ptr + eye_part;
+            hipLaunchKernelGGL(build_lean_lists_kernel, dim3((unsigned)((lean_cells + 255) / 256)), dim3(256), 0, ctx->stream, full, full + families * sph_cells,
+                               (unsigned long long)lean_cells, (unsigned)sph_cells, (unsigned)P, ctx->T->d_pool.ptr, ctx->T->d_pool_used.ptr,
+                               (unsigned)ctx->T->pool_scene_words, g.list_bits);
+            ctx->T->lean_at = eye_part + families * sph_cells;
         }
         HIP_TRY(hipGetLastError());
         HIP_TRY(hipStreamSynchronize(ctx->stream));
@@ -348,6 +396,7 @@
     g.g_eye = ge;
     g.g_sph = gs;
     g.path_enabled = 1;
+    apply_lean_lists(ctx);
     return TRT_OK;
 }
 
@@ -359,7 +408,9 @@
     const size_t sd = (size_t)std::max(ctx->dirgrid_slabs, 1), sp = (size_t)std::max(ctx->pointgrid_shells, 1);
     const int m = patches_for(ctx, (int)n);
     const size_t sphere_cells = 2 * n * (m ? 6 * (size_t)m * m : 1) * 6 * gs * gs;
-    const size_t wide = n > TRT_LIST_MAX_SPHERES ? 2 : 1, sphere_part = n > TRT_PATH_MAX_SPHERES ? 0 : (m ? sphere_cells / 2 : sphere_cells);
+    const bool twins = builds_lean_lists(ctx, 2 * n * (m ? 6 * (size_t)m * m : 1), 6 * gs * gs, (size_t)kEyeSlots * 2 * 6 * ge * ge);
+    const size_t with_twins = twins ? sphere_cells + sphere_cells / 2 : sphere_cells;
+    const size_t wide = n > TRT_LIST_MAX_SPHERES ? 2 : 1, sphere_part = n > TRT_PATH_MAX_SPHERES ? 0 : (m ? with_twins / 2 : with_twins);
     ctx->T->pool_scene_words = std::max<size_t>(1024, wide * (nd * sd * gd * gd + np * 6 * sp * gp * gp + sphere_part));
     const size_t per_word = wide == 2 ? 4 : 8;
     ctx->T->pool_eye_words = std::max<size_t>(1024, 2 * 6 * ge * ge * std::min<size_t>((n + per_word - 1) / per_word, 64));
diff --git a/terminalraytracer_amd/hip.py b/terminalraytracer_amd/hip.py
--- a/terminalraytracer_amd/hip.py
+++ b/terminalraytracer_amd/hip.py
@@ -112,6 +112,9 @@
     "trt_set_scratch_fill": (_I, [_VP, _I]),
     "trt_default_context": (_VP, []),
     "trt_build_counts": (_I, [_VP, C.POINTER(C.c_ulonglong), C.POINTER(C.c_ulonglong)]),
+    "trt_set_path_lean_lists": (_I, [_VP, _I]),
+    "trt_get_path_lean_lists": (_I, [_VP, C.POINTER(_I), C.POINTER(C.c_ulonglong)]),
+    "trt_read_path_lean_tables": (C.c_long, [_VP, _VP, C.c_size_t]),
     "trt_read_path_tables": (C.c_long, [_VP, C.POINTER(L.Camera), _VP, C.c_size_t, _VP, C.c_size_t, C.POINTER(C.c_long)]),
     "trt_read_sweep_fallbacks": (_I, [_VP, C.POINTER(C.c_ulonglong)]),
     "trt_read_shading_passes": (_I, [_VP, C.POINTER(C.c_ulonglong)]),
@@ -310,6 +313,22 @@
         keys = ("enabled", "eye_cells", "sphere_cells", "spheres", "cells", "pool_used_scene", "pool_used_eye", "pool_capacity")
         return dict(zip(keys, [int(x) for x in info])), cells[:got], pool
 
+    def set_path_lean_lists(self, mode):
+        _check(lib().trt_set_path_lean_lists(self._h, mode))
+
+    def path_lean_lists(self):
+        u, b = _I(), C.c_ulonglong()
+        _check(lib().trt_get_path_lean_lists(self._h, C.byref(u), C.byref(b)))
+        return {"in_use": bool(u.value), "twin_bytes": b.value}
+
+    def read_path_lean_tables(self):
+        n = self.path_lean_lists()["twin_bytes"] // 8
+        cells = np.zeros(max(1, n), dtype=np.uint64)
+        got = lib().trt_read_path_lean_tables(self._h, cells.ctypes.data, cells.size)
+        if got < 0:
+            _check(int(got))
+        return cells[:got]
+
     def set_refraction(self, ior=None):
         if ior is None:
             _check(lib().trt_set_refraction(self._h, None, 0))
```

Result: faster. 37.74 billion, median of 6 (+1.1%).
